# ingonyama-zk/blaze

Measured on AMD Instinct MI355X. Metric: BLS12-381 MSM/s at 2^26, higher is better.
Workload: dtype u32 registers holding 28-bit limbs (381-bit Fq, Montgomery)

## Files before the change

### blaze_amd/_lib.py

```python
from __future__ import annotations

import ctypes as C
import os

_HERE = os.path.dirname(os.path.abspath(__file__))
LIB_PATH = os.environ.get("BLAZE_HIP_LIB") or os.path.join(_HERE, "lib", "libblaze_hip.so")


class DriverClientError(Exception):

    VARIANTS = {
        1: "WriteError",
        2: "ReadError",
        3: "HBICAPNotReady",
        4: "InvalidPrimitiveParam",
        5: "CsvError",
        6: "LoadFailed",
        7: "FileError",
        8: "Unknown",
    }

    def __init__(self, code: int, message: str):
        self.code = code
        self.variant = self.VARIANTS.get(code, "Unknown")
        super().__init__(f"{self.variant}: {message}")


_lib = None
_aux = None

class BlzVecArg(C.Structure):
    _fields_ = [("d_ptr", C.c_void_p), ("buf", C.c_uint32), ("reserved", C.c_uint32), ("count", C.c_uint64)]


class BlzVecView(C.Structure):
    _fields_ = [("offset", C.c_uint64), ("stride", C.c_uint64), ("len", C.c_uint64)]


GATE_MAX_TABLES, GATE_MAX_TERMS, GATE_MAX_FACTORS, GATE_MAX_POINTS = 12, 8, 4, 6


class BlzGateTerm(C.Structure):
    _fields_ = [("nfactors", C.c_uint8), ("negate", C.c_uint8), ("factor", C.c_uint8 * GATE_MAX_FACTORS), ("reserved", C.c_uint8 * 2)]


class BlzSumGate(C.Structure):
    _fields_ = [("ntables", C.c_uint32), ("nterms", C.c_uint32), ("common", C.c_int32), ("reserved", C.c_uint32),
                ("term", BlzGateTerm * GATE_MAX_TERMS)]


class BlzVecCsr(C.Structure):
    _fields_ = [("d_row_ptr", C.c_void_p), ("d_col", C.c_void_p), ("d_val", C.c_void_p), ("rows", C.c_uint64), ("nnz", C.c_uint64)]


class BlzVecScatter(C.Structure):
    _fields_ = [("d_idx", C.c_void_p), ("d_src", C.c_void_p), ("d_val", C.c_void_p), ("nnz", C.c_uint64), ("reserved", C.c_uint64)]


_u8p = C.c_void_p
_SIGS = {
    "blz_last_error_message": (C.c_char_p, []),
    "blz_device_count": (C.c_int, []),
    "blz_point_size": (C.c_size_t, [C.c_int]),
    "blz_result_size": (C.c_size_t, [C.c_int]),
    "blz_msm_new": (C.c_int, [C.c_int, C.c_int, C.c_int, C.c_int, C.POINTER(C.c_void_p)]),
    "blz_msm_free": (None, [C.c_void_p]),
    "blz_msm_loaded_binary_parameters": (C.c_int, [C.c_void_p, C.POINTER(C.c_uint32)]),
    "blz_msm_initialize": (C.c_int, [C.c_void_p, C.c_uint32, C.c_int, C.c_uint64, C.c_uint64]),
    "blz_msm_start_process": (C.c_int, [C.c_void_p]),
    "blz_msm_set_data": (C.c_int, [C.c_void_p, _u8p, C.c_size_t, _u8p, C.c_size_t, C.c_uint32, C.c_int, C.c_uint64, C.c_uint64]),
    "blz_msm_set_data_device": (C.c_int, [C.c_void_p, _u8p, C.c_size_t, _u8p, C.c_size_t, C.c_uint32, C.c_int, C.c_uint64, C.c_uint64]),
    "blz_msm_wait_result": (C.c_int, [C.c_void_p]),
    "blz_msm_result": (C.c_int, [C.c_void_p, _u8p, C.c_size_t, C.POINTER(C.c_size_t), C.POINTER(C.c_uint32)]),
    "blz_msm_load_data_to_hbm": (C.c_int, [C.c_void_p, _u8p, C.c_size_t, C.c_uint64, C.c_uint64]),
    "blz_msm_load_data_to_hbm_device": (C.c_int, [C.c_void_p, _u8p, C.c_size_t, C.c_uint64, C.c_uint64]),
    "blz_msm_get_data_from_hbm": (C.c_int, [C.c_void_p, _u8p, C.c_size_t, C.c_uint64, C.c_uint64]),
    "blz_arena_release": (C.c_int, [C.c_int]),
    "blz_arena_set_policy": (C.c_int, [C.c_int, C.c_uint32]),
    "blz_arena_export": (C.c_int, [C.c_int, C.c_char_p]),
    "blz_arena_attach": (C.c_int, [C.c_int, C.c_char_p]),
    "blz_msm_stream": (C.c_int, [C.c_void_p, C.POINTER(C.c_void_p), C.POINTER(C.c_int)]),
    "blz_msm_task_label": (C.c_int, [C.c_void_p, C.POINTER(C.c_uint32)]),
    "blz_msm_nof_elements": (C.c_int, [C.c_void_p, C.POINTER(C.c_uint32)]),
    "blz_msm_is_engine_ready": (C.c_int, [C.c_void_p, C.POINTER(C.c_uint32)]),
    "blz_msm_stream_progress": (C.c_int, [C.c_void_p, C.POINTER(C.c_uint32)]),
    "blz_msm_reset": (C.c_int, [C.c_void_p]),
    "blz_msm_last_timings": (C.c_int, [C.c_void_p, C.POINTER(C.c_float)]),
    "blz_comm_unique_id": (C.c_int, [_u8p]),
    "blz_msm_comm_init": (C.c_int, [C.c_void_p, C.c_int, C.c_int, _u8p]),
    "blz_msm_all_gather_combine": (C.c_int, [C.c_void_p, _u8p, _u8p, C.c_size_t]),
    "blz_msm_comm_init_all": (C.c_int, [C.POINTER(C.c_void_p), C.c_int]),
    "blz_msm_all_gather_combine_all": (C.c_int, [C.POINTER(C.c_void_p), C.c_int, _u8p, _u8p, C.c_size_t]),
    "blz_msm_comm_free": (C.c_int, [C.c_void_p]),
    "blz_msm_precompute_bases_device": (C.c_int, [C.c_int, C.c_int, C.c_void_p, C.c_void_p, C.c_uint64]),
    "blz_msm_combine_partials": (C.c_int, [C.c_void_p, _u8p, C.c_size_t, _u8p, C.c_size_t]),
    "blz_msm_last_sort_hidden": (C.c_int, [C.c_void_p, C.POINTER(C.c_int)]),
    "blz_msm_memory_info": (C.c_int, [C.c_void_p, C.POINTER(C.c_uint64)]),
    "blz_msm_set_window_table": (C.c_int, [C.c_void_p, C.c_int]),
    "blz_msm_prepare_window_table": (C.c_int, [C.c_void_p, C.c_uint32, C.c_uint64, C.c_uint64, C.c_int, C.POINTER(C.c_int)]),
    "blz_msm_set_precompute_plan": (C.c_int, [C.c_void_p, C.c_int]),
    "blz_msm_prepare_precompute_plan": (C.c_int, [C.c_void_p, C.c_uint32, C.c_uint64, C.c_uint64, C.POINTER(C.c_int)]),
    "blz_msm_precompute_plan_info": (C.c_int, [C.c_void_p, C.POINTER(C.c_uint64)]),
    "blz_msm_set_scalar_range": (C.c_int, [C.c_void_p, C.c_uint32, C.c_uint32]),
    "blz_msm_shard_layout": (C.c_int, [C.c_int, C.c_uint32, C.c_int, C.c_int, C.POINTER(C.c_uint32)]),
    "blz_msm_shard_layout_ex": (C.c_int, [C.c_int, C.c_uint32, C.c_int, C.c_int, C.c_uint32, C.POINTER(C.c_uint32)]),
    "blz_msm_shard_layout_candidate": (C.c_int, [C.c_int, C.c_uint32, C.c_int, C.c_int, C.c_uint32, C.c_int, C.POINTER(C.c_uint32)]),
    "blz_msm_window_table_info": (C.c_int, [C.c_void_p, C.POINTER(C.c_uint64)]),
    "blz_msm_plan": (C.c_int, [C.c_int, C.c_uint32, C.c_int, C.POINTER(C.c_uint32), C.POINTER(C.c_uint8)]),
    "blz_ntt_new": (C.c_int, [C.c_int, C.c_int, C.POINTER(C.c_void_p)]),
    "blz_ntt_new_ex": (C.c_int, [C.c_int, C.c_int, C.c_int, C.POINTER(C.c_void_p)]),
    "blz_ntt_new_field": (C.c_int, [C.c_int, C.c_int, C.c_int, C.c_int, C.POINTER(C.c_void_p)]),
    "blz_ntt_new_ex2": (C.c_int, [C.c_int, C.c_int, C.c_int, C.c_int, C.c_uint32, C.POINTER(C.c_void_p)]),
    "blz_ntt_new_ex3": (C.c_int, [C.c_int, C.c_int, C.c_int, C.c_uint32, C.c_void_p, C.POINTER(C.c_void_p)]),
    "blz_ntt_set_coset": (C.c_int, [C.c_void_p, C.c_void_p]),
    "blz_ntt_get_coset": (C.c_int, [C.c_void_p, _u8p]),
    "blz_ntt_info": (C.c_int, [C.c_void_p, C.POINTER(C.c_uint64)]),
    "blz_ntt_exchange": (C.c_int, [C.c_void_p, C.c_size_t, _u8p, C.c_size_t, _u8p, C.c_size_t]),
    "blz_ntt_free": (None, [C.c_void_p]),
    "blz_ntt_initialize": (C.c_int, [C.c_void_p]),
    "blz_ntt_set_data": (C.c_int, [C.c_void_p, C.c_size_t, _u8p, C.c_size_t]),
    "blz_ntt_set_data_device": (C.c_int, [C.c_void_p, C.c_size_t, _u8p, C.c_size_t]),
    "blz_ntt_start_process": (C.c_int, [C.c_void_p, C.c_size_t]),
    "blz_ntt_wait_result": (C.c_int, [C.c_void_p]),
    "blz_ntt_result": (C.c_int, [C.c_void_p, C.c_size_t, _u8p, C.c_size_t]),
    "blz_ntt_result_device": (C.c_int, [C.c_void_p, C.c_size_t, _u8p, C.c_size_t]),
    "blz_ntt_stream": (C.c_int, [C.c_void_p, C.POINTER(C.c_void_p), C.POINTER(C.c_int)]),
    "blz_ntt_reset": (C.c_int, [C.c_void_p]),
    "blz_ntt_last_kernel_ms": (C.c_int, [C.c_void_p, C.POINTER(C.c_float)]),
    "blz_ntt_gate_eval": (C.c_int, [C.c_void_p, C.POINTER(BlzSumGate), C.POINTER(BlzVecArg), C.POINTER(BlzVecArg), C.POINTER(C.c_uint64), C.c_uint64]),
    "blz_ntt_vec_op": (C.c_int, [C.c_void_p, C.c_int, C.c_size_t, C.POINTER(BlzVecArg), C.POINTER(BlzVecArg), C.POINTER(BlzVecArg)]),
    "blz_ntt_vec_reduce": (C.c_int, [C.c_void_p, C.c_int, C.POINTER(BlzVecArg), C.POINTER(BlzVecArg), C.c_void_p]),
    "blz_ntt_vec_scan": (C.c_int, [C.c_void_p, C.c_int, C.c_uint32, C.c_size_t, C.POINTER(BlzVecArg), C.c_void_p]),
    "blz_ntt_vec_horner": (C.c_int, [C.c_void_p, C.c_uint32, C.c_size_t, C.POINTER(BlzVecArg), C.POINTER(BlzVecArg), C.c_void_p]),
    "blz_ntt_vec_gather": (C.c_int, [C.c_void_p, C.c_size_t, C.POINTER(BlzVecArg), C.POINTER(BlzVecView)]),
    "blz_ntt_vec_scatter": (C.c_int, [C.c_void_p, C.c_size_t, C.POINTER(BlzVecArg), C.POINTER(BlzVecScatter)]),
    "blz_ntt_vec_spmv": (C.c_int, [C.c_void_p, C.c_size_t, C.POINTER(BlzVecArg), C.POINTER(BlzVecCsr)]),
    "blz_ntt_vec_mle_fold": (C.c_int, [C.c_void_p, C.c_uint32, C.POINTER(BlzVecArg), C.POINTER(BlzVecArg), C.POINTER(BlzVecArg), C.c_uint64]),
    "blz_ntt_vec_mle_round": (C.c_int, [C.c_void_p, C.c_uint32, C.POINTER(BlzVecArg), C.POINTER(BlzVecArg), C.POINTER(BlzVecArg), C.c_uint32,
                                        C.c_uint64, C.c_void_p]),
    "blz_ntt_vec_mle_eq": (C.c_int, [C.c_void_p, C.POINTER(BlzVecArg), C.c_void_p, C.c_uint32]),
    "blz_ntt_banks_preprocess_device": (C.c_int, [C.c_void_p, _u8p, _u8p]),
    "blz_ntt_banks_postprocess_device": (C.c_int, [C.c_void_p, _u8p, _u8p]),
    "blz_ntt_sumcheck_step": (C.c_int, [C.c_void_p, C.c_uint32, C.POINTER(BlzVecArg), C.POINTER(BlzVecArg), C.POINTER(BlzVecArg), C.POINTER(BlzVecArg),
                                        C.POINTER(BlzVecArg), C.c_uint32, C.c_uint64, C.c_void_p]),
    "blz_ntt_sumcheck_gate": (C.c_int, [C.c_void_p, C.POINTER(BlzSumGate), C.POINTER(BlzVecArg), C.POINTER(BlzVecArg), C.c_uint32, C.c_uint64, C.c_void_p]),
    "blz_poseidon_new": (C.c_int, [C.c_int, C.c_int, C.POINTER(C.c_void_p)]),
    "blz_poseidon_free": (None, [C.c_void_p]),
    "blz_poseidon_loaded_binary_parameters": (C.c_int, [C.c_void_p, C.POINTER(C.c_uint32)]),
    "blz_poseidon_initialize": (C.c_int, [C.c_void_p, C.c_uint32, C.c_int, C.c_char_p]),
    "blz_poseidon_check_words": (C.c_int, [C.c_int, C.c_int, _u8p, C.c_size_t, C.POINTER(C.c_uint32)]),
    "blz_poseidon_initialize_words": (C.c_int, [C.c_void_p, C.c_uint32, C.c_int, _u8p, C.c_size_t]),
    "blz_poseidon_set_data": (C.c_int, [C.c_void_p, _u8p, C.c_size_t]),
    "blz_poseidon_set_data_device": (C.c_int, [C.c_void_p, C.c_void_p, C.c_size_t]),
    "blz_poseidon_wait_result": (C.c_int, [C.c_void_p]),
    "blz_poseidon_num_pending_results": (C.c_int, [C.c_void_p, C.POINTER(C.c_uint32)]),
    "blz_poseidon_raw_results": (C.c_int, [C.c_void_p, C.c_uint32, _u8p, C.c_size_t]),
    "blz_poseidon_result": (C.c_int, [C.c_void_p, C.c_uint32, _u8p, C.c_size_t, C.POINTER(C.c_uint32)]),
    "blz_poseidon_tree_device": (C.c_int, [C.c_void_p, C.c_void_p, C.c_size_t]),
    "blz_poseidon_counters": (C.c_int, [C.c_void_p, C.POINTER(C.c_uint32)]),
    "blz_poseidon_info": (C.c_int, [C.c_void_p, C.POINTER(C.c_uint64)]),
    "blz_poseidon_set_round_plan": (C.c_int, [C.c_void_p, C.c_int]),
    "blz_poseidon_prepare_round_plan": (C.c_int, [C.c_void_p, C.POINTER(C.c_uint32)]),
    "blz_poseidon_last_kernel_ms": (C.c_int, [C.c_void_p, C.POINTER(C.c_float)]),
    "blz_poseidon_stream": (C.c_int, [C.c_void_p, C.POINTER(C.c_void_p), C.POINTER(C.c_int)]),
    "blz_poseidon_reset": (C.c_int, [C.c_void_p]),
    "blz_device_malloc": (C.c_int, [C.c_int, C.c_size_t, C.POINTER(C.c_void_p)]),
    "blz_device_free": (C.c_int, [C.c_int, C.c_void_p]),
    "blz_host_malloc": (C.c_int, [C.c_int, C.c_size_t, C.POINTER(C.c_void_p)]),
    "blz_host_free": (C.c_int, [C.c_void_p]),
    "blz_memcpy_h2d": (C.c_int, [C.c_int, C.c_void_p, _u8p, C.c_size_t]),
    "blz_memcpy_d2h": (C.c_int, [C.c_int, _u8p, C.c_void_p, C.c_size_t]),
}
EXPORTED_SYMBOLS = tuple(_SIGS)
_AUX_SIGS = {
    "blz_synth_scalars": (C.c_int, [C.c_int, C.c_int, C.c_void_p, C.c_uint64, C.c_uint64]),
    "blz_synth_scalars_at": (C.c_int, [C.c_int, C.c_int, C.c_void_p, C.c_uint64, C.c_uint64, C.c_uint64]),
    "blz_synth_points": (C.c_int, [C.c_int, C.c_int, C.c_void_p, C.c_uint64, C.c_int, C.c_uint64]),
    "blz_synth_field_elements": (C.c_int, [C.c_int, C.c_void_p, C.c_uint64, C.c_uint64]),
    "blz_calib_mad_rate": (C.c_int, [C.c_int, C.c_uint32, C.POINTER(C.c_double)]),
    "blz_test_msm_stall": (C.c_int, [C.c_void_p, C.c_uint32, C.POINTER(C.c_void_p)]),
    "blz_test_ntt_stall": (C.c_int, [C.c_void_p, C.c_uint32, C.POINTER(C.c_void_p)]),
    "blz_test_stall_release": (C.c_int, [C.c_void_p]),
    "blz_test_field_op": (C.c_int, [C.c_int, C.c_int, C.c_int, C.c_int, _u8p, _u8p, _u8p, C.c_size_t]),
    "blz_test_ec_op": (C.c_int, [C.c_int, C.c_int, C.c_int, _u8p, _u8p, _u8p, _u8p, _u8p, C.c_size_t]),
    "blz_test_msm_tail_plan": (C.c_int, [C.c_int, C.c_int, C.c_uint32, C.c_int, C.c_int, C.c_int, C.c_int, C.c_int, C.POINTER(C.c_uint32), C.POINTER(C.c_uint8),
                                         C.c_char_p, C.c_size_t]),
    "blz_test_msm_sort_plan": (C.c_int, [C.c_int, C.c_int, C.c_uint32, C.c_int, C.c_int, C.c_int, C.c_int, C.c_int, C.c_int, C.c_int, C.c_int, C.c_int,
                                         C.c_char_p, C.c_size_t]),
    "blz_test_law_layout": (C.c_int, [C.c_int, C.c_int, C.c_int, C.POINTER(C.c_uint32)]),
    "blz_test_law_op": (C.c_int, [C.c_int, C.c_int, C.c_int, C.c_int, C.c_int, C.c_int, C.c_uint32, C.c_uint32, _u8p, _u8p, C.c_size_t]),
    "blz_test_rr_layout": (C.c_int, [C.c_int, C.c_int, C.POINTER(C.c_uint32)]),
    "blz_test_rr_op": (C.c_int, [C.c_int, C.c_int, C.c_int, C.c_int, C.c_int, _u8p, _u8p, C.c_size_t]),
    "blz_test_sort_fits_beside": (C.c_int, [C.c_int, C.c_int, C.c_int, C.c_int]),
    "blz_test_poseidon_permute": (C.c_int, [C.c_int, C.c_int, _u8p, C.c_size_t, C.c_int, _u8p, _u8p, C.c_size_t]),
    "blz_test_poseidon_hash": (C.c_int, [C.c_int, C.c_int, _u8p, C.c_size_t, C.c_int, _u8p, _u8p, C.c_size_t]),
    "blz_test_poseidon_hash_plan": (C.c_int, [C.c_int, C.c_int, _u8p, C.c_size_t, C.c_int, _u8p, _u8p, C.c_size_t, C.POINTER(C.c_uint32)]),
    "blz_test_poseidon_tree_check": (C.c_int, [C.c_int, C.c_int, _u8p, C.c_size_t, C.c_int, C.c_uint32, C.c_void_p, C.c_void_p, C.POINTER(C.c_uint64)]),
}
AUX_EXPORTED_SYMBOLS = tuple(_AUX_SIGS)


def lib():
    global _lib
    if _lib is None:
        if not os.path.exists(LIB_PATH):
            raise RuntimeError(
                f"{LIB_PATH} is missing: build it with `make -C blaze_amd/csrc` "
                "(or __graft_entry__.build()); blaze_amd has no CPU fallback"
            )
        L = C.CDLL(LIB_PATH, mode=C.RTLD_GLOBAL)
        for name, (res, args) in _SIGS.items():
            fn = getattr(L, name)
            fn.restype = res
            fn.argtypes = args
        _lib = L
    return _lib


def aux():
    global _aux
    if _aux is None:
        lib()
        path = LIB_PATH[:-3] + "_aux.so"
        if not os.path.exists(path):
            raise RuntimeError(f"{path} is missing: build it with `make -C blaze_amd/csrc`")
        A = C.CDLL(path)
        for name, (res, args) in _AUX_SIGS.items():
            fn = getattr(A, name)
            fn.restype = res
            fn.argtypes = args
        _aux = A
    return _aux


def check(rc: int):
    if rc != 0:
        msg = lib().blz_last_error_message()
        raise DriverClientError(rc, msg.decode() if msg else "")


def buf_ptr(buf):
    if buf is None:
        return None, 0, None
    if isinstance(buf, bytes):
        return C.cast(C.c_char_p(buf), C.c_void_p), len(buf), buf
    if isinstance(buf, bytearray):
        arr = (C.c_char * len(buf)).from_buffer(buf)
        return C.cast(arr, C.c_void_p), len(buf), arr
    if hasattr(buf, "ctypes") and hasattr(buf, "nbytes"):
        if not buf.flags["C_CONTIGUOUS"]:
            raise ValueError("numpy array is not C-contiguous: pass np.ascontiguousarray(a) (inputs) or a contiguous buffer (outputs)")
        return C.c_void_p(buf.ctypes.data), int(buf.nbytes), buf
    mv = memoryview(buf)
    if mv.readonly:
        b = mv.tobytes()
        return C.cast(C.c_char_p(b), C.c_void_p), len(b), b
    arr = (C.c_char * mv.nbytes).from_buffer(mv)
    return C.cast(arr, C.c_void_p), mv.nbytes, arr


class DeviceBuffer:

    def __init__(self, device_id: int, nbytes: int):
        self.device_id = device_id
        self.nbytes = nbytes
        p = C.c_void_p()
        check(lib().blz_device_malloc(device_id, nbytes, C.byref(p)))
        self.ptr = p.value

    def upload(self, data):
        p, n, _keep = buf_ptr(data)
        assert n <= self.nbytes
        check(lib().blz_memcpy_h2d(self.device_id, self.ptr, p, n))

    def download(self, nbytes: int | None = None, offset: int = 0) -> bytearray:
        n = self.nbytes - offset if nbytes is None else nbytes
        out = bytearray(n)
        p, _, _keep = buf_ptr(out)
        check(lib().blz_memcpy_d2h(self.device_id, p, self.ptr + offset, n))
        return out

    def free(self):
        if self.ptr:
            lib().blz_device_free(self.device_id, self.ptr)
            self.ptr = None

    def __del__(self):
        try:
            self.free()
        except Exception:
            pass


class HostBuffer:

    def __init__(self, device_id: int, nbytes: int):
        self.nbytes = nbytes
        p = C.c_void_p()
        check(lib().blz_host_malloc(device_id, nbytes, C.byref(p)))
        self.ptr = p.value
        self._arr = (C.c_uint8 * nbytes).from_address(self.ptr)

    def array(self):
        import numpy as np

        return np.frombuffer(self._arr, dtype=np.uint8)

    def free(self):
        if self.ptr:
            self._arr = None
            lib().blz_host_free(self.ptr)
            self.ptr = None

    def __del__(self):
        try:
            self.free()
        except Exception:
            pass
```

### blaze_amd/csrc/msm.hip

```cpp
#include "msm_engine.hpp"
#include <mutex>
#include "field.hip.hpp"
#include "msm_digits.hip.hpp"

namespace blz {

size_t fq_bytes(int curve) { return curve == BLZ_BN254 ? 32 : 48; }
size_t mont_point_bytes(int curve) { return curve == BLZ_BN254 ? 64 : 128; }

static uint32_t unit_length(uint32_t npts, int W) {
    const double chain = (double)npts * W * 5.5e-6;
    uint32_t L = 16;
    while (L < 256 && 2.0 * L <= chain) L <<= 1;
    return L;
}

static MsmPlan search_plan(uint32_t npts, int sbits, int ebits, int force_c, int split_ns, int max_w) {
    MsmPlan best;
    double best_cost = 1e300;
    const double t_entry = 0.163, t_bucket = 0.62, t_empty = 0.03, t_hot = 0.01;
    const int need = sbits + 1;
    const double t_split = (double)split_ns;
    for (int cmin = 3; cmin <= 23; ++cmin) {
        if (force_c > 0 && cmin != force_c) continue;
// ... 47 lines not shown
                    }
                    best.boff[W] = b;
                    best.Wv = (int)(G >> (cmin - 1));
                    best.cost = cost;
                    best.ebits = ebits;
                }
            }
        }
    }
    best.L = unit_length(npts, best.W);
    return best;
}

MsmPlan make_plan(uint32_t npts, int sbits, int ebits, int force_c) {
    if (ebits <= 0 || ebits > sbits) ebits = sbits;
    const int split_ns = plan_override("split_ns", 6000);
    struct Memo {
        uint32_t npts = 0;
        int sbits = 0, ebits = 0, force_c = 0, split_ns = 0;
        MsmPlan plan;
    };
    static std::mutex mu;
    static Memo memo[16];
    static unsigned next = 0;
    {
        std::lock_guard<std::mutex> lk(mu);
        for (const Memo& m : memo)
            if (m.sbits == sbits && m.npts == npts && m.ebits == ebits && m.force_c == force_c && m.split_ns == split_ns) return m.plan;
    }
    const int max_w = (sbits == 64 && force_c == 0 && npts >= (3u << 22)) ? 3 : MSM_MAX_W;
    const MsmPlan P = search_plan(npts, sbits, ebits, force_c, split_ns, max_w);
    std::lock_guard<std::mutex> lk(mu);
    Memo& m = memo[next++ % 16];
    m.npts = npts; m.sbits = sbits; m.ebits = ebits; m.force_c = force_c; m.split_ns = split_ns;
    m.plan = P;
    return P;
}

int table_window_bits(uint32_t npts, int need_bits) {
    const int forced = plan_override("table_c", 0);
    int best = 0;
    double best_cost = 1e300;
    for (int c = 16; c <= 26; ++c) {
        if (forced > 0 && c != forced) continue;
        const int W = table_windows(c, need_bits);
        if (c > 16 && table_windows(c - 1, need_bits) == W && forced <= 0) continue;
        if ((uint64_t)npts * W >= (1ull << 30)) continue;
        const double cost = (double)npts * W * 0.130 + (double)(1ull << (c - 1)) * 0.34;
        if (cost < best_cost) { best_cost = cost; best = c; }
    }
    return best;
}

MsmPlan make_table_plan(uint32_t npts, int c, int need_bits) {
    MsmPlan P;
    if (c < 16 || c > 26 || need_bits < 2 || need_bits > 257) return P;
    const int W = table_windows(c, need_bits);
    if ((uint64_t)npts * W >= (1ull << 30)) return P;
    P.npts = npts; P.sbits = need_bits - 1; P.c = c; P.W = W; P.table = true;
    P.G = 1ull << (c - 1);
    for (int w = 0; w < W; ++w) { P.width[w] = (uint8_t)c; P.boff[w] = 0; }
    P.boff[W] = (uint32_t)P.G;
    P.Bw = 1u << (c - 1 - 5);
    P.Wv = 32;
    P.L = unit_length(npts, W);
    return P;
}

int plan_tail(const MsmPlan& P, TailTraits tr, bool piecewise, TailPlan& T) {
    T = TailPlan();
    const uint64_t maxunits = ((uint64_t)P.npts * (P.table ? P.W : 1) + P.L - 1) / P.L;
    for (uint64_t stride = 1; stride < maxunits; stride *= 16) ++T.unit_passes;
    T.thr = ((uint64_t)P.npts * P.W / (P.G ? P.G : 1) > P.L / 2 || P.npts <= (1u << 22)) ? 64u : 0u;
    T.hot_start = (uint32_t)P.G;
    if (tr.rr && !P.table && !piecewise && P.ebits > 0) {
        int lowest = -1, off = 0;
        bool any = false;
        int offs[MSM_MAX_W];
        for (int w = 0; w < P.W; ++w) { offs[w] = off; off += P.width[w]; }
        for (int w = P.W - 1; w >= 0; --w) {
            const int cw = P.width[w];
            int t = P.ebits - offs[w];
            if (t > cw) t = cw;
            const double slots = (double)(1ull << (cw - 1));
            double active = t >= cw ? slots : t > 0 ? (double)(1ull << t) + 1.0 : t == 0 ? 1.0 : 0.0;
            if (active > slots) active = slots;
            const double entries = t >= 0 ? (double)P.npts : 0.0;
            const bool hot = active > 0 && entries / active >= 12.0 * (double)P.L;
            if (!hot && entries > 0) break;
            lowest = w;
            any = any || hot;
        }
        if (any && lowest > 0 && P.G - P.boff[lowest] <= 16384) T.hot_start = P.boff[lowest];
    }
    if (T.hot_start < P.G) T.hot = tr.row ? TailPlan::HOT_ROW : TailPlan::HOT_WAVES8;

    uint32_t seg0 = 64;
    while (seg0 > 8 && P.G / seg0 < 262144) seg0 >>= 1;
    seg0 = (uint32_t)exp_knob("BLAZE_MSM_SEG", (int)seg0);
    const uint32_t segu = (uint32_t)exp_knob("BLAZE_MSM_SEG_UPPER", 8);
    const uint32_t quad_max = (uint32_t)exp_knob("BLAZE_REDUCE_QUAD_MAX", 131072), row_max = (uint32_t)exp_knob("BLAZE_REDUCE_ROW_MAX", 8192);
    bool row_levels = false;
    int shift = 0;
    for (uint32_t M = P.Bw;;) {
        if (T.levels == 16) return fail(BLZ_ERR_UNKNOWN, "bucket reduce of %u buckets per window needs more than 16 levels (segments of %u / %u)", P.Bw, seg0, segu);
        TailPlan::Level& l = T.level[T.levels];
        l.M = M;
        l.SEG = T.levels == 0 ? seg0 : segu;
        l.T = l.SEG ? (M + l.SEG - 1) / l.SEG : M;
        l.shift = shift;
        if (tr.row && l.T * (uint32_t)P.Wv <= row_max) row_levels = true;
        l.kind = row_levels ? TailPlan::Level::ROW : !tr.rr ? TailPlan::Level::W32
                 : T.levels > 0 || l.T * (uint32_t)P.Wv <= quad_max ? TailPlan::Level::QUAD : TailPlan::Level::RR;
        for (uint32_t t = 1; t < l.SEG; t <<= 1) ++shift;
        ++T.levels;
        M = l.T;
        if (M == 1) break;
    }

    if (T.thr == 0 || T.hot_start == 0) T.fold = TailPlan::FOLD_NONE;
    else if (tr.row && !piecewise && P.G <= (1u << 17) && (uint64_t)P.npts * P.W / P.L <= (1u << 17))
        T.fold = T.level[0].kind == TailPlan::Level::ROW ? TailPlan::FOLD_ROW_WEAK : TailPlan::FOLD_ROW_STRICT;
    else
        T.fold = tr.rr && T.hot_start <= 32768 ? TailPlan::FOLD_WAVE : TailPlan::FOLD_LANE;

    T.finish_row = tr.row;
    FinishPlan& fp = T.fp;
    fp.W = P.W;
    fp.logV = 0;
    while ((1u << fp.logV) < P.Bw) ++fp.logV;
    if (P.table) {
        fp.W = 1;
        fp.v0[0] = 0;
        fp.m[0] = (uint8_t)(P.G >> fp.logV);
        fp.off[0] = 0;
    } else {
        int off = P.base_bit;
        for (int w = 0; w < P.W; ++w) {
            const uint32_t v0 = P.boff[w] >> fp.logV, m = (P.boff[w + 1] - P.boff[w]) >> fp.logV;
            if (v0 > 0xffffu || m > 0xffu || off > 0xffff)
                return fail(BLZ_ERR_UNKNOWN, "window plan outside k_finish's table range (window %d: v0=%u m=%u off=%d)", w, v0, m, off);
            fp.v0[w] = (uint16_t)v0;
            fp.m[w] = (uint8_t)m;
            fp.off[w] = (uint16_t)off;
            off += P.width[w];
        }
    }

    const char* bad = nullptr;
    if ((T.hot == TailPlan::HOT_WAVES8 || T.fold == TailPlan::FOLD_WAVE) && !tr.rr) bad = "a reduced-radix fold";
    if ((T.hot == TailPlan::HOT_ROW || T.fold == TailPlan::FOLD_ROW_STRICT || T.fold == TailPlan::FOLD_ROW_WEAK || T.finish_row) && !tr.row) bad = "a row-law kernel";
    if (!T.finish_row && tr.row) bad = "the quad walk";
    if (T.fold == TailPlan::FOLD_ROW_WEAK && T.level[0].kind != TailPlan::Level::ROW) bad = "a weak row fold without a row level 0 behind it";
    for (int l = 0; l < T.levels && !bad; ++l) {
        const TailPlan::Level::Kind k = T.level[l].kind;
        if (k == TailPlan::Level::ROW ? !tr.row : k == TailPlan::Level::W32 ? tr.rr : !tr.rr) bad = "a reduce level on a law the field lacks";
        else if (k == TailPlan::Level::RR && l > 0) bad = "the lane-per-segment reduced-radix level above level 0";
        else if (l > 0 && T.level[l - 1].kind == TailPlan::Level::ROW && k != TailPlan::Level::ROW) bad = "a row level in front of another law's";
    }
    if (bad) return fail(BLZ_ERR_UNKNOWN, "tail plan names %s (%s)", bad, describe(T).c_str());
    return BLZ_OK;
}

std::string describe(const TailPlan& T) {
    static const char* const hot[] = {"", " hot", " hot_row"};
    static const char* const fold[] = {"none", "lane", "wave", "row_strict", "row_weak"};
    static const char* const kind[] = {"w32", "rr", "quad", "row"};
    std::string s = "units" + std::to_string(T.unit_passes) + hot[T.hot] + " fold_" + fold[T.fold] + " |";
    for (int l = 0; l < T.levels; ++l) s += std::string(l ? " L" : " L0") + kind[T.level[l].kind];
    return s + (T.finish_row ? " finish_row" : " finish");
}

__global__ __launch_bounds__(64) void k_words_to_pinned(uint32_t* __restrict__ dst, const uint32_t* __restrict__ src, uint32_t n) {
    __builtin_amdgcn_s_setprio(3);
    if (threadIdx.x < n) __hip_atomic_store(dst + threadIdx.x, src[threadIdx.x], __ATOMIC_RELAXED, __HIP_MEMORY_SCOPE_SYSTEM);
}
int copy_words_to_pinned(void* host_pinned, const void* d_src, uint32_t dwords, hipStream_t st) {
    if (dwords > 64) return fail(BLZ_ERR_UNKNOWN, "copy_words_to_pinned: %u dwords", dwords);
    hipLaunchKernelGGL(k_words_to_pinned, dim3(1), dim3(64), 0, st, (uint32_t*)host_pinned, (const uint32_t*)d_src, dwords);
    BLZ_HIP(hipGetLastError(), BLZ_ERR_READ);
    return BLZ_OK;
}

__global__ __launch_bounds__(256) void k_iota(uint32_t* __restrict__ p, uint64_t n) {
    for (uint64_t i = (uint64_t)blockIdx.x * 256 + threadIdx.x; i < n; i += (uint64_t)gridDim.x * 256) p[i] = (uint32_t)i;
}


const MsmCurveOps* msm_ops_for(int curve, int repr) {
    switch (curve) {
        case BLZ_BLS377: return &msm_ops_bls377();
        case BLZ_BLS381: return &msm_ops_bls381();
        case BLZ_BN254: return repr ? &msm_ops_bn254_w32() : &msm_ops_bn254();
    }
    return nullptr;
}

int msm_points_from_mont(int format_id, const void* d_mont, void* d_raw, uint64_t npts, hipStream_t st) {
    const MsmCurveOps* ops = (format_id >> 16) ? nullptr : msm_ops_for(format_id & 0xff, (format_id >> 8) & 0xff);
    if (!ops) return fail(BLZ_ERR_UNKNOWN, "no conversion back from Montgomery format 0x%x", format_id);
    return ops->points_from_mont(d_mont, d_raw, npts, st);
}
int msm_points_all_canonical(int format_id, const void* d_raw, uint64_t npts, uint32_t* flag, hipStream_t st) {
    const MsmCurveOps* ops = msm_ops_for(format_id & 0xff, (format_id >> 8) & 0xff);
    if (!ops) return fail(BLZ_ERR_UNKNOWN, "unknown Montgomery format 0x%x", format_id);
    return ops->points_all_canonical(d_raw, npts, flag, st);
}

int MsmEngine::init(int device_id, int curve_id, int precompute_factor) {
    device = device_id;
    curve = curve_id;
    repr = 0;
    if (curve == BLZ_BN254) {
        repr = exp_knob("BLAZE_BN254_REPR", precompute_factor > 1 ? 1 : 0) ? 1 : 0;
    }
    if (!msm_ops_for(curve, repr)) return fail(BLZ_ERR_INVALID_PARAM, "unknown curve %d", curve);
    BLZ_TRY(use_device(device));
    int prio_low = 0, prio_high = 0;
    BLZ_HIP(hipDeviceGetStreamPriorityRange(&prio_low, &prio_high), BLZ_ERR_UNKNOWN);
    BLZ_HIP(hipStreamCreateWithFlags(&stream, hipStreamNonBlocking), BLZ_ERR_UNKNOWN);
    BLZ_HIP(hipStreamCreateWithPriority(&tail_stream, hipStreamNonBlocking, prio_high), BLZ_ERR_UNKNOWN);
    BLZ_HIP(hipStreamCreateWithPriority(&aux_stream, hipStreamNonBlocking, prio_high), BLZ_ERR_UNKNOWN);
    BLZ_HIP(hipStreamCreateWithPriority(&sort_stream, hipStreamNonBlocking, prio_high), BLZ_ERR_UNKNOWN);
    last_sort_done = nullptr;
    for (auto& S : slots) {
        BLZ_TRY(for_each_event(S, [](hipEvent_t& e, bool timed) -> int {
            if (timed) BLZ_HIP(hipEventCreate(&e), BLZ_ERR_UNKNOWN);
            else BLZ_HIP(hipEventCreateWithFlags(&e, hipEventDisableTiming), BLZ_ERR_UNKNOWN);
            return BLZ_OK;
        }));
        BLZ_HIP(hipHostMalloc((void**)&S.result_h, 256), BLZ_ERR_UNKNOWN);
        BLZ_HIP(hipHostMalloc((void**)&S.stats_h, 64), BLZ_ERR_UNKNOWN);
        memset(S.stats_h, 0, 64);
    }
    BLZ_HIP(hipHostMalloc((void**)&combine_h, 256), BLZ_ERR_UNKNOWN);
    for (auto& B : sbuf) BLZ_TRY(B.stats.reserve(64));
    BLZ_TRY(result.reserve(256 * 64));
    return BLZ_OK;
}

bool MsmEngine::destroy() {
    if (!stream) return true;
    (void)hipSetDevice(device);
    if (sync_stream_bounded(stream, "free: main stream") != BLZ_OK || sync_stream_bounded(tail_stream, "free: tail stream") != BLZ_OK ||
        sync_stream_bounded(sort_stream, "free: sort stream") != BLZ_OK) {
        BLZ_LOG(0, "MSM engine freed while its device work is wedged: workspace and streams are leaked");
        stream = tail_stream = aux_stream = sort_stream = nullptr;
        return false;
    }
    for_each_buf([](DevBuf& b) { b.release(); });
    for (auto& S : slots) {
        (void)for_each_event(S, [](hipEvent_t& e, bool) -> int { if (e) (void)hipEventDestroy(e); return BLZ_OK; });
        if (S.result_h) (void)hipHostFree(S.result_h);
        if (S.stats_h) (void)hipHostFree(S.stats_h);
        S = MsmSlot();
    }
    inputs_event = nullptr;
    if (combine_h) (void)hipHostFree(combine_h);
    combine_h = nullptr;
    for (hipStream_t s : {stream, tail_stream, aux_stream, sort_stream}) (void)hipStreamDestroy(s);
    stream = tail_stream = aux_stream = sort_stream = nullptr;
    last_sort_done = nullptr;
    return true;
}

bool MsmEngine::can_accept() const {
    for (const auto& S : slots)
        if (!S.busy) return true;
    return false;
}

int MsmEngine::sync_all() {
    BLZ_TRY(use_device(device));
    BLZ_TRY(sync_stream_bounded(stream, "reset: main stream"));
    BLZ_TRY(sync_stream_bounded(tail_stream, "reset: tail stream"));
    BLZ_TRY(sync_stream_bounded(aux_stream, "reset: exchange stream"));
    BLZ_TRY(sync_stream_bounded(sort_stream, "reset: sort stream"));
    for (auto& S : slots) { S.busy = false; S.open = false; S.task_inputs_event = nullptr; }
    return BLZ_OK;
}

int MsmEngine::points_to_mont(const void* d_raw, void* d_mont, uint32_t npts) {
    BLZ_TRY(use_device(device));
    return msm_ops_for(curve, repr)->points_to_mont(*this, d_raw, d_mont, npts);
}

int MsmEngine::points_to_mont_even(const void* d_raw, void* d_mont, uint32_t nq) {
    BLZ_TRY(use_device(device));
    return msm_ops_for(curve, repr)->points_to_mont_even(*this, d_raw, d_mont, nq);
}
int MsmEngine::check_precompute(const void* d_raw, uint64_t nelem, uint32_t* flag, hipStream_t st) {
    BLZ_TRY(use_device(device));
    return msm_ops_for(curve, 0)->check_precompute(*this, d_raw, nelem, flag, st);
}

int MsmEngine::build_table(const void* d_raw, void* d_table, uint32_t npts, int c, int W, int base_shift, void* scratch, uint32_t* flag,
                           hipStream_t st) {
    BLZ_TRY(use_device(device));
    return msm_ops_for(curve, repr)->build_table(*this, d_raw, d_table, npts, c, W, base_shift, scratch, flag, st);
}
size_t MsmEngine::table_scratch_bytes(int W) const { return msm_ops_for(curve, repr)->table_scratch_bytes(W); }

static const int kScalarFieldBits[3] = {253, 255, 254};

MsmPlan MsmEngine::plan_for(uint32_t npts, int sbits) const {
    const int ebits = sbits == 256 ? kScalarFieldBits[curve] : sbits;
    return make_plan(npts, sbits, ebits, plan_override("c", 0));
}

static MsmPlan range_plan(int curve, uint32_t npts, int bit_lo, int bit_hi) {
    const int vbits = bit_hi - bit_lo;
    int ebits = kScalarFieldBits[curve] - bit_lo;
    if (ebits > vbits) ebits = vbits;
    if (ebits < 1) ebits = 1;
    MsmPlan P = make_plan(npts, vbits, ebits, plan_override("c", 0));
    P.base_bit = bit_lo;
    return P;
}
MsmPlan MsmEngine::plan_for_range(uint32_t npts, int bit_lo, int bit_hi) const { return range_plan(curve, npts, bit_lo, bit_hi); }

int msm_task_plan(int curve, uint32_t npts, int sbits, int table_c, int bit_lo, int bit_hi, MsmPlan& P, bool* ranged_out) {
    if (curve < 0 || curve > 2) return fail(BLZ_ERR_INVALID_PARAM, "unknown curve %d", curve);
    const int ebits = sbits == 256 ? kScalarFieldBits[curve] : sbits;
    const bool ranged = bit_hi > bit_lo && !(bit_lo == 0 && bit_hi >= sbits);
    if (ranged && (sbits != 256 || (bit_lo & 31) || (bit_hi & 31) || bit_hi > 256))
        return fail(BLZ_ERR_INVALID_PARAM, "scalar range [%d, %d): 32-bit aligned ranges of 256-bit scalars", bit_lo, bit_hi);
    P = table_c > 0 ? make_table_plan(npts, table_c, ranged ? bit_hi - bit_lo + 1 : 257)
        : ranged    ? range_plan(curve, npts, bit_lo, bit_hi)
                    : make_plan(npts, sbits, ebits, plan_override("c", 0));
    if (P.c == 0) return fail(BLZ_ERR_INVALID_PARAM, "no window plan for npts=%u sbits=%d%s", npts, sbits, table_c > 0 ? " (window table)" : "");
    if (P.table && !msm_sort3_ok(P, sbits)) return fail(BLZ_ERR_INVALID_PARAM, "window-table task outside the sort's range (c=%d)", P.c);
    P.L = (uint32_t)plan_override("L", (int)P.L);
    if (P.L < 1) P.L = 1;
    if (P.L > (uint32_t)MAX_L) P.L = MAX_L;
    if (ranged_out) *ranged_out = ranged;
    return BLZ_OK;
}

int msm_task_pieces(const MsmPlan& P, int want, bool phased, uint32_t* per_out) {
    if (want < 1 || P.table) want = 1;
    if (want > MSM_MAX_SLICES) want = MSM_MAX_SLICES;
    const uint64_t halves = (phased && want >= 4) ? 2ull * want - 1 : 2ull * want;
    const uint32_t per = (uint32_t)(((2ull * P.npts + halves - 1) / halves + 15) & ~(uint64_t)15);
    if (want > 1) want = (int)(((uint64_t)P.npts + per - 1) / per);
    *per_out = want > 1 ? per : P.npts;
    return want;
}

int MsmEngine::take_slot(int* slot_out) {
    int slot = (rr_cursor + 1) % MSM_QUEUE_DEPTH;
    if (slots[slot].busy) slot = (slot + 1) % MSM_QUEUE_DEPTH;
    if (slots[slot].busy) return fail(BLZ_ERR_INVALID_PARAM, "task queue full (%d tasks in flight)", MSM_QUEUE_DEPTH);
    *slot_out = slot;
    return BLZ_OK;
}

int MsmEngine::step(int slot, int piece, bool curve_kernels, std::optional<MsmStep>& out) {
    BLZ_TRY(use_device(device));
    if (slot < 0 || slot >= MSM_QUEUE_DEPTH || !slots[slot].open) return fail(BLZ_ERR_INVALID_PARAM, "slot %d has no task being enqueued", slot);
    MsmSlot& S = slots[slot];
    if (curve_kernels && S.repr != repr) return fail(BLZ_ERR_INVALID_PARAM, "the handle's arithmetic changed while task %d was being enqueued", slot);
    if (S.slices == 1) piece = -1;
    const int set = S.sort.where == SortPlan::PINGPONG && piece >= 0 ? (slot + piece) % MSM_QUEUE_DEPTH : slot;
    out.emplace(MsmStep{slot, S, piece, S.plan, sbuf[set], stream, S.sort.where != SortPlan::OPEN ? sort_stream : stream});
    return BLZ_OK;
}

int MsmEngine::begin(uint32_t npts, int sbits, int* slot_out, int table_c, int bit_lo, int bit_hi, int nslices, bool phased) {
    BLZ_TRY(use_device(device));
    const MsmCurveOps* ops = msm_ops_for(curve, repr);
    hipStream_t st = stream;
    if (npts == 0) return fail(BLZ_ERR_INVALID_PARAM, "begin: empty task");
    int slot = -1;
    BLZ_TRY(take_slot(&slot));
    MsmSlot& S = slots[slot];
    MsmPlan P;
    bool ranged = false;
    BLZ_TRY(msm_task_plan(curve, npts, sbits, table_c, bit_lo, bit_hi, P, &ranged));
    const uint64_t G = P.G;
    uint32_t per = npts;
    nslices = msm_task_pieces(P, nslices, phased, &per);
    BLZ_TRY(plan_tail(P, ops->tail, nslices > 1, S.tail));
    const SortInputs sort_in = {env_int("BLAZE_SORT_HIDE", 1), slots[(slot + 1) % MSM_QUEUE_DEPTH].busy, recent_hot[0] || recent_hot[1],
                                msm_sort_fits_beside(ops->accumulate_vgprs(), msm_sort3_max_vgprs(P.table), ops->accumulate_lds(), msm_sort3_max_lds(P.table))};
    const SortPlan sort = plan_sort(P, npts, sbits, nslices, sort_in);
    BLZ_LOG(2, "msm plan: npts=%u sbits=%d c=%d W=%d Bw=%u G=%llu L=%u pieces=%d sort: %s tail: %s", npts, sbits, P.c, P.W, P.Bw,
            (unsigned long long)G, P.L, nslices, describe(sort).c_str(), describe(S.tail).c_str());
    const uint64_t max_entries = (uint64_t)per * P.W;
    const uint64_t max_units = G + max_entries / P.L + 1;
    if (max_units >= (1ull << 32)) return fail(BLZ_ERR_INVALID_PARAM, "unit bound %llu exceeds 32 bits", (unsigned long long)max_units);

    rr_cursor = slot;
    if (slot_out) *slot_out = slot;
    S.plan = P;
    S.npts = npts;
    S.sbits = sbits;
    S.ranged = ranged;
    S.bit_lo = bit_lo;
    S.bit_hi = bit_hi;
    S.repr = repr;
    S.slices = nslices;
    S.pts_per_slice = per;
    S.max_units = max_units;
    S.sort = sort;
    S.acc_pp_recorded[0] = S.acc_pp_recorded[1] = false;
    S.phased = phased;
    S.task_inputs_event = inputs_event;
    S.accum_timed = false;
    BLZ_HIP(hipEventRecord(S.ev[0], st), BLZ_ERR_UNKNOWN);
    for (int b = 0; b < MSM_QUEUE_DEPTH; ++b) {
        if (b != slot && sort.where != SortPlan::PINGPONG) continue;
        BLZ_TRY(sbuf[b].count.reserve((G + 1) * 4 + 16));
        BLZ_TRY(sbuf[b].off.reserve((G + 2) * 4));
        BLZ_TRY(sbuf[b].unit_off.reserve((G + 2) * 4));
        BLZ_TRY(sbuf[b].entries.reserve(max_entries * 4));
    }
    BLZ_TRY(blocksums.reserve((size_t)((G + 1 + SCAN_TILE - 1) / SCAN_TILE) * 8));
    if (nslices > 1) {
        const size_t sum_bytes = (size_t)ops->tail.partial_dwords * 4;
        BLZ_TRY(bucket_sums.reserve((G + 1) * sum_bytes));
        BLZ_TRY(bucket_ident.reserve((G + 2) * 4));
        launch_zero(bucket_sums.p, ((G + 1) * sum_bytes + 15) / 16, st);
        BLZ_HIP(hipGetLastError(), BLZ_ERR_UNKNOWN);
    }
    S.open = true;
    S.busy = true;
    return BLZ_OK;
}

int MsmEngine::sort_slice(int slot, int sl, const void* d_scalars, uint32_t np) {
    std::optional<MsmStep> C;
    BLZ_TRY(step(slot, sl, false, C));
    MsmSlot& S = C->S;
    if (sl < 0 || sl >= S.slices || np == 0 || np > S.pts_per_slice) return fail(BLZ_ERR_INVALID_PARAM, "piece %d of %d with %u points", sl, S.slices, np);
    rr_cursor = slot;
    MsmSlot& O = slots[(slot + 1) % MSM_QUEUE_DEPTH];
    const bool hide = S.sort.where != SortPlan::OPEN, pingpong = S.sort.where == SortPlan::PINGPONG;
    hipStream_t ss = C->sort_stream;
    if (last_sort_done) BLZ_HIP(hipStreamWaitEvent(ss, last_sort_done, 0), BLZ_ERR_UNKNOWN);
    if (hide) {
        if (pingpong && S.acc_pp_recorded[sl & 1]) {
            BLZ_HIP(hipStreamWaitEvent(ss, S.ev_acc_pp[sl & 1], 0), BLZ_ERR_UNKNOWN);
        } else {
            if (S.l0_recorded) BLZ_HIP(hipStreamWaitEvent(ss, S.ev_l0, 0), BLZ_ERR_UNKNOWN);
            if (O.sort.where == SortPlan::PINGPONG && O.l0_recorded) BLZ_HIP(hipStreamWaitEvent(ss, O.ev_l0, 0), BLZ_ERR_UNKNOWN);
        }
    }
    BLZ_HIP(hipEventRecord(S.ev_s0, ss), BLZ_ERR_UNKNOWN);
    BLZ_TRY(msm_sort_stage(*this, *C, d_scalars, np));
    hipEvent_t sorted = pingpong ? S.ev_sorted_pp[sl & 1] : S.ev_sorted;
    BLZ_HIP(hipEventRecord(sorted, ss), BLZ_ERR_UNKNOWN);
    last_sort_done = sorted;
    BLZ_HIP(hipEventRecord(S.ev_s1, ss), BLZ_ERR_UNKNOWN);
    if (!S.phased && S.task_inputs_event && sl + 1 == S.slices) {
        if (hide) BLZ_HIP(hipStreamWaitEvent(ss, S.ev[0], 0), BLZ_ERR_UNKNOWN);
        BLZ_HIP(hipEventRecord(S.task_inputs_event, ss), BLZ_ERR_UNKNOWN);
        S.task_inputs_event = nullptr;
    }
    return BLZ_OK;
}

int MsmEngine::accumulate_slice(int slot, int sl, const void* d_pts) {
    std::optional<MsmStep> C;
    BLZ_TRY(step(slot, sl, true, C));
    MsmSlot& S = C->S;
    const MsmCurveOps* ops = msm_ops_for(curve, repr);
    rr_cursor = slot;
    const bool pingpong = S.sort.where == SortPlan::PINGPONG;
    if (S.sort.where != SortPlan::OPEN) BLZ_HIP(hipStreamWaitEvent(stream, pingpong ? S.ev_sorted_pp[sl & 1] : S.ev_sorted, 0), BLZ_ERR_UNKNOWN);
    BLZ_TRY(ops->run_accumulate(*this, *C, d_pts, (uint32_t)S.max_units));
    if (S.slices > 1) BLZ_TRY(ops->merge_buckets(*this, *C));
    if (pingpong) {
        BLZ_HIP(hipEventRecord(S.ev_acc_pp[sl & 1], stream), BLZ_ERR_UNKNOWN);
        S.acc_pp_recorded[sl & 1] = true;
    }
    return BLZ_OK;
}

int MsmEngine::end(int slot) {
    std::optional<MsmStep> C;
    BLZ_TRY(step(slot, -1, true, C));
    MsmSlot& S = C->S;
    const MsmCurveOps* ops = msm_ops_for(curve, repr);
    rr_cursor = slot;
    if (S.task_inputs_event) {
        BLZ_HIP(hipEventRecord(S.task_inputs_event, stream), BLZ_ERR_UNKNOWN);
        S.task_inputs_event = nullptr;
    }
    if (S.slices > 1) {
        hipLaunchKernelGGL(k_iota, dim3(1024), dim3(256), 0, stream, bucket_ident.as<uint32_t>(), S.plan.G + 2);
        BLZ_TRY(ops->run_reduce(*this, *C, bucket_sums.p, bucket_ident.p));
    } else {
        BLZ_TRY(ops->run_reduce(*this, *C, partial.p, C->B.unit_off.p));
    }
    S.l0_recorded = true;
    S.open = false;
    return BLZ_OK;
}

void MsmEngine::abandon(int slot) {
    if (slot < 0 || slot >= MSM_QUEUE_DEPTH) return;
    MsmSlot& S = slots[slot];
    if (S.busy && S.open) {
        S.busy = false;
        S.open = false;
        S.task_inputs_event = nullptr;
    }
}

int MsmEngine::run(const void* d_pts, const void* d_scalars, uint32_t npts, int sbits, int* slot_out, int table_c, int bit_lo,
                   int bit_hi) {
    BLZ_TRY(use_device(device));
    if (npts == 0) {
        hipStream_t st = stream;
        int slot = -1;
        BLZ_TRY(take_slot(&slot));
        rr_cursor = slot;
        MsmSlot& S = slots[slot];
        if (slot_out) *slot_out = slot;
        BLZ_HIP(hipEventRecord(S.ev[0], st), BLZ_ERR_UNKNOWN);
        BLZ_TRY(msm_ops_for(curve, repr)->emit_infinity(*this, slot));
        for (int i = 1; i <= 4; ++i) BLZ_HIP(hipEventRecord(S.ev[i], st), BLZ_ERR_UNKNOWN);
        BLZ_TRY(copy_words_to_pinned(S.result_h, slot_result(slot), (uint32_t)(3 * fq_bytes(curve) / 4), st));
        BLZ_HIP(hipEventRecord(S.ev_done, st), BLZ_ERR_UNKNOWN);
        S.plan = MsmPlan();
        S.accum_timed = false;
        S.open = false;
        S.busy = true;
        return BLZ_OK;
    }
    int pieces = env_int("BLAZE_MSM_PIECES", 1);
    int slot = -1;
    BLZ_TRY(begin(npts, sbits, &slot, table_c, bit_lo, bit_hi, pieces, false));
    if (slot_out) *slot_out = slot;
    MsmSlot& S = slots[slot];
    int rc = BLZ_OK;
    for (int sl = 0; sl < S.slices && rc == BLZ_OK; ++sl) {
        const uint32_t p0 = (uint32_t)sl * S.pts_per_slice;
        const uint32_t np = npts - p0 < S.pts_per_slice ? npts - p0 : S.pts_per_slice;
        rc = sort_slice(slot, sl, (const char*)d_scalars + (size_t)p0 * (sbits / 8), np);
        if (rc == BLZ_OK) rc = accumulate_slice(slot, sl, (const char*)d_pts + (size_t)p0 * mont_point_bytes(curve));
    }
    if (rc == BLZ_OK) rc = end(slot);
    if (rc != BLZ_OK) abandon(slot);
    return rc;
}

int MsmEngine::finish(int slot, uint8_t* out) {
    BLZ_TRY(use_device(device));
    if (slot < 0 || slot >= MSM_QUEUE_DEPTH || !slots[slot].busy) return fail(BLZ_ERR_INVALID_PARAM, "no task in slot %d", slot);
    if (slots[slot].open) return fail(BLZ_ERR_INVALID_PARAM, "task in slot %d never received all of its data", slot);
    MsmSlot& S = slots[slot];
    BLZ_TRY(sync_event_bounded(S.ev_done, "wait_result: MSM task"));
    S.busy = false;
    if (S.plan.c) {
        BLZ_LOG(2, "msm: units=%u max_bucket=%u entries=%u", S.stats_h[0], S.stats_h[1], S.stats_h[2]);
        if ((uint64_t)S.stats_h[0] > S.max_units) return fail(BLZ_ERR_UNKNOWN, "unit count %u exceeds its bound", S.stats_h[0]);
        const uint64_t mean = (uint64_t)S.stats_h[2] / (S.plan.G ? S.plan.G : 1) + 1;
        recent_hot[1] = recent_hot[0];
        recent_hot[0] = (uint64_t)S.stats_h[1] > 64 * mean + 4096;
    }
    memcpy(out, S.result_h, 3 * fq_bytes(curve));
    float t = 0;
    (void)hipEventElapsedTime(&t, S.ev[0], S.ev[4]); last_ms[0] = t;
    last_ms[1] = 0;
    if (S.accum_timed && S.plan.c) {
        if (S.slices > 1) {
            for (int i = 0; i < S.slices; ++i)
                if (hipEventElapsedTime(&t, S.slice_ev[2 * i], S.slice_ev[2 * i + 1]) == hipSuccess) last_ms[1] += t;
        } else {
            (void)hipEventElapsedTime(&t, S.ev[5], S.ev[6]);
            last_ms[1] = t;
        }
    }
    last_sort_hidden = S.sort.where != SortPlan::OPEN && S.plan.c != 0;
    if (S.plan.c) (void)hipEventElapsedTime(&t, S.ev_s0, S.ev_s1);
    else t = 0;
    last_ms[2] = t;
    (void)hipEventElapsedTime(&t, S.ev[1], S.ev[2]); last_ms[3] = t;
    (void)hipEventElapsedTime(&t, S.ev[2], S.ev[3]); last_ms[4] = t;
    (void)hipEventElapsedTime(&t, S.ev[3], S.ev[4]); last_ms[5] = t;
    last_ms[6] = (float)S.plan.c;
    last_ms[7] = (float)S.plan.W;
    return BLZ_OK;
}

int MsmEngine::combine_partials(const uint8_t* partials, size_t cnt, uint8_t* out, bool on_device) {
    BLZ_TRY(use_device(device));
    return msm_ops_for(curve, repr)->combine(*this, partials, cnt, out, on_device);
}

}
```

### blaze_amd/csrc/msm_engine.hpp

```cpp
#pragma once
#include "common.hpp"
#include <optional>

namespace blz {

constexpr int MSM_MAX_W = 96;
constexpr uint64_t MSM_MAX_ENTRIES = (1ull << 32) - (1ull << 26);
struct MsmPlan {
    uint32_t npts = 0;
    int sbits = 256;
    int c = 0;
    int W = 0;
    uint8_t width[MSM_MAX_W] = {};
    uint32_t boff[MSM_MAX_W + 1] = {};
    uint32_t Bw = 0;
    int Wv = 0;
    uint64_t G = 0;
    uint32_t L = 0;
    bool table = false;
    int ebits = 0;
    int base_bit = 0;
    double cost = 0;
};
MsmPlan make_plan(uint32_t npts, int sbits, int ebits, int force_c);
int table_window_bits(uint32_t npts, int need_bits = 257);
inline int table_windows(int c, int need_bits = 257) { return (need_bits + c - 1) / c; }
MsmPlan make_table_plan(uint32_t npts, int c, int need_bits = 257);
int msm_task_plan(int curve, uint32_t npts, int sbits, int table_c, int bit_lo, int bit_hi, MsmPlan& P, bool* ranged);
int msm_task_pieces(const MsmPlan& P, int want, bool phased, uint32_t* per);

struct TailTraits {
    bool rr = false;
    bool row = false;
    int partial_dwords = 0;
};
struct FinishPlan {
    int W, logV;
    uint16_t v0[MSM_MAX_W], off[MSM_MAX_W];
    uint8_t m[MSM_MAX_W];
};
struct TailPlan {
    uint32_t thr = 0, hot_start = 0;
    int unit_passes = 0;
    enum Hot { HOT_NONE, HOT_WAVES8, HOT_ROW } hot = HOT_NONE;
    enum Fold { FOLD_NONE, FOLD_LANE, FOLD_WAVE, FOLD_ROW_STRICT, FOLD_ROW_WEAK } fold = FOLD_NONE;
    struct Level {
        uint32_t M, SEG, T;
        int shift;
        enum Kind { W32, RR, QUAD, ROW } kind;
    } level[16];
    int levels = 0;
    bool finish_row = false;
    FinishPlan fp;
};
int plan_tail(const MsmPlan& P, TailTraits tr, bool piecewise, TailPlan& out);
std::string describe(const TailPlan& T);

struct SortPlan {
    enum Kind { LDS, S3, TINY } kind;
    enum Where { OPEN, HIDDEN, PINGPONG } where;
};
struct SortInputs { int hide_env; bool other_busy, recent_hot, fits; };
SortPlan plan_sort(const MsmPlan& P, uint32_t npts, int sbits, int pieces, const SortInputs& in);
std::string describe(const SortPlan&);
constexpr int SCAN_TILE = 2048;
constexpr int MAX_L = 1024;

constexpr int MSM_QUEUE_DEPTH = 2;
constexpr int MSM_MAX_SLICES = 64;
struct MsmSlot {
    hipEvent_t ev[8] = {};
    hipEvent_t ev_l0 = nullptr;
    hipEvent_t ev_sorted = nullptr;
    hipEvent_t ev_s0 = nullptr, ev_s1 = nullptr;
    bool l0_recorded = false;
    hipEvent_t ev_done = nullptr;
    DevBuf lvlA[2], lvlC[2];
    uint8_t* result_h = nullptr;
    uint32_t* stats_h = nullptr;
    uint64_t max_units = 0;
    MsmPlan plan;
    SortPlan sort{};
    TailPlan tail;
    hipEvent_t slice_ev[2 * 64] = {};
    int slices = 1;
    bool accum_timed = false;
    bool busy = false;
    bool open = false;
    bool phased = false;
    bool ranged = false;
    uint32_t npts = 0, pts_per_slice = 0;
    int sbits = 0, bit_lo = 0, bit_hi = 0;
    int repr = 0;
    hipEvent_t task_inputs_event = nullptr;
    hipEvent_t ev_sorted_pp[2] = {nullptr, nullptr};
    hipEvent_t ev_acc_pp[2] = {nullptr, nullptr};
    bool acc_pp_recorded[2] = {false, false};
};

struct MsmStep;
struct MsmEngine {
    int device = 0;
    int curve = 0;
    int repr = 0;
    int format_id() const { return curve | (repr << 8); }
    hipStream_t stream = nullptr, tail_stream = nullptr, aux_stream = nullptr;
    MsmSlot slots[MSM_QUEUE_DEPTH];
    int rr_cursor = 0;
    struct SortBufs {
        DevBuf count, off, unit_off, unit_bucket, unit_order, lenhist, entries, stats;
        DevBuf range_scalars;
    };
    SortBufs sbuf[MSM_QUEUE_DEPTH];
    hipStream_t sort_stream = nullptr;
    hipEvent_t last_sort_done = nullptr;
    DevBuf coarse, inter, inter2, slice_map, partial, blocksums, result, sort3_tabs;
    DevBuf bucket_sums, bucket_ident;
    int begin(uint32_t npts, int sbits, int* slot, int table_c, int bit_lo, int bit_hi, int pieces, bool phased);
    int sort_slice(int slot, int piece, const void* d_scalars, uint32_t np);
    int accumulate_slice(int slot, int piece, const void* d_points_mont);
    int end(int slot);
    void abandon(int slot);
    int take_slot(int* slot);
    int step(int slot, int piece, bool curve_kernels, std::optional<MsmStep>& out);
    hipEvent_t inputs_event = nullptr;
    uint8_t* combine_h = nullptr;
    float last_ms[8] = {};
    bool last_sort_hidden = false;
    bool recent_hot[2] = {false, false};
    template <class Fn>
    void for_each_buf(Fn&& f) {
        for (DevBuf* b : {&coarse, &inter, &inter2, &slice_map, &partial, &blocksums, &result, &sort3_tabs, &bucket_sums, &bucket_ident}) f(*b);
        for (auto& B : sbuf)
            for (DevBuf* b : {&B.count, &B.off, &B.unit_off, &B.unit_bucket, &B.unit_order, &B.lenhist, &B.entries, &B.stats, &B.range_scalars}) f(*b);
        for (auto& S : slots)
            for (DevBuf* b : {&S.lvlA[0], &S.lvlA[1], &S.lvlC[0], &S.lvlC[1]}) f(*b);
    }
    template <class Fn>
    static int for_each_event(MsmSlot& S, Fn&& f) {
        for (auto& e : S.ev) BLZ_TRY(f(e, true));
        for (auto& e : S.slice_ev) BLZ_TRY(f(e, true));
        for (hipEvent_t* e : {&S.ev_l0, &S.ev_done, &S.ev_sorted, &S.ev_sorted_pp[0], &S.ev_acc_pp[0], &S.ev_sorted_pp[1], &S.ev_acc_pp[1]}) BLZ_TRY(f(*e, false));
        for (hipEvent_t* e : {&S.ev_s0, &S.ev_s1}) BLZ_TRY(f(*e, true));
        return BLZ_OK;
    }

    int init(int device_id, int curve_id, int precompute_factor);
    bool destroy();
    uint32_t* slot_result(int s) { return result.as<uint32_t>() + (size_t)s * 64; }
    bool can_accept() const;
    MsmPlan plan_for(uint32_t npts, int sbits) const;
    int points_to_mont(const void* d_raw, void* d_mont, uint32_t npts);
    int points_to_mont_even(const void* d_raw, void* d_mont, uint32_t nq);
    int check_precompute(const void* d_raw, uint64_t nelem, uint32_t* flag, hipStream_t st);
    int build_table(const void* d_raw, void* d_table, uint32_t npts, int c, int W, int base_shift, void* scratch, uint32_t* flag,
                    hipStream_t st);
    size_t table_scratch_bytes(int W) const;
    int run(const void* d_points_mont, const void* d_scalars, uint32_t npts, int sbits, int* slot, int table_c = 0, int bit_lo = 0,
            int bit_hi = 0);
    MsmPlan plan_for_range(uint32_t npts, int bit_lo, int bit_hi) const;
    int finish(int slot, uint8_t* out);
    int combine_partials(const uint8_t* partials, size_t count, uint8_t* out, bool on_device);
    int sync_all();
};

struct MsmStep {
    int slot;
    MsmSlot& S;
    int piece;
    const MsmPlan& P;
    MsmEngine::SortBufs& B;
    hipStream_t stream, sort_stream;
};

int msm_points_from_mont(int format_id, const void* d_mont, void* d_raw, uint64_t npts, hipStream_t st);
int msm_points_all_canonical(int format_id, const void* d_raw, uint64_t npts, uint32_t* flag, hipStream_t st);
int copy_words_to_pinned(void* host_pinned, const void* d_src, uint32_t dwords, hipStream_t st);
size_t fq_bytes(int curve);
size_t mont_point_bytes(int curve);
int msm_sort_stage(MsmEngine& E, const MsmStep& C, const void* d_scalars, uint32_t np);
void launch_zero(void* p, size_t n16, hipStream_t st);
bool msm_sort3_ok(const MsmPlan& P, int sbits);
int msm_sort3_max_vgprs(bool table);
int msm_sort3_max_lds(bool table);
bool msm_sort_fits_beside(int av, int sv, int al, int sl);
bool msm_sort_tiny_ok(const MsmPlan& P, uint32_t npts, int sbits);

struct MsmCurveOps {
    int (*points_to_mont)(MsmEngine&, const void* d_raw, void* d_mont, uint32_t npts);
    int (*emit_infinity)(MsmEngine&, int slot);
    int (*run_accumulate)(MsmEngine&, const MsmStep& C, const void* d_pts, uint32_t max_units);
    int (*merge_buckets)(MsmEngine&, const MsmStep& C);
    int (*run_reduce)(MsmEngine&, const MsmStep& C, const void* sums, const void* unit_off);
    TailTraits tail;
    int (*accumulate_vgprs)();
    int (*accumulate_lds)();
    int (*build_table)(MsmEngine&, const void* d_raw, void* d_table, uint32_t npts, int c, int W, int base_shift, void* scratch,
                       uint32_t* flag, hipStream_t st);
    size_t (*table_scratch_bytes)(int W);
    int (*combine)(MsmEngine&, const uint8_t* partials, size_t count, uint8_t* out, bool on_device);
    int (*points_to_mont_even)(MsmEngine&, const void* d_raw, void* d_mont, uint32_t nq);
    int (*check_precompute)(MsmEngine&, const void* d_raw, uint64_t nelem, uint32_t* flag, hipStream_t st);
    int (*points_from_mont)(const void* d_mont, void* d_raw, uint64_t npts, hipStream_t st);
    int (*points_all_canonical)(const void* d_raw, uint64_t npts, uint32_t* flag, hipStream_t st);
};
const MsmCurveOps& msm_ops_bls377();
const MsmCurveOps& msm_ops_bls381();
const MsmCurveOps& msm_ops_bn254();
const MsmCurveOps& msm_ops_bn254_w32();
const MsmCurveOps* msm_ops_for(int curve, int repr = 0);

}
```

### blaze_amd/csrc/msm_sort3.hip

```cpp
#include "msm_sort.hpp"
#include "msm_digits.hip.hpp"

namespace blz {

constexpr int S3_THREADS = 256;
constexpr int S3_SH1 = 14;
constexpr int S3_SH2 = 7;
#ifndef BLZ_S3_T
#define BLZ_S3_T 8
#endif
constexpr int S3_T = BLZ_S3_T;
constexpr int S3_PB = S3_THREADS * S3_T;
constexpr uint32_t S3_SLICE2 = 4096;
constexpr int S3_T2 = S3_SLICE2 / S3_THREADS;
constexpr int S3_T3 = 28;
constexpr uint32_t S3_R3 = S3_THREADS * S3_T3;
constexpr uint32_t S3_MAXNB1 = 2048;
constexpr uint32_t S3_CNT_PTS = 16384;
constexpr uint32_t S3T_IMG = 12288;

struct S3Geom {
    int W, prio;
    uint32_t NB1;
    uint8_t width[MSM_MAX_W];
    uint16_t bitoff[MSM_MAX_W];
    uint16_t binoff1[MSM_MAX_W + 1];
    static constexpr bool TABLE = false;
    static constexpr uint32_t HIST1 = S3_MAXNB1;
    using Win = int;
    __device__ int cw(int w) const { return width[w]; }
    __device__ uint32_t first_bin(int w) const { return binoff1[w]; }
    __device__ static constexpr uint32_t shift1() { return S3_SH1; }
    static constexpr uint32_t bits3() { return S3_SH2; }
    __device__ static uint32_t index1(uint32_t p, uint32_t, uint32_t) { return p; }
    __device__ static uint32_t rem1(uint32_t rem) { return rem; }
    struct L2 {
        int prio;
        using Lo = uint8_t;
        static constexpr uint32_t TAB2 = 128;
        static constexpr uint32_t KY_D = 8, KY_R = 16;
        static constexpr uint32_t LO_MASK = 127u;
        __device__ static constexpr uint32_t shift2() { return S3_SH2; }
        __device__ static constexpr uint32_t bits2() { return S3_SH1 - S3_SH2; }
        __device__ static uint32_t low2(uint32_t r, uint32_t) { return r & 127u; }
        __device__ static uint32_t index2(uint32_t iw) { return iw; }
    };
    L2 l2() const { return L2{prio}; }
};

struct S3TGeom {
    int W, prio, c;
    uint32_t sh1, b2, b3, xs, NB1;
    static constexpr bool TABLE = true;
    static constexpr uint32_t HIST1 = 256;
    using Win = uint32_t;
    __device__ int cw(int) const { return c; }
    __device__ static constexpr uint32_t first_bin(int) { return 0; }
    __device__ uint32_t shift1() const { return sh1; }
    uint32_t bits3() const { return b3; }
    __device__ uint32_t index1(uint32_t p, uint32_t w, uint32_t rem) const { return (p * (uint32_t)W + w) | (xs ? (rem & 1u) << 30 : 0u); }
    __device__ uint32_t rem1(uint32_t rem) const { return rem >> xs; }
    using L2 = S3TGeom;
    using Lo = uint16_t;
    static constexpr uint32_t TAB2 = 256;
    static constexpr uint32_t KY_D = 10, KY_R = 18;
    static constexpr uint32_t LO_MASK = 0x3ffu;
    __device__ uint32_t shift2() const { return b3 - xs; }
    __device__ uint32_t bits2() const { return b2; }
    __device__ uint32_t low2(uint32_t r, uint32_t iw) const {
        const uint32_t lomask = (1u << shift2()) - 1u;
        return xs ? ((r & lomask) << 1) | ((iw >> 30) & 1u) : (r & lomask);
    }
    __device__ static uint32_t index2(uint32_t iw) { return iw & 0xbfffffffu; }
    const L2& l2() const { return *this; }
};

__device__ __forceinline__ void s3_setprio(int p) {
    if (p >= 3) __builtin_amdgcn_s_setprio(3);
    else if (p == 2) __builtin_amdgcn_s_setprio(2);
    else if (p == 1) __builtin_amdgcn_s_setprio(1);
}

__device__ __forceinline__ uint32_t s3_wave_incl_scan(uint32_t v) {
    for (int o = 1; o < 64; o <<= 1) {
        uint32_t t = __shfl_up(v, o, 64);
        if ((threadIdx.x & 63u) >= (uint32_t)o) v += t;
    }
    return v;
}
__device__ __forceinline__ uint32_t s3_block_excl_scan(uint32_t v, uint32_t* wave_tot, uint32_t* total) {
    const uint32_t incl = s3_wave_incl_scan(v);
    if ((threadIdx.x & 63u) == 63u) wave_tot[threadIdx.x >> 6] = incl;
    __syncthreads();
    uint32_t wbase = 0;
    for (uint32_t q = 0; q < (threadIdx.x >> 6); ++q) wbase += wave_tot[q];
    *total = wave_tot[0] + wave_tot[1] + wave_tot[2] + wave_tot[3];
    return wbase + incl - v;
}

template <class Geom, int NW>
__global__ __launch_bounds__(S3_THREADS, 4) void k3_l1_count(const uint32_t* __restrict__ scalars, uint32_t npts, Geom g,
                                                            uint32_t* __restrict__ cnt1) {
    s3_setprio(g.prio);
    __shared__ uint32_t hist[Geom::HIST1];
    if constexpr (Geom::HIST1 == S3_THREADS) hist[threadIdx.x] = 0;
    else for (uint32_t i = threadIdx.x; i < g.NB1; i += S3_THREADS) hist[i] = 0;
    __syncthreads();
    const uint32_t base = blockIdx.x * S3_CNT_PTS;
    uint32_t end = base + S3_CNT_PTS;
    if (end > npts) end = npts;
    for (uint32_t p0 = base + threadIdx.x; p0 < end; p0 += 4 * S3_THREADS) {
        ScalarWords<NW> sw[4];
#pragma unroll
        for (int u = 0; u < 4; ++u) {
            const uint32_t p = p0 + u * S3_THREADS;
            sw[u].load(scalars, p < end ? p : p0);
        }
#pragma unroll
        for (int u = 0; u < 4; ++u) {
            if (p0 + u * S3_THREADS >= end) break;
            uint32_t carry = 0;
            for (int w = 0; w < g.W; ++w) {
                const int cw = g.cw(w);
                const int d = sw[u].next(cw, (1u << cw) - 1u, 1u << (cw - 1), carry);
                if (d != 0) {
                    const uint32_t b = (uint32_t)(d < 0 ? -d : d) - 1u;
                    atomicAdd(&hist[g.first_bin(w) + (b >> g.shift1())], 1u);
                }
            }
        }
    }
    __syncthreads();
    auto flush = [&](uint32_t i) {
        const uint32_t v = hist[i];
        if (v) atomicAdd(&cnt1[i], v);
    };
    if constexpr (Geom::HIST1 == S3_THREADS) { if (threadIdx.x < g.NB1) flush(threadIdx.x); }
    else for (uint32_t i = threadIdx.x; i < g.NB1; i += S3_THREADS) flush(i);
}

__global__ __launch_bounds__(S3_THREADS) void k3_scan_small(const uint32_t* __restrict__ cnt, uint32_t n, uint32_t* __restrict__ off,
                                                           uint32_t* __restrict__ cur, int prio) {
    s3_setprio(prio);
    __shared__ uint32_t wave_tot[4];
    uint32_t v[8], sum = 0;
    const uint32_t b0 = threadIdx.x * 8u;
#pragma unroll
    for (int k = 0; k < 8; ++k) {
        v[k] = b0 + k < n ? cnt[b0 + k] : 0u;
        sum += v[k];
    }
    uint32_t total;
    uint32_t run = s3_block_excl_scan(sum, wave_tot, &total);
#pragma unroll
    for (int k = 0; k < 8; ++k) {
        if (b0 + k < n) {
            off[b0 + k] = run;
            cur[b0 + k] = run;
        }
        run += v[k];
    }
    if (threadIdx.x == 0) off[n] = total;
}

template <class Geom, int NW>
__global__ __launch_bounds__(S3_THREADS, 4) void k3_l1_scatter(const uint32_t* __restrict__ scalars, uint32_t npts, Geom g,
                                                              uint32_t* __restrict__ cur1, uint32_t* __restrict__ o_idx,
                                                              uint16_t* __restrict__ o_rem) {
    s3_setprio(g.prio);
    extern __shared__ __attribute__((aligned(16))) uint32_t sh[];
    uint32_t* sc = sh;
    uint2* stage = reinterpret_cast<uint2*>(sh + NW * S3_PB);
    uint32_t* hist = sh + (NW + 2) * S3_PB;
    uint32_t* lstart = hist + 256;
    uint32_t* gbase = lstart + 256;
    __shared__ uint32_t wave_tot[4];
    const uint32_t tid = threadIdx.x;
    const uint32_t base = blockIdx.x * (uint32_t)S3_PB;
#pragma unroll
    for (int u = 0; u < S3_T; ++u) {
        const uint32_t p = base + u * S3_THREADS + tid;
        const uint32_t i = u * S3_THREADS + tid;
        if constexpr (NW == 8) {
            uint4 a = make_uint4(0, 0, 0, 0), b = make_uint4(0, 0, 0, 0);
            if (p < npts) {
                const uint4* q = reinterpret_cast<const uint4*>(scalars) + 2 * (size_t)p;
                a = q[0];
                b = q[1];
            }
            sc[0 * S3_PB + i] = a.x; sc[1 * S3_PB + i] = a.y; sc[2 * S3_PB + i] = a.z; sc[3 * S3_PB + i] = a.w;
            sc[4 * S3_PB + i] = b.x; sc[5 * S3_PB + i] = b.y; sc[6 * S3_PB + i] = b.z; sc[7 * S3_PB + i] = b.w;
        } else if constexpr (NW == 2) {
            uint2 a = make_uint2(0, 0);
            if (p < npts) a = reinterpret_cast<const uint2*>(scalars)[p];
            sc[0 * S3_PB + i] = a.x; sc[1 * S3_PB + i] = a.y;
        } else {
            sc[i] = p < npts ? scalars[p] : 0u;
        }
    }
    uint32_t carry = 0;
    using Win = typename Geom::Win;
    for (Win w = 0; w < (Win)g.W; ++w) {
        uint32_t cw, off, nb;
        if constexpr (Geom::TABLE) { cw = (uint32_t)g.c; off = w * cw; nb = g.NB1; }
        else { cw = g.width[w]; off = g.bitoff[w]; nb = (uint32_t)g.binoff1[w + 1] - (uint32_t)g.binoff1[w]; }
        const uint32_t sh1 = g.shift1(), lowmask = (1u << sh1) - 1u;
        const uint32_t j = off >> 5, shb = off & 31u, mask = (1u << cw) - 1u, half = 1u << (cw - 1);
        if (Geom::TABLE || tid < nb) hist[tid] = 0;
        __syncthreads();
        uint32_t key[S3_T], rk[S3_T];
#pragma unroll
        for (int u = 0; u < S3_T; ++u) {
            const uint32_t i = u * S3_THREADS + tid;
            const uint32_t lo = j < (uint32_t)NW ? sc[j * S3_PB + i] : 0u;
            const uint32_t hi = j + 1 < (uint32_t)NW ? sc[(j + 1) * S3_PB + i] : 0u;
            const uint32_t raw = (shb ? __builtin_amdgcn_alignbit(hi, lo, shb) : lo) & mask;
            const uint32_t v = raw + ((carry >> u) & 1u);
            int d;
            if (v > half) { d = (int)v - (int)(half << 1); carry |= 1u << u; }
            else { d = (int)v; carry &= ~(1u << u); }
            rk[u] = ~0u;
            key[u] = 0;
            if (d != 0 && base + i < npts) {
                const uint32_t b = (uint32_t)(d < 0 ? -d : d) - 1u;
                const uint32_t bin = b >> sh1;
                key[u] = (b & lowmask) | (bin << sh1) | (d < 0 ? 0x80000000u : 0u);
                rk[u] = atomicAdd(&hist[bin], 1u);
            }
        }
        __syncthreads();
        {
            const uint32_t v = tid < nb ? hist[tid] : 0u;
            uint32_t total;
            const uint32_t excl = s3_block_excl_scan(v, wave_tot, &total);
            if (tid < nb) {
                lstart[tid] = excl;
                uint32_t ci;
                if constexpr (Geom::TABLE) ci = tid; else ci = (uint32_t)g.binoff1[w] + tid;
                gbase[tid] = v ? atomicAdd(&cur1[ci], v) : 0u;
            }
            __syncthreads();
#pragma unroll
            for (int u = 0; u < S3_T; ++u) {
                if (rk[u] != ~0u) {
                    const uint32_t bin = (key[u] >> sh1) & (Geom::TABLE ? 0xffu : 0x1ffu);
                    const uint32_t p = base + u * S3_THREADS + tid;
                    const uint32_t rem = key[u] & lowmask;
                    stage[lstart[bin] + rk[u]] = make_uint2((Geom::TABLE ? g.index1(p, (uint32_t)w, rem) : p) | (key[u] & 0x80000000u), g.rem1(rem) | (bin << 16));
                }
            }
            __syncthreads();
            for (uint32_t slot = tid; slot < total; slot += S3_THREADS) {
                const uint2 e = stage[slot];
                const uint32_t bin = e.y >> 16;
                const uint32_t dst = gbase[bin] + (slot - lstart[bin]);
                o_idx[dst] = e.x;
                o_rem[dst] = (uint16_t)e.y;
            }
        }
        __syncthreads();
    }
}

__global__ __launch_bounds__(S3_THREADS) void k3_slice_map(const uint32_t* __restrict__ off, uint32_t nbins, uint32_t slice,
                                                          uint2* __restrict__ map, uint32_t* __restrict__ nitems, int prio) {
    s3_setprio(prio);
    __shared__ uint32_t wave_tot[4];
    __shared__ uint32_t carry_sh;
    if (threadIdx.x == 0) carry_sh = 0;
    __syncthreads();
    for (uint32_t base = 0; base < nbins; base += S3_THREADS) {
        const uint32_t i = base + threadIdx.x;
        const uint32_t size = i < nbins ? off[i + 1] - off[i] : 0u;
        const uint32_t v = (size + slice - 1) / slice;
        uint32_t total;
        const uint32_t excl = s3_block_excl_scan(v, wave_tot, &total);
        const uint32_t first = carry_sh + excl;
        for (uint32_t q = 0; q < v; ++q) map[first + q] = make_uint2(i, q);
        __syncthreads();
        if (threadIdx.x == 0) carry_sh += total;
        __syncthreads();
    }
    if (threadIdx.x == 0) *nitems = carry_sh;
}

__global__ __launch_bounds__(S3_THREADS) void k3_scan_a(const uint32_t* __restrict__ cnt, uint32_t n, uint32_t* __restrict__ bsum, int prio) {
    s3_setprio(prio);
    __shared__ uint32_t wave_tot[4];
    const uint32_t b0 = blockIdx.x * 2048u + threadIdx.x * 8u;
    uint32_t sum = 0;
#pragma unroll
    for (int k = 0; k < 8; ++k) sum += b0 + k < n ? cnt[b0 + k] : 0u;
    uint32_t total;
    (void)s3_block_excl_scan(sum, wave_tot, &total);
    if (threadIdx.x == 0) bsum[blockIdx.x] = total;
}
__global__ __launch_bounds__(S3_THREADS) void k3_scan_b(uint32_t* __restrict__ bsum, uint32_t nblocks, int prio) {
    s3_setprio(prio);
    __shared__ uint32_t wave_tot[4];
    const uint32_t v = threadIdx.x < nblocks ? bsum[threadIdx.x] : 0u;
    uint32_t total;
    const uint32_t excl = s3_block_excl_scan(v, wave_tot, &total);
    if (threadIdx.x < nblocks) bsum[threadIdx.x] = excl;
    if (threadIdx.x == 0) bsum[256] = total;
}
__global__ __launch_bounds__(S3_THREADS) void k3_scan_c(const uint32_t* __restrict__ cnt, uint32_t n, const uint32_t* __restrict__ bsum,
                                                       uint32_t* __restrict__ off, uint32_t* __restrict__ cur, int prio) {
    s3_setprio(prio);
    __shared__ uint32_t wave_tot[4];
    const uint32_t b0 = blockIdx.x * 2048u + threadIdx.x * 8u;
    uint32_t v[8], sum = 0;
#pragma unroll
    for (int k = 0; k < 8; ++k) {
        v[k] = b0 + k < n ? cnt[b0 + k] : 0u;
        sum += v[k];
    }
    uint32_t total;
    uint32_t run = bsum[blockIdx.x] + s3_block_excl_scan(sum, wave_tot, &total);
#pragma unroll
    for (int k = 0; k < 8; ++k) {
        if (b0 + k < n) {
            off[b0 + k] = run;
            cur[b0 + k] = run;
        }
        run += v[k];
    }
    if (blockIdx.x == 0 && threadIdx.x == 0) off[n] = bsum[256];
}

__device__ __forceinline__ bool s3_item(const uint32_t* off1, const uint2* map, const uint32_t* nitems, uint32_t id, uint32_t slice,
                                        uint32_t& k, uint32_t& lo, uint32_t& hi) {
    if (id >= *nitems) return false;
    const uint2 m = map[id];
    k = m.x;
    const uint32_t a = off1[k], b = off1[k + 1];
    lo = a + m.y * slice;
    hi = lo + slice < b ? lo + slice : b;
    return lo < hi;
}

template <class Geom>
__global__ __launch_bounds__(S3_THREADS, 4) void k3_l2_count(const uint16_t* __restrict__ rem, const uint32_t* __restrict__ off1,
                                                            const uint2* __restrict__ map, const uint32_t* __restrict__ nitems,
                                                            uint32_t* __restrict__ cnt2, Geom g) {
    s3_setprio(g.prio);
    __shared__ uint32_t hist[Geom::TAB2];
    uint32_t k, lo, hi;
    if (!s3_item(off1, map, nitems, blockIdx.x, S3_SLICE2, k, lo, hi)) return;
    if (Geom::TAB2 == S3_THREADS || threadIdx.x < Geom::TAB2) hist[threadIdx.x] = 0;
    __syncthreads();
    const uint32_t sh = g.shift2();
    uint32_t r[S3_T2];
#pragma unroll
    for (int t = 0; t < S3_T2; ++t) {
        const uint32_t i = lo + t * S3_THREADS + threadIdx.x;
        r[t] = i < hi ? rem[i] : 0xffffffffu;
    }
#pragma unroll
    for (int t = 0; t < S3_T2; ++t)
        if (r[t] != 0xffffffffu) atomicAdd(&hist[r[t] >> sh], 1u);
    __syncthreads();
    if (threadIdx.x < (1u << g.bits2())) {
        const uint32_t v = hist[threadIdx.x];
        if (v) atomicAdd(&cnt2[(k << g.bits2()) + threadIdx.x], v);
    }
}

template <class Geom>
__global__ __launch_bounds__(S3_THREADS, 4) void k3_l2_scatter(const uint32_t* __restrict__ i_idx, const uint16_t* __restrict__ i_rem,
                                                              const uint32_t* __restrict__ off1, const uint2* __restrict__ map,
                                                              const uint32_t* __restrict__ nitems, uint32_t* __restrict__ cur2,
                                                              uint32_t* __restrict__ o_idx, typename Geom::Lo* __restrict__ o_lo, Geom g) {
    s3_setprio(g.prio);
    constexpr uint32_t TAB2 = Geom::TAB2, KY_D = Geom::KY_D, KY_R = Geom::KY_R;
    __shared__ uint2 stage[S3_SLICE2];
    __shared__ uint32_t hist[TAB2], lstart[TAB2], gbase[TAB2];
    __shared__ uint32_t wave_tot[4];
    uint32_t k, lo, hi;
    if (!s3_item(off1, map, nitems, blockIdx.x, S3_SLICE2, k, lo, hi)) return;
    const uint32_t tid = threadIdx.x;
    if (TAB2 == S3_THREADS || tid < TAB2) hist[tid] = 0;
    __syncthreads();
    const uint32_t sh = g.shift2(), nb2 = 1u << g.bits2();
    uint32_t ex[S3_T2], ky[S3_T2];
#pragma unroll
    for (int t = 0; t < S3_T2; ++t) {
        const uint32_t i = lo + t * S3_THREADS + tid;
        ky[t] = 0xffffffffu;
        ex[t] = 0;
        if (i < hi) {
            const uint32_t r = i_rem[i];
            const uint32_t iw = i_idx[i];
            const uint32_t h2 = r >> sh;
            const uint32_t low = g.low2(r, iw);
            ex[t] = g.index2(iw);
            const uint32_t rank = atomicAdd(&hist[h2], 1u);
            ky[t] = low | (h2 << KY_D) | (rank << KY_R);
        }
    }
    __syncthreads();
    const uint32_t v = tid < nb2 ? hist[tid] : 0u;
    uint32_t total;
    const uint32_t excl = s3_block_excl_scan(v, wave_tot, &total);
    if (tid < nb2) {
        lstart[tid] = excl;
        gbase[tid] = v ? atomicAdd(&cur2[(k << g.bits2()) + tid], v) : 0u;
    }
    __syncthreads();
#pragma unroll
    for (int t = 0; t < S3_T2; ++t) {
        if (ky[t] != 0xffffffffu) {
            const uint32_t h2 = (ky[t] >> KY_D) & (TAB2 - 1u);
            stage[lstart[h2] + (ky[t] >> KY_R)] = make_uint2(ex[t], ky[t] & ((TAB2 << KY_D) - 1u));
        }
    }
    __syncthreads();
    for (uint32_t slot = tid; slot < total; slot += S3_THREADS) {
        const uint2 e = stage[slot];
        const uint32_t h2 = (e.y >> KY_D) & (TAB2 - 1u);
        const uint32_t dst = gbase[h2] + (slot - lstart[h2]);
        o_idx[dst] = e.x;
        o_lo[dst] = (typename Geom::Lo)(e.y & Geom::LO_MASK);
    }
}

__global__ __launch_bounds__(S3_THREADS, 4) void k3_l3(const uint32_t* __restrict__ i_idx, const uint8_t* __restrict__ i_lo,
                                                      const uint32_t* __restrict__ off2, uint32_t* __restrict__ count,
                                                      uint32_t* __restrict__ entries, int prio) {
    s3_setprio(prio);
    __shared__ uint32_t out[S3_R3];
    __shared__ uint32_t hist[128], cursor[128];
    __shared__ uint32_t wave_tot[4];
    const uint32_t j = blockIdx.x, tid = threadIdx.x;
    const uint32_t a = off2[j], b = off2[j + 1], s = b - a;
    if (tid < 128) hist[tid] = 0;
    __syncthreads();
    if (s <= S3_R3) {
        uint32_t ex[S3_T3], ky[S3_T3];
#pragma unroll
        for (int t = 0; t < S3_T3; ++t) {
            const uint32_t i = a + t * S3_THREADS + tid;
            ky[t] = 0xffffffffu;
            ex[t] = 0;
            if (i < b) {
                ky[t] = i_lo[i];
                ex[t] = i_idx[i];
            }
        }
#pragma unroll
        for (int t = 0; t < S3_T3; ++t)
            if (ky[t] != 0xffffffffu) ky[t] |= atomicAdd(&hist[ky[t]], 1u) << 8;
        __syncthreads();
        const uint32_t v = tid < 128 ? hist[tid] : 0u;
        uint32_t total;
        const uint32_t excl = s3_block_excl_scan(v, wave_tot, &total);
        if (tid < 128) {
            count[((size_t)j << 7) + tid] = v;
            cursor[tid] = excl;
        }
        __syncthreads();
#pragma unroll
        for (int t = 0; t < S3_T3; ++t)
            if (ky[t] != 0xffffffffu) out[cursor[ky[t] & 127u] + (ky[t] >> 8)] = ex[t];
        __syncthreads();
        for (uint32_t t = tid; t < s; t += S3_THREADS) entries[a + t] = out[t];
    } else {
        for (uint32_t i = a + tid; i < b; i += S3_THREADS) atomicAdd(&hist[i_lo[i]], 1u);
        __syncthreads();
        const uint32_t v = tid < 128 ? hist[tid] : 0u;
        uint32_t total;
        const uint32_t excl = s3_block_excl_scan(v, wave_tot, &total);
        if (tid < 128) {
            count[((size_t)j << 7) + tid] = v;
            cursor[tid] = excl;
        }
        constexpr int TB = S3_T3 / 2;
        constexpr uint32_t RB = S3_THREADS * TB;
        __shared__ uint32_t chist[128], cstart[128];
        __shared__ uint8_t cbkt[RB];
        for (uint32_t c0 = a; c0 < b; c0 += RB) {
            const uint32_t c1 = c0 + RB < b ? c0 + RB : b;
            if (tid < 128) chist[tid] = 0;
            __syncthreads();
            uint32_t ex[TB], ky[TB];
#pragma unroll
            for (int t = 0; t < TB; ++t) {
                const uint32_t i = c0 + t * S3_THREADS + tid;
                ky[t] = 0xffffffffu;
                ex[t] = 0;
                if (i < c1) {
                    ky[t] = i_lo[i];
                    ex[t] = i_idx[i];
                }
            }
#pragma unroll
            for (int t = 0; t < TB; ++t)
                if (ky[t] != 0xffffffffu) ky[t] |= atomicAdd(&chist[ky[t]], 1u) << 8;
            __syncthreads();
            const uint32_t cv = tid < 128 ? chist[tid] : 0u;
            uint32_t ctotal;
            const uint32_t cexcl = s3_block_excl_scan(cv, wave_tot, &ctotal);
            if (tid < 128) cstart[tid] = cexcl;
            __syncthreads();
#pragma unroll
            for (int t = 0; t < TB; ++t)
                if (ky[t] != 0xffffffffu) {
                    const uint32_t slot = cstart[ky[t] & 127u] + (ky[t] >> 8);
                    out[slot] = ex[t];
                    cbkt[slot] = (uint8_t)(ky[t] & 127u);
                }
            __syncthreads();
            for (uint32_t slot = tid; slot < ctotal; slot += S3_THREADS) {
                const uint32_t bk = cbkt[slot];
                entries[a + cursor[bk] + (slot - cstart[bk])] = out[slot];
            }
            __syncthreads();
            if (tid < 128) cursor[tid] += chist[tid];
            __syncthreads();
        }
    }
}

template <bool REGS>
__global__ __launch_bounds__(S3_THREADS, 4) void k3t_l3(const uint32_t* __restrict__ i_idx, const uint16_t* __restrict__ i_lo,
                                                       const uint32_t* __restrict__ off2, uint32_t* __restrict__ count,
                                                       uint32_t* __restrict__ entries, S3TGeom g, uint32_t img) {
    s3_setprio(g.prio);
    extern __shared__ __attribute__((aligned(16))) uint32_t out[];
    __shared__ uint32_t hist[1024], cursor[1024];
    __shared__ uint32_t wave_tot[4];
    const uint32_t j = blockIdx.x, tid = threadIdx.x;
    const uint32_t a = off2[j], b = off2[j + 1], s = b - a;
    const uint32_t nb3 = 1u << g.b3;
#pragma unroll
    for (int q = 0; q < 4; ++q) hist[q * S3_THREADS + tid] = 0;
    __syncthreads();
    auto scan_counts = [&]() {
        uint32_t v[4], sum = 0;
#pragma unroll
        for (int q = 0; q < 4; ++q) {
            const uint32_t t = tid * 4u + q;
            v[q] = t < nb3 ? hist[t] : 0u;
            sum += v[q];
        }
        uint32_t total;
        uint32_t run = s3_block_excl_scan(sum, wave_tot, &total);
#pragma unroll
        for (int q = 0; q < 4; ++q) {
            const uint32_t t = tid * 4u + q;
            if (t < nb3) {
                count[((size_t)j << g.b3) + t] = v[q];
                cursor[t] = run;
            }
            run += v[q];
        }
    };
    if (REGS && s <= S3_R3 && s <= img) {
        uint32_t ex[S3_T3], ky[S3_T3];
#pragma unroll
        for (int t = 0; t < S3_T3; ++t) {
            const uint32_t i = a + t * S3_THREADS + tid;
            ky[t] = 0xffffffffu;
            ex[t] = 0;
            if (i < b) {
                ky[t] = i_lo[i];
                ex[t] = i_idx[i];
            }
        }
#pragma unroll
        for (int t = 0; t < S3_T3; ++t)
            if (ky[t] != 0xffffffffu) ky[t] |= atomicAdd(&hist[ky[t]], 1u) << 10;
        __syncthreads();
        scan_counts();
        __syncthreads();
#pragma unroll
        for (int t = 0; t < S3_T3; ++t)
            if (ky[t] != 0xffffffffu) out[cursor[ky[t] & 1023u] + (ky[t] >> 10)] = ex[t];
        __syncthreads();
        for (uint32_t t = tid; t < s; t += S3_THREADS) entries[a + t] = out[t];
        return;
    }
    for (uint32_t i = a + tid; i < b; i += S3_THREADS) atomicAdd(&hist[i_lo[i]], 1u);
    __syncthreads();
    scan_counts();
    __syncthreads();
    if (s <= img) {
        for (uint32_t i = a + tid; i < b; i += S3_THREADS) out[atomicAdd(&cursor[i_lo[i]], 1u)] = i_idx[i];
        __syncthreads();
        for (uint32_t t = tid; t < s; t += S3_THREADS) entries[a + t] = out[t];
    } else {
        for (uint32_t i = a + tid; i < b; i += S3_THREADS) entries[a + atomicAdd(&cursor[i_lo[i]], 1u)] = i_idx[i];
    }
}

static S3Geom s3_geometry(const MsmPlan& P) {
    S3Geom g;
    g.W = P.W;
    g.prio = exp_knob("BLAZE_SORT_PRIO", 3);
    g.NB1 = (uint32_t)(P.G >> S3_SH1);
    uint32_t bit = 0;
    for (int w = 0; w < P.W; ++w) {
        g.width[w] = P.width[w];
        g.bitoff[w] = (uint16_t)bit;
        g.binoff1[w] = (uint16_t)(P.boff[w] >> S3_SH1);
        bit += P.width[w];
    }
    g.binoff1[P.W] = (uint16_t)(P.boff[P.W] >> S3_SH1);
    return g;
}

static S3TGeom s3t_geometry(const MsmPlan& P, uint32_t npts) {
    S3TGeom g;
    g.W = P.W;
    g.c = P.c;
    g.prio = exp_knob("BLAZE_SORT_PRIO", 3);
    g.sh1 = (uint32_t)(P.c - 1 - 8);
    g.NB1 = (uint32_t)(P.G >> g.sh1);
    const double per_bucket = (double)npts * P.W / (double)P.G;
    int b3 = 4;
    while (b3 < 10 && (double)(2u << b3) * per_bucket <= 6144.0) ++b3;
    if ((uint32_t)b3 > g.sh1) b3 = (int)g.sh1;
    int b2 = (int)g.sh1 - b3;
    if (b2 > 8) { b2 = 8; b3 = (int)g.sh1 - 8; }
    g.b2 = (uint32_t)b2;
    g.b3 = (uint32_t)b3;
    g.xs = g.sh1 > 16 ? g.sh1 - 16 : 0;
    return g;
}

bool msm_sort3_ok(const MsmPlan& P, int sbits) {
    if (P.table) {
        if (sbits != 256 || P.sbits < 1 || P.sbits > 256 || P.c < 16 || P.c > 26 || P.W * P.c < P.sbits + 1) return false;
        if ((uint64_t)P.npts * P.W >= (1ull << 30)) return false;
        const S3TGeom g = s3t_geometry(P, P.npts);
        return g.NB1 <= 256 && g.b2 <= 8 && g.b3 >= 1 && g.b3 <= 10 && g.xs <= 1 && g.b3 > g.xs;
    }
    if ((sbits != 256 && sbits != 64 && sbits != 32) || P.W < 1) return false;
    for (int w = 0; w < P.W; ++w)
        if (P.width[w] < S3_SH1 + 1 || P.width[w] > 23) return false;
    if ((P.G >> S3_SH1) > S3_MAXNB1 || (P.G & ((1u << S3_SH1) - 1u))) return false;
    if ((P.G >> S3_SH2) > 2048u * 256u) return false;
    return true;
}

static constexpr size_t s3_lds1(int nw) { return (size_t)((nw + 2) * S3_PB + 3 * 256) * 4; }
struct S3Need { int vgprs, lds; };
static S3Need s3_needs(bool table) {
    using L2 = S3Geom::L2;
    struct K { const void* f; size_t dyn; };
    static const K plain_ks[] = {{(const void*)k3_l1_count<S3Geom, 8>, 0}, {(const void*)k3_l1_scatter<S3Geom, 8>, s3_lds1(8)},
                                 {(const void*)k3_l1_count<S3Geom, 1>, 0}, {(const void*)k3_l1_scatter<S3Geom, 1>, s3_lds1(1)},
                                 {(const void*)k3_l1_count<S3Geom, 2>, 0}, {(const void*)k3_l1_scatter<S3Geom, 2>, s3_lds1(2)},
                                 {(const void*)k3_l2_count<L2>, 0}, {(const void*)k3_l2_scatter<L2>, 0}, {(const void*)k3_l3, 0}};
    static const K table_ks[] = {{(const void*)k3_l1_count<S3TGeom, 8>, 0}, {(const void*)k3_l1_scatter<S3TGeom, 8>, s3_lds1(8)},
                                 {(const void*)k3_l2_count<S3TGeom>, 0}, {(const void*)k3_l2_scatter<S3TGeom>, 0},
                                 {(const void*)k3t_l3<true>, (size_t)S3_R3 * 4}, {(const void*)k3t_l3<false>, (size_t)S3T_IMG * 4}};
    static S3Need cached[2] = {{-1, -1}, {-1, -1}};
    S3Need& c = cached[table ? 1 : 0];
    if (c.vgprs >= 0) return c;
    const K* ks = table ? table_ks : plain_ks;
    const size_t n = table ? sizeof(table_ks) / sizeof(*table_ks) : sizeof(plain_ks) / sizeof(*plain_ks);
    S3Need mx = {0, 0};
    for (size_t i = 0; i < n; ++i) {
        hipFuncAttributes a;
        if (hipFuncGetAttributes(&a, ks[i].f) != hipSuccess) {
            (void)hipGetLastError();
            return c = S3Need{0, 0};
        }
        if (a.numRegs > mx.vgprs) mx.vgprs = a.numRegs;
        const int lds = (int)(a.sharedSizeBytes + ks[i].dyn);
        if (lds > mx.lds) mx.lds = lds;
    }
    return c = mx;
}
int msm_sort3_max_vgprs(bool table) { return s3_needs(table).vgprs; }
int msm_sort3_max_lds(bool table) { return s3_needs(table).lds; }

template <class Geom, int NW>
static int s3_level1(hipStream_t st, const uint32_t* sc, uint32_t npts, const Geom& g, uint32_t* cnt1, uint32_t* off1, uint32_t* cur1,
                     uint32_t* i1_idx, uint16_t* i1_rem) {
    const dim3 blk(S3_THREADS);
    const size_t lds1 = s3_lds1(NW);
    hipLaunchKernelGGL((k3_l1_count<Geom, NW>), dim3((npts + S3_CNT_PTS - 1) / S3_CNT_PTS), blk, 0, st, sc, npts, g, cnt1);
    hipLaunchKernelGGL(k3_scan_small, dim3(1), blk, 0, st, cnt1, g.NB1, off1, cur1, g.prio);
    BLZ_TRY(ensure_dynamic_lds((const void*)k3_l1_scatter<Geom, NW>, (int)lds1));
    hipLaunchKernelGGL((k3_l1_scatter<Geom, NW>), dim3((npts + S3_PB - 1) / S3_PB), blk, lds1, st, sc, npts, g, cur1, i1_idx, i1_rem);
    return BLZ_OK;
}

template <class Geom>
static int s3_enqueue(MsmEngine& E, const MsmStep& C, const Geom& g, const void* d_scalars, uint32_t npts, int sbits) {
    using L2 = typename Geom::L2;
    using Lo = typename L2::Lo;
    const MsmPlan& P = C.P;
    hipStream_t st = C.sort_stream;
    MsmEngine::SortBufs& B = C.B;
    const uint32_t NB1 = g.NB1, NB2 = (uint32_t)(P.G >> g.bits3());
    const uint64_t max_entries = (uint64_t)npts * P.W;
    const uint32_t max_items = (uint32_t)(max_entries / S3_SLICE2) + NB1 + 1;
    const uint32_t nsb = (NB2 + 2047u) / 2048u;
    if (Geom::TABLE && nsb > 256) return fail(BLZ_ERR_UNKNOWN, "window-table sort: %u final-level bins exceed the scan's range", NB2);
    const size_t tab_dw = (size_t)3 * (NB1 + 2) + (size_t)3 * (NB2 + 2) + 260 + 4 + 2 * ((size_t)max_items + 2);
    BLZ_TRY(E.sort3_tabs.reserve(tab_dw * 4));
    uint32_t* cnt1 = E.sort3_tabs.as<uint32_t>();
    uint32_t* off1 = cnt1 + NB1 + 2;
    uint32_t* cur1 = off1 + NB1 + 2;
    uint32_t* cnt2 = cur1 + NB1 + 2;
    uint32_t* off2 = cnt2 + NB2 + 2;
    uint32_t* cur2 = off2 + NB2 + 2;
    uint32_t* bsum = cur2 + NB2 + 2;
    uint32_t* nitems = bsum + 260;
    uint2* map = reinterpret_cast<uint2*>(nitems + 4);
    BLZ_TRY(E.inter.reserve(max_entries * 6 + 64));
    BLZ_TRY(E.inter2.reserve(max_entries * (4 + sizeof(Lo)) + 64));
    uint32_t* i1_idx = E.inter.as<uint32_t>();
    uint16_t* i1_rem = reinterpret_cast<uint16_t*>(i1_idx + max_entries);
    uint32_t* i2_idx = E.inter2.as<uint32_t>();
    Lo* i2_lo = reinterpret_cast<Lo*>(i2_idx + max_entries);
    uint32_t* count = B.count.as<uint32_t>();
    uint32_t* entries = B.entries.as<uint32_t>();
    const uint32_t* sc = (const uint32_t*)d_scalars;
    const dim3 blk(S3_THREADS);
    const L2 g2 = g.l2();

    BLZ_HIP(hipMemsetAsync(cnt1, 0, (size_t)(NB1 + 2) * 4, st), BLZ_ERR_UNKNOWN);
    BLZ_HIP(hipMemsetAsync(cnt2, 0, (size_t)(NB2 + 2) * 4, st), BLZ_ERR_UNKNOWN);
    if constexpr (Geom::TABLE) {
        BLZ_TRY((s3_level1<Geom, 8>(st, sc, npts, g, cnt1, off1, cur1, i1_idx, i1_rem)));
    } else {
        BLZ_SW_DISPATCH(sbits, BLZ_TRY((s3_level1<Geom, SW>(st, sc, npts, g, cnt1, off1, cur1, i1_idx, i1_rem))));
    }
    hipLaunchKernelGGL(k3_slice_map, dim3(1), blk, 0, st, off1, NB1, S3_SLICE2, map, nitems, g.prio);
    hipLaunchKernelGGL(k3_l2_count<L2>, dim3(max_items), blk, 0, st, i1_rem, off1, map, nitems, cnt2, g2);
    hipLaunchKernelGGL(k3_scan_a, dim3(nsb), blk, 0, st, cnt2, NB2, bsum, g.prio);
    hipLaunchKernelGGL(k3_scan_b, dim3(1), blk, 0, st, bsum, nsb, g.prio);
    hipLaunchKernelGGL(k3_scan_c, dim3(nsb), blk, 0, st, cnt2, NB2, bsum, off2, cur2, g.prio);
    hipLaunchKernelGGL(k3_l2_scatter<L2>, dim3(max_items), blk, 0, st, i1_idx, i1_rem, off1, map, nitems, cur2, i2_idx, i2_lo, g2);
    if constexpr (Geom::TABLE) {
        const double mean_bin = (double)max_entries / (double)(NB2 ? NB2 : 1);
        const bool big_bins = mean_bin * 1.1 > (double)S3_R3;
        const uint32_t img = big_bins ? S3T_IMG : S3_R3;
        auto l3 = big_bins ? k3t_l3<false> : k3t_l3<true>;
        BLZ_TRY(ensure_dynamic_lds((const void*)l3, (int)(img * 4)));
        hipLaunchKernelGGL(l3, dim3(NB2), blk, (size_t)img * 4, st, i2_idx, i2_lo, off2, count, entries, g, img);
    } else {
        hipLaunchKernelGGL(k3_l3, dim3(NB2), blk, 0, st, i2_idx, i2_lo, off2, count, entries, g.prio);
    }
    BLZ_HIP(hipGetLastError(), BLZ_ERR_UNKNOWN);
    return BLZ_OK;
}

int msm_sort3(MsmEngine& E, const MsmStep& C, const void* d_scalars, uint32_t npts, int sbits) {
    const MsmPlan& P = C.P;
    return P.table ? s3_enqueue(E, C, s3t_geometry(P, P.npts), d_scalars, npts, sbits) : s3_enqueue(E, C, s3_geometry(P), d_scalars, npts, sbits);
}

}
```

### blaze_amd/csrc/msm_sort_stage.hip

```cpp
#include "msm_sort.hpp"

namespace blz {

SortPlan plan_sort(const MsmPlan& P, uint32_t npts, int sbits, int pieces, const SortInputs& in) {
    const bool on = in.hide_env != 0, guarded = in.hide_env == 1;
    if (P.table)
        return {SortPlan::S3, on && in.other_busy && (!guarded || in.fits) ? SortPlan::HIDDEN : SortPlan::OPEN};
    const bool s3_ok = on && msm_sort3_ok(P, sbits);
    if (pieces > 1) return s3_ok && !in.other_busy && !in.recent_hot && in.fits ? SortPlan{SortPlan::S3, SortPlan::PINGPONG} : SortPlan{SortPlan::LDS, SortPlan::OPEN};
    const bool s3 = s3_ok && (!guarded || (!in.recent_hot && in.fits));
    if (s3 && in.other_busy) return {SortPlan::S3, SortPlan::HIDDEN};
    if (s3 && in.hide_env == 2) return {SortPlan::S3, SortPlan::OPEN};
    return {msm_sort_tiny_ok(P, npts, sbits) ? SortPlan::TINY : SortPlan::LDS, SortPlan::OPEN};
}

std::string describe(const SortPlan& s) {
    static const char* const kind[] = {"lds", "s3", "tiny"};
    static const char* const where[] = {"open", "hidden", "pingpong"};
    return std::string(kind[s.kind]) + " " + where[s.where];
}

bool msm_sort_fits_beside(int av, int sv, int al, int sl) {
    if (av <= 0 || sv <= 0) return true;
    const int a = (av + 7) & ~7, s = (sv + 7) & ~7;
    int waves = 512 / a;
    if (waves > 4) waves = 4;
    if (waves < 1) waves = 1;
    if (waves * a + s > 512 - 32) return false;
    if (al <= 0 || sl <= 0) return true;
    const int ak = (al + 1023) >> 10, sk = (sl + 1023) >> 10;
    return 2 * waves * ak + sk <= 160;
}

__global__ __launch_bounds__(256) void k_zero(uint4* __restrict__ p, size_t n16) {
    __builtin_amdgcn_s_setprio(3);
    const uint4 z = make_uint4(0, 0, 0, 0);
    for (size_t i = (size_t)blockIdx.x * 256 + threadIdx.x; i < n16; i += (size_t)gridDim.x * 256) p[i] = z;
}
void launch_zero(void* p, size_t n16, hipStream_t st) { hipLaunchKernelGGL(k_zero, dim3(2048), dim3(256), 0, st, (uint4*)p, n16); }

__global__ __launch_bounds__(256) void k_extract_range(const uint32_t* __restrict__ src, uint32_t* __restrict__ dst, uint64_t n, uint32_t w0,
                                                       uint32_t nw) {
    __builtin_amdgcn_s_setprio(3);
    const uint64_t total = n * 8;
    for (uint64_t i = (uint64_t)blockIdx.x * 256 + threadIdx.x; i < total; i += (uint64_t)gridDim.x * 256) {
        const uint32_t j = (uint32_t)(i & 7u);
        dst[i] = j < nw ? src[(i & ~(uint64_t)7) + w0 + j] : 0u;
    }
}

constexpr int SCAN_ITEMS = 8;
static_assert(SCAN_TILE == 256 * SCAN_ITEMS, "a scan block of 256 lanes takes SCAN_ITEMS buckets per lane");

__device__ __forceinline__ uint64_t pack_cu(uint32_t cnt, uint32_t L) {
    return (uint64_t)cnt | ((uint64_t)((cnt + L - 1) / L) << 32);
}
__device__ __forceinline__ uint64_t block_sum_u64(uint64_t v, uint64_t* sh) {
    for (int o = 32; o > 0; o >>= 1) v += __shfl_down(v, o, 64);
    int lane = threadIdx.x & 63, wv = threadIdx.x >> 6;
    if (lane == 0) sh[wv] = v;
    __syncthreads();
    uint64_t t = sh[0] + sh[1] + sh[2] + sh[3];
    __syncthreads();
    return t;
}

__global__ __launch_bounds__(256) void k_scan_reduce(const uint32_t* __restrict__ count, uint64_t G, uint32_t L,
                                                     uint64_t* __restrict__ blocksums, uint32_t* __restrict__ stats) {
    __builtin_amdgcn_s_setprio(3);
    __shared__ uint64_t sh[4];
    uint64_t base = (uint64_t)blockIdx.x * SCAN_TILE;
    uint64_t acc = 0;
    uint32_t mx = 0;
#pragma unroll
    for (int k = 0; k < SCAN_ITEMS; ++k) {
        uint64_t i = base + (uint64_t)k * 256 + threadIdx.x;
        if (i < G) {
            uint32_t cn = count[i];
            acc += pack_cu(cn, L);
            mx = cn > mx ? cn : mx;
        }
    }
    uint64_t tot = block_sum_u64(acc, sh);
    for (int o = 32; o > 0; o >>= 1) { uint32_t t = __shfl_down(mx, o, 64); mx = t > mx ? t : mx; }
    if ((threadIdx.x & 63) == 0 && mx > *(volatile uint32_t*)&stats[1]) atomicMax(&stats[1], mx);
    if (threadIdx.x == 0) blocksums[blockIdx.x] = tot;
}

constexpr int SCAN_SUMS_THREADS = 256;
__global__ __launch_bounds__(SCAN_SUMS_THREADS) void k_scan_sums(uint64_t* __restrict__ blocksums, uint32_t nblocks,
                                                                 uint32_t* __restrict__ stats) {
    __builtin_amdgcn_s_setprio(3);
    __shared__ uint64_t sh[SCAN_SUMS_THREADS];
    __shared__ uint64_t carry_sh;
    if (threadIdx.x == 0) carry_sh = 0;
    __syncthreads();
    for (uint32_t base = 0; base < nblocks; base += SCAN_SUMS_THREADS) {
        uint32_t i = base + threadIdx.x;
        uint64_t v = i < nblocks ? blocksums[i] : 0;
        sh[threadIdx.x] = v;
        __syncthreads();
        for (int o = 1; o < SCAN_SUMS_THREADS; o <<= 1) {
            uint64_t t = threadIdx.x >= (uint32_t)o ? sh[threadIdx.x - o] : 0;
            __syncthreads();
            sh[threadIdx.x] += t;
            __syncthreads();
        }
        uint64_t incl = sh[threadIdx.x];
        uint64_t carry = carry_sh;
        if (i < nblocks) blocksums[i] = carry + incl - v;
        __syncthreads();
        if (threadIdx.x == SCAN_SUMS_THREADS - 1) carry_sh = carry + incl;
        __syncthreads();
    }
    if (threadIdx.x == 0) {
        stats[0] = (uint32_t)(carry_sh >> 32);
        stats[2] = (uint32_t)(carry_sh & 0xffffffffu);
    }
}

__global__ __launch_bounds__(256) void k_scan_final(uint32_t* __restrict__ count, uint64_t G, uint32_t L,
                                                    const uint64_t* __restrict__ blocksums,
                                                    uint32_t* __restrict__ off, uint32_t* __restrict__ unit_off) {
    __builtin_amdgcn_s_setprio(3);
    __shared__ uint64_t sh[256];
    uint64_t base = (uint64_t)blockIdx.x * SCAN_TILE + (uint64_t)threadIdx.x * SCAN_ITEMS;
    uint64_t v[SCAN_ITEMS];
    uint64_t tsum = 0;
#pragma unroll
    for (int k = 0; k < SCAN_ITEMS; ++k) {
        uint64_t i = base + k;
        v[k] = i < G ? pack_cu(count[i], L) : 0;
        tsum += v[k];
    }
    sh[threadIdx.x] = tsum;
    __syncthreads();
    for (int o = 1; o < 256; o <<= 1) {
        uint64_t t = threadIdx.x >= (uint32_t)o ? sh[threadIdx.x - o] : 0;
        __syncthreads();
        sh[threadIdx.x] += t;
        __syncthreads();
    }
    uint64_t run = blocksums[blockIdx.x] + sh[threadIdx.x] - tsum;
#pragma unroll
    for (int k = 0; k < SCAN_ITEMS; ++k) {
        uint64_t i = base + k;
        if (i <= G) {
            off[i] = (uint32_t)(run & 0xffffffffu);
            unit_off[i] = (uint32_t)(run >> 32);
            if (i < G) count[i] = (uint32_t)(run & 0xffffffffu);
        }
        run += v[k];
    }
}

constexpr uint32_t UNITS_INLINE = 8;

constexpr uint32_t UNIT_GRID = 2048;

__global__ __launch_bounds__(256) void k_fill_units(const uint32_t* __restrict__ off, const uint32_t* __restrict__ unit_off,
                                                    uint64_t G, uint32_t L, uint32_t* __restrict__ unit_bucket,
                                                    uint32_t* __restrict__ hist) {
    __builtin_amdgcn_s_setprio(3);
    __shared__ uint32_t sh[MAX_L + 1];
    __shared__ uint32_t big[256], nbig;
    for (uint32_t i = threadIdx.x; i <= L; i += 256) sh[i] = 0;
    const uint64_t nchunks = (G + 255) / 256;
    for (uint64_t chunk = blockIdx.x; chunk < nchunks; chunk += gridDim.x) {
        if (threadIdx.x == 0) nbig = 0;
        __syncthreads();
        const uint64_t g0 = chunk * 256;
        uint64_t g = g0 + threadIdx.x;
        if (g < G) {
            uint32_t u0 = unit_off[g], u1 = unit_off[g + 1];
            uint32_t cnt = off[g + 1] - off[g];
            uint32_t nfull = cnt / L, rem = cnt - nfull * L;
            if (nfull) atomicAdd(&sh[L], nfull);
            if (rem) atomicAdd(&sh[rem], 1u);
            if (u1 - u0 > UNITS_INLINE) big[atomicAdd(&nbig, 1u)] = threadIdx.x;
            else for (uint32_t u = u0; u < u1; ++u) unit_bucket[u] = (uint32_t)g;
        }
        __syncthreads();
        for (uint32_t b = 0; b < nbig; ++b) {
            uint64_t gb = g0 + big[b];
            uint32_t u0 = unit_off[gb], u1 = unit_off[gb + 1];
            for (uint32_t u = u0 + threadIdx.x; u < u1; u += 256) unit_bucket[u] = (uint32_t)gb;
        }
        __syncthreads();
    }
    for (uint32_t i = threadIdx.x; i <= L; i += 256)
        if (sh[i]) atomicAdd(&hist[i], sh[i]);
}

__global__ __launch_bounds__(256) void k_unit_len_scan(const uint32_t* __restrict__ hist, uint32_t L,
                                                       uint32_t* __restrict__ cursor) {
    __builtin_amdgcn_s_setprio(3);
    if (threadIdx.x != 0) return;
    uint32_t run = 0;
    for (int len = (int)L; len >= 0; --len) {
        cursor[len] = run;
        run += hist[len];
    }
}

__global__ __launch_bounds__(256) void k_unit_order(const uint32_t* __restrict__ off, const uint32_t* __restrict__ unit_off,
                                                    uint64_t G, uint32_t L, uint32_t* __restrict__ cursor,
                                                    uint32_t* __restrict__ unit_order) {
    __builtin_amdgcn_s_setprio(3);
    __shared__ uint32_t sh_cnt[MAX_L + 1];
    __shared__ uint32_t sh_base[MAX_L + 1];
    __shared__ uint32_t big[256], big_pos[256], nbig;
    for (uint32_t i = threadIdx.x; i <= L; i += 256) sh_cnt[i] = 0;
    __syncthreads();
    const uint64_t nchunks = (G + 255) / 256;
    for (uint64_t chunk = blockIdx.x; chunk < nchunks; chunk += gridDim.x) {
        uint64_t g = chunk * 256 + threadIdx.x;
        if (g < G) {
            uint32_t cnt = off[g + 1] - off[g];
            uint32_t nfull = cnt / L, rem = cnt - nfull * L;
            if (nfull) atomicAdd(&sh_cnt[L], nfull);
            if (rem) atomicAdd(&sh_cnt[rem], 1u);
        }
    }
    __syncthreads();
    for (uint32_t i = threadIdx.x; i <= L; i += 256) {
        uint32_t v = sh_cnt[i];
        sh_base[i] = v ? atomicAdd(&cursor[i], v) : 0u;
        sh_cnt[i] = 0;
    }
    for (uint64_t chunk = blockIdx.x; chunk < nchunks; chunk += gridDim.x) {
        if (threadIdx.x == 0) nbig = 0;
        __syncthreads();
        const uint64_t g0 = chunk * 256;
        uint64_t g = g0 + threadIdx.x;
        if (g < G) {
            uint32_t u0 = unit_off[g];
            uint32_t cnt = off[g + 1] - off[g];
            uint32_t nfull = cnt / L, rem = cnt - nfull * L;
            if (nfull) {
                uint32_t pos = sh_base[L] + atomicAdd(&sh_cnt[L], nfull);
                if (nfull > UNITS_INLINE) {
                    uint32_t q = atomicAdd(&nbig, 1u);
                    big[q] = threadIdx.x;
                    big_pos[q] = pos;
                } else {
                    for (uint32_t k = 0; k < nfull; ++k) unit_order[pos + k] = u0 + k;
                }
            }
            if (rem) unit_order[sh_base[rem] + atomicAdd(&sh_cnt[rem], 1u)] = u0 + nfull;
        }
        __syncthreads();
        for (uint32_t b = 0; b < nbig; ++b) {
            uint64_t gb = g0 + big[b];
            uint32_t ub = unit_off[gb];
            uint32_t nf = (off[gb + 1] - off[gb]) / L, pos = big_pos[b];
            for (uint32_t k = threadIdx.x; k < nf; k += 256) unit_order[pos + k] = ub + k;
        }
        __syncthreads();
    }
}

int launch_fill_units(const MsmStep& C, uint32_t U ) {
    const uint64_t G = C.P.G;
    const uint32_t L = C.P.L;
    hipStream_t st = C.sort_stream;
    MsmEngine::SortBufs& B = C.B;
    BLZ_TRY(B.unit_bucket.reserve(((size_t)U + 1) * 4));
    BLZ_TRY(B.unit_order.reserve(((size_t)U + 1) * 4));
    BLZ_TRY(B.lenhist.reserve(2 * (MAX_L + 1) * 4));
    uint32_t* hist = B.lenhist.as<uint32_t>();
    uint32_t* cursor = hist + (MAX_L + 1);
    BLZ_HIP(hipMemsetAsync(hist, 0, 2 * (MAX_L + 1) * 4, st), BLZ_ERR_UNKNOWN);
    uint64_t nchunks = (G + 255) / 256;
    dim3 gg((uint32_t)(nchunks < UNIT_GRID ? nchunks : UNIT_GRID)), b(256);
    hipLaunchKernelGGL(k_fill_units, gg, b, 0, st, B.off.as<uint32_t>(), B.unit_off.as<uint32_t>(), G, L, B.unit_bucket.as<uint32_t>(), hist);
    hipLaunchKernelGGL(k_unit_len_scan, dim3(1), b, 0, st, hist, L, cursor);
    hipLaunchKernelGGL(k_unit_order, gg, b, 0, st, B.off.as<uint32_t>(), B.unit_off.as<uint32_t>(), G, L, cursor, B.unit_order.as<uint32_t>());
    BLZ_HIP(hipGetLastError(), BLZ_ERR_UNKNOWN);
    return BLZ_OK;
}

static void launch_scans(MsmEngine& E, const MsmStep& C) {
    const uint64_t G = C.P.G;
    const uint32_t nscan = (uint32_t)((G + 1 + SCAN_TILE - 1) / SCAN_TILE);
    MsmEngine::SortBufs& B = C.B;
    hipStream_t ss = C.sort_stream;
    dim3 b256(256);
    hipLaunchKernelGGL(k_scan_reduce, dim3(nscan), b256, 0, ss, B.count.as<uint32_t>(), G, C.P.L, E.blocksums.as<uint64_t>(),
                       B.stats.as<uint32_t>());
    hipLaunchKernelGGL(k_scan_sums, dim3(1), dim3(SCAN_SUMS_THREADS), 0, ss, E.blocksums.as<uint64_t>(), nscan, B.stats.as<uint32_t>());
    hipLaunchKernelGGL(k_scan_final, dim3(nscan), b256, 0, ss, B.count.as<uint32_t>(), G, C.P.L, E.blocksums.as<uint64_t>(),
                       B.off.as<uint32_t>(), B.unit_off.as<uint32_t>());
}

int msm_sort_stage(MsmEngine& E, const MsmStep& C, const void* d_scalars, uint32_t np) {
    MsmSlot& S = C.S;
    MsmEngine::SortBufs& B = C.B;
    hipStream_t ss = C.sort_stream;
    const char* sc_s = (const char*)d_scalars;
    if (S.ranged) {
        BLZ_TRY(B.range_scalars.reserve((size_t)np * 32 + 16));
        hipLaunchKernelGGL(k_extract_range, dim3(2048), dim3(256), 0, ss, (const uint32_t*)sc_s, B.range_scalars.as<uint32_t>(),
                           (uint64_t)np, (uint32_t)(S.bit_lo >> 5), (uint32_t)((S.bit_hi - S.bit_lo) >> 5));
        sc_s = (const char*)B.range_scalars.p;
    }
    BLZ_HIP(hipMemsetAsync(B.stats.p, 0, 64, ss), BLZ_ERR_UNKNOWN);
    auto stats_to_host = [&]() -> int {
        BLZ_HIP(hipGetLastError(), BLZ_ERR_UNKNOWN);
        return copy_words_to_pinned(S.stats_h, B.stats.p, 4, ss);
    };
    switch (S.sort.kind) {
        case SortPlan::TINY:
            BLZ_TRY(msm_sort_tiny(E, C, sc_s, np, S.sbits, (uint32_t)S.max_units));
            BLZ_TRY(stats_to_host());
            break;
        case SortPlan::S3:
            BLZ_TRY(msm_sort3(E, C, sc_s, np, S.sbits));
            launch_scans(E, C);
            BLZ_TRY(stats_to_host());
            BLZ_TRY(launch_fill_units(C, (uint32_t)S.max_units));
            break;
        case SortPlan::LDS: {
// ... 15 lines not shown
```

### blaze_amd/csrc/testhooks.hip

```cpp
#include "common.hpp"
#include "ec_rr.hip.hpp"
#include "ec_row.hip.hpp"
#include "ec_law.hip.hpp"
#include "poseidon_engine.hpp"
#include "poseidon_impl.hip.hpp"
#include "msm_engine.hpp"
#include "../../include/blaze_hip_aux.h"

namespace blz {

template <class P>
__global__ __launch_bounds__(64) void k_test_field(int op, const uint32_t* a, const uint32_t* b, uint32_t* out, uint32_t n) {
    uint32_t i = blockIdx.x * 64u + threadIdx.x;
    if (i >= n) return;
    Fp<P> x, y, r;
    fp_load(x, a + (size_t)i * P::N);
    fp_load(y, b + (size_t)i * P::N);
    fp_to_mont(x, x);
    fp_to_mont(y, y);
    switch (op) {
        case 0: fp_mul(r, x, y); break;
        case 1: fp_add(r, x, y); break;
        case 2: fp_sub(r, x, y); break;
        case 3: fp_inv(r, x); break;
        case 5:
        case 6:
            if constexpr (P::LAZY) {
                Fp<P> s, d;
                fp_add(s, x, y);
                fp_sub(d, x, y);
                if (op == 5) fp_mul2(r, x, y, s, d);
                else fp_mulsub2(r, x, y, s, d);
            } else {
                fp_zero(r);
            }
            break;
        case 10: case 11: case 12: case 13: case 14: case 15:
            if constexpr (USE_RR<P>) {
                using Q = typename P::RR;
                fp_load(x, a + (size_t)i * P::N);
                fp_load(y, b + (size_t)i * P::N);
                Frr<Q, 1, 2> xr, yr, rr;
                rr_to_mont_from_words<Q>(xr, x.v);
                rr_to_mont_from_words<Q>(yr, y.v);
                if (op == 10) rr_mul(rr, xr, yr);
                else if (op == 11) rr_sqr(rr, xr);
                else if (op == 12) rr_mul2(rr, xr, yr, rr_norm(rr_add(xr, yr)), rr_sub<2>(xr, yr));
                else if (op == 13) rr_mul(rr, rr_norm(rr_sub_twice<2>(rr_sub<2>(xr, yr), yr)), yr);
                else if (op == 15) {
                    const auto t = rr_reduce2m(rr_sub_twice<2>(rr_sub<2>(xr, yr), yr));
                    rr_mul(rr, t, xr);
                }
                else {
                    const auto d = rr_sub<2>(xr, yr);
                    const bool eq = rr_maybe_equal(xr, yr) && rr_is_zero(d);
                    if (rr_is_zero(d) != eq) { rr_zero(rr); rr.v[0] = 7; }
                    else if (eq) rr_one(rr);
                    else rr_zero(rr);
                }
                rr_to_mont32_words<Q>(r.v, rr);
            } else {
                fp_zero(r);
            }
            break;
        default: fp_sqr(r, x); break;
    }
    fp_from_mont(r, r);
    fp_store(out + (size_t)i * P::N, r);
}

template <class F>
__global__ __launch_bounds__(64) void k_test_ec(int op, const uint32_t* p, const uint32_t* q, const uint8_t* inf_flags,
                                                uint32_t* out, uint8_t* out_inf, uint32_t n) {
    uint32_t i = blockIdx.x * 64u + threadIdx.x;
    if (i >= n) return;
    Affine<F> P, Q;
    fp_load(P.x, p + (size_t)i * 2 * F::N);
    fp_load(P.y, p + (size_t)i * 2 * F::N + F::N);
    fp_load(Q.x, q + (size_t)i * 2 * F::N);
    fp_load(Q.y, q + (size_t)i * 2 * F::N + F::N);
    fp_to_mont(P.x, P.x); fp_to_mont(P.y, P.y); fp_to_mont(Q.x, Q.x); fp_to_mont(Q.y, Q.y);
    uint8_t fl = inf_flags[i];
    XYZZ<F> acc, qq;
    if (fl & 1) pt_set_inf(acc); else pt_from_affine(acc, P);
    if (fl & 2) pt_set_inf(qq); else pt_from_affine(qq, Q);
    if (!(fl & 1)) {
        Fp<F> z, z2, z3;
        z = P.x; fp_add(z, z, Q.y);
        if (fp_is_zero(z)) fp_one(z);
        fp_sqr(z2, z); fp_mul(z3, z2, z);
        fp_mul(acc.x, acc.x, z2); fp_mul(acc.y, acc.y, z3); acc.zz = z2; acc.zzz = z3;
    }
    switch (op) {
        case 0: if (!(fl & 2)) pt_madd(acc, Q); break;
        case 1: { XYZZ<F> d; pt_dbl(d, acc); acc = d; } break;
        case 2: {
            if (!(fl & 2)) {
                Fp<F> z, z2, z3;
                z = Q.x; fp_add(z, z, P.y);
                if (fp_is_zero(z)) fp_one(z);
                fp_sqr(z2, z); fp_mul(z3, z2, z);
                fp_mul(qq.x, qq.x, z2); fp_mul(qq.y, qq.y, z3); qq.zz = z2; qq.zzz = z3;
            }
            pt_add(acc, qq);
        } break;
        case 4: case 5:
            if constexpr (USE_RR<F>) {
                if (!(fl & 2)) {
                    using QQ = typename F::RR;
                    XYZZRR<QQ> a;
                    ptrr_from_xyzz32<F>(a, acc);
                    AffineRR<QQ> q;
                    rr_from_mont32_words<QQ>(q.x, Q.x.v);
                    rr_from_mont32_words<QQ>(q.y, Q.y.v);
                    ptrr_madd<QQ, 2>(a, q, op == 5);
                    ptrr_madd<QQ, 2>(a, q, op == 5);
                    ptrr_madd<QQ, 2>(a, q, op != 5);
                    ptrr_to_xyzz32<F>(acc, a);
                }
            } else {
                pt_set_inf(acc);
            }
            break;
        case 8: case 9:
            if constexpr (USE_RR<F>) {
                using QQ = typename F::RR;
                if (op == 8 && !(fl & 2)) {
                    Fp<F> z, z2, z3;
                    z = Q.x; fp_add(z, z, P.y);
                    if (fp_is_zero(z)) fp_one(z);
                    fp_sqr(z2, z); fp_mul(z3, z2, z);
                    fp_mul(qq.x, qq.x, z2); fp_mul(qq.y, qq.y, z3); qq.zz = z2; qq.zzz = z3;
                }
                XYZZRR<QQ> a, b;
                ptrr_from_xyzz32<F>(a, acc);
                ptrr_from_xyzz32<F>(b, qq);
                if (op == 8) ptrr_add<QQ, 2>(a, b);
                else a = ptrr_dbl_val<QQ, 2>(a);
                ptrr_to_xyzz32<F>(acc, a);
            } else {
                pt_set_inf(acc);
            }
            break;
        case 6: case 7:
            if constexpr (USE_RR<F>) {
                using QQ = typename F::RR;
                AffineRR<QQ> p, q;
                rr_from_mont32_words<QQ>(p.x, P.x.v);
                rr_from_mont32_words<QQ>(p.y, P.y.v);
                rr_from_mont32_words<QQ>(q.x, Q.x.v);
                rr_from_mont32_words<QQ>(q.y, Q.y.v);
                XYZZRR<QQ> a;
                ptrr_set_inf(a);
                if (fl == 0) ptrr_aadd<QQ, 2>(a, p, op == 7, q, false);
                else if (fl == 1) ptrr_madd<QQ, 2>(a, q, false);
                else if (fl == 2) ptrr_madd<QQ, 2>(a, p, op == 7);
                ptrr_to_xyzz32<F>(acc, a);
            } else {
                pt_set_inf(acc);
            }
            break;
        default: if (!(fl & 2)) { fp_neg(Q.y, Q.y); pt_madd(acc, Q); } break;
    }
    Affine<F> r;
    bool fin = pt_to_affine(r, acc);
    Fp<F> x, y;
    if (fin) { fp_from_mont(x, r.x); fp_from_mont(y, r.y); } else { fp_zero(x); fp_zero(y); }
    fp_store(out + (size_t)i * 2 * F::N, x);
    fp_store(out + (size_t)i * 2 * F::N + F::N, y);
    out_inf[i] = fin ? 0 : 1;
}

struct Tmp {
    std::vector<void*> ptrs;
    ~Tmp() { for (void* p : ptrs) (void)hipFree(p); }
    int alloc(void** p, size_t n) {
        BLZ_HIP(hipMalloc(p, n ? n : 16), BLZ_ERR_UNKNOWN);
        ptrs.push_back(*p);
        return BLZ_OK;
    }
};

template <class P>
__global__ __launch_bounds__(64) void k_test_row(int op, const uint32_t* a, const uint32_t* b, uint32_t* out, uint32_t n) {
    if constexpr (USE_RR<P>) {
        using Q = typename P::RR;
        if constexpr (!RR_TIGHT<Q> && Q::B == 28) {
            __shared__ uint32_t sh[2][4][16];
            const RowCtx<Q> c = row_ctx<Q>();
            const uint32_t e = op == 23 ? blockIdx.x : blockIdx.x * 4u + c.row;
            const uint32_t ee = e < n ? e : n - 1;
            Fp<P> x, y;
            fp_load(x, a + (size_t)ee * P::N);
            fp_load(y, b + (size_t)ee * P::N);
            uint32_t xl = 0, yl = 0;
            if (op == 24) {
                const uint32_t bits = (x.v[c.li % P::N] >> (3u * (c.li / P::N))) ^ (y.v[(c.li * 5u) % P::N] >> 7);
                const uint32_t pat[8] = {0u, 1u, Q::MASK, Q::MASK - 1u, 1u << 28, (1u << 28) + 3u, 15u * (1u << 28) + Q::MASK, (7u << 28) + 1u};
                xl = c.li < (uint32_t)Q::NL ? pat[bits & 7u] : 0u;
                if (c.li == (uint32_t)Q::NL - 1u) xl &= 0xffffu;
            } else {
                Frr<Q, 1, 2> xr, yr;
                rr_to_mont_from_words<Q>(xr, x.v);
                rr_to_mont_from_words<Q>(yr, y.v);
                if ((threadIdx.x & 15u) == 0u) {
#pragma unroll
                    for (int i = 0; i < Q::NL; ++i) { sh[0][c.row][i] = xr.v[i]; sh[1][c.row][i] = yr.v[i]; }
                    sh[0][c.row][14] = sh[0][c.row][15] = sh[1][c.row][14] = sh[1][c.row][15] = 0u;
                }
                __syncthreads();
                xl = sh[0][c.row][c.li];
                yl = sh[1][c.row][c.li];
                __syncthreads();
            }
            uint32_t r = 0;
            if (op == 20) r = row_mul<Q>(c, xl, yl);
            else if (op == 21) r = row_mul<Q>(c, row_norm<Q>(c, xl + (c.km2 - yl) + 2u * (c.km2 - yl)), yl);
            else if (op == 22) {
                r = row_mul<Q>(c, xl + (c.km5 - yl), xl + yl);
            } else if (op == 23) {
                const uint32_t d = row_norm<Q>(c, xl + (c.km2 - yl));
                const bool z = row_is_zero<Q>(c, d);
                const bool eq = row_maybe_equal<Q>(c, d) && z;
                r = z != eq ? (c.li == 0u ? 7u : 0u) : eq ? c.one : 0u;
            } else if (op == 24) {
                r = row_resolve<Q>(c, row_norm<Q>(c, xl));
            }
            if (op != 24) r = row_resolve<Q>(c, r);
            sh[0][c.row][c.li] = r;
            sh[1][c.row][c.li] = xl;
            __syncthreads();
            if (c.li == 0u && e < n && (op != 23 || c.row == 0u)) {
                Fp<P> o;
                if (op == 24) {
                    uint64_t carry = 0;
                    bool same = true;
                    for (int i = 0; i < Q::NL; ++i) {
                        const uint64_t t = (uint64_t)sh[1][c.row][i] + carry;
                        const uint32_t want = i + 1 < Q::NL ? (uint32_t)t & Q::MASK : (uint32_t)t;
                        carry = i + 1 < Q::NL ? t >> Q::B : 0;
                        same = same && want == sh[0][c.row][i];
                    }
                    fp_zero(o);
                    o.v[0] = same ? 1u : 0u;
                    fp_store(out + (size_t)e * P::N, o);
                } else {
                    Frr<Q, 1, 2> rr;
#pragma unroll
                    for (int i = 0; i < Q::NL; ++i) rr.v[i] = sh[0][c.row][i];
                    rr_to_mont32_words<Q>(o.v, rr);
                    fp_from_mont(o, o);
                    fp_store(out + (size_t)e * P::N, o);
                }
            }
        }
    }
}

template <class P>
int test_field_t(int op, const uint8_t* a, const uint8_t* b, uint8_t* out, size_t n) {
    Tmp tmp;
    size_t bytes = n * P::N * 4;
    void *da, *db, *dout;
    BLZ_TRY(tmp.alloc(&da, bytes)); BLZ_TRY(tmp.alloc(&db, bytes)); BLZ_TRY(tmp.alloc(&dout, bytes));
    BLZ_HIP(hipMemcpy(da, a, bytes, hipMemcpyHostToDevice), BLZ_ERR_WRITE);
    BLZ_HIP(hipMemcpy(db, b, bytes, hipMemcpyHostToDevice), BLZ_ERR_WRITE);
    if (op >= 20 && op <= 24) {
        BLZ_HIP(hipMemset(dout, 0, bytes), BLZ_ERR_UNKNOWN);
        hipLaunchKernelGGL(k_test_row<P>, dim3((unsigned)(op == 23 ? n : (n + 3) / 4)), dim3(64), 0, 0, op, (const uint32_t*)da, (const uint32_t*)db,
                           (uint32_t*)dout, (uint32_t)n);
    } else
        hipLaunchKernelGGL(k_test_field<P>, dim3((unsigned)((n + 63) / 64)), dim3(64), 0, 0, op, (const uint32_t*)da,
                           (const uint32_t*)db, (uint32_t*)dout, (uint32_t)n);
    BLZ_HIP(hipGetLastError(), BLZ_ERR_UNKNOWN);
    BLZ_HIP(hipMemcpy(out, dout, bytes, hipMemcpyDeviceToHost), BLZ_ERR_READ);
    return BLZ_OK;
}

template <class F>
int test_ec_t(int op, const uint8_t* p, const uint8_t* q, const uint8_t* fl, uint8_t* out, uint8_t* out_inf, size_t n) {
    Tmp tmp;
    size_t bytes = n * 2 * F::N * 4;
    void *dp, *dq, *dfl, *dout, *dinf;
    BLZ_TRY(tmp.alloc(&dp, bytes)); BLZ_TRY(tmp.alloc(&dq, bytes)); BLZ_TRY(tmp.alloc(&dfl, n));
    BLZ_TRY(tmp.alloc(&dout, bytes)); BLZ_TRY(tmp.alloc(&dinf, n));
    BLZ_HIP(hipMemcpy(dp, p, bytes, hipMemcpyHostToDevice), BLZ_ERR_WRITE);
    BLZ_HIP(hipMemcpy(dq, q, bytes, hipMemcpyHostToDevice), BLZ_ERR_WRITE);
    BLZ_HIP(hipMemcpy(dfl, fl, n, hipMemcpyHostToDevice), BLZ_ERR_WRITE);
    hipLaunchKernelGGL(k_test_ec<F>, dim3((unsigned)((n + 63) / 64)), dim3(64), 0, 0, op, (const uint32_t*)dp,
                       (const uint32_t*)dq, (const uint8_t*)dfl, (uint32_t*)dout, (uint8_t*)dinf, (uint32_t)n);
    BLZ_HIP(hipGetLastError(), BLZ_ERR_UNKNOWN);
    BLZ_HIP(hipMemcpy(out, dout, bytes, hipMemcpyDeviceToHost), BLZ_ERR_READ);
    BLZ_HIP(hipMemcpy(out_inf, dinf, n, hipMemcpyDeviceToHost), BLZ_ERR_READ);
    return BLZ_OK;
}


template <class P>
__global__ __launch_bounds__(64) void k_test_pos_mont(const uint32_t* words, uint32_t* out, uint32_t n) {
    const uint32_t i = blockIdx.x * 64u + threadIdx.x;
    if (i >= n) return;
    Fp<P> x;
    fp_load(x, words + (size_t)i * P::N);
    fp_to_mont(x, x);
    fp_store(out + (size_t)i * P::N, x);
}
template <class P>
BLZ_DEV void pos_def_load(Fp<P>& x, const uint32_t* p) {
    fp_load(x, p);
// ... 686 lines not shown
            uint32_t w[Q::N32], w32[Q::N32];
            rr_to_words<Q>(w, a);
            rr_to_mont32_words<Q>(w32, a);
            rr_put_words<Q::NL>(out, 0, w);
            rr_put_words<Q::NL>(out, 1, w32);
        } else {
            uint32_t w[Q::N32];
#pragma unroll
            for (int i = 0; i < Q::N32; ++i) w[i] = in[i];
            Frr<Q, 1, 2> r;
            if constexpr (VAR == 0) {
                Frr<Q, 1, VRAW> x;
                rr_from_words<Q>(x, w);
                rr_to_mont_from_words<Q>(r, w);
                rr_put(out, 0, x);
                rr_put(out, 1, r);
            } else {
                rr_from_mont32_words<Q>(r, w);
                rr_put(out, 0, r);
            }
        }
    }
};
template <class Q, int VAR, int VIN, bool U>
struct RrvDft8 {
    using RQ = Q;
    static constexpr int op = RR_DFT8, var = VAR, param = U ? 0 : 1;
    using A = Frr<Q, 1, VIN>;
    using W = std::conditional_t<U, RRShoupU<Q>, RRShoup<Q>>;
    using O = decltype(dft8_rr<Q>(std::declval<const A (&)[8]>(), std::declval<const W&>(), std::declval<const W&>(), std::declval<const W&>()));
    using In = cat_t<typename Rep<8, A>::type, typename Rep<3, Frr<Q, 1, 1>>::type>;
    using Out = typename OctTypes<O>::type;
    static BLZ_DEV void run(const uint32_t* in, uint32_t* out) {
        A a[8];
#pragma unroll
        for (int j = 0; j < 8; ++j) a[j] = rr_img<A>(in, j);
        RRShoup<Q> t[3];
#pragma unroll
        for (int j = 0; j < 3; ++j) rr_shoup_quot<Q>(t[j], rr_img<Frr<Q, 1, 1>>(in, 8 + j));
        if constexpr (U) {
            RRShoupU<Q> u[3];
#pragma unroll
            for (int j = 0; j < 3; ++j) rr_shoup_uniform<Q>(u[j], t[j]);
            auto o = dft8_rr<Q>(a, u[0], u[1], u[2]);
            BLZ_RR_FOR8(o, { rr_put(out, K, X); })
        } else {
            auto o = dft8_rr<Q>(a, t[0], t[1], t[2]);
            BLZ_RR_FOR8(o, { rr_put(out, K, X); })
        }
    }
};

template <class Q>
struct RrList {
    using L = RrLim<Q>;
    static constexpr bool SH = Q::NL == 9, TIGHT = RR_TIGHT<Q>;
    static constexpr int VX = XYZZRR<Q>::VX;
    static constexpr bool DFT = SH && !std::is_same_v<Q, Fq_BN254::RR>;
    using D2 = RrDftTypes<Q, 2>;
    using D1 = RrDftTypes<Q, L::VIN1>;
    using Mul = TL<RrvMul<Q, 0, L::F1, L::VMAX, 1, 1>, RrvMul<Q, 1, 1, 1, L::F1, L::VMAX>, RrvMul<Q, 2, L::FBA, L::VBA, L::FBB, L::VBB>,
                   RrvMul<Q, 100, 1, VX, 1, 2>>;
    using Sqr = TL<RrvSqr<Q, 0, L::FSQ, L::VBA>, std::conditional_t<TIGHT, RrvSqr<Q, 100, 1, 6>, RrvSqr<Q, 100, 3, 10>>>;
    using Mul2 = TL<RrvMul2<Q, 0, L::FM2A, L::VMAX / 2, 1, 1, L::FS - L::FM2A, 1, 1, L::VMAX / 2>,
                    RrvMul2<Q, 1, L::FM2, L::VHA, L::FM2, L::VHB, 1, L::VHB, L::FS - L::FM2 * L::FM2, L::VHA>,
                    std::conditional_t<TIGHT, RrvMul2<Q, 100, 3, 6, 1, 6, 2, 4, 1, 2>, RrvMul2<Q, 100, 3, 10, 3, 34, 2, 8, 1, 2>>>;
    using Pair = TL<RrvMulPair<Q, 0, L::F1, L::VMAX, 1, 1, L::FBA, L::VBA, L::FBB, L::VBB>, RrvSqrPair<Q, 1, L::FSQ, L::VBA, 1, 1>,
                    RrvMulPair<Q, 100, 1, 2, 1, 2, 2, 4, 1, 2>,
                    std::conditional_t<TIGHT, RrvSqrPair<Q, 101, 1, 6, 1, 6>, RrvSqrPair<Q, 101, 3, 34, 3, 10>>>;
    template <int... Ns>
    static auto dots(std::integer_sequence<int, Ns...>) -> TL<RrvDot<Q, Ns + 1, Ns + 1, 1, L::VMAX / (Ns + 1), 1, 1>...>;
    using Dot = cat_t<decltype(dots(std::make_integer_sequence<int, L::FS>{})),
                      only_if<SH, RrvDot<Q, 100, POS_DOT, 1, 7, 1, 1>>, only_if<SH, RrvDot<Q, 101, POS_DOT, 1, 3, 1, 1>>>;
    using Shoup = std::conditional_t<SH,
        TL<RrvShoup<Q, 0, 1, L::VMAX, false>, RrvShoup<Q, 1, L::F1, L::VMAX, false>, RrvShoup<Q, 100, 3, 6, false>, RrvShoup<Q, 101, 1, L::VIN1, false>,
           RrvShoup<Q, 0, 1, L::VMAX, true>, RrvShoup<Q, 1, L::F1, L::VMAX, true>, RrvShoup<Q, 100, 3, 6, true>, RrvShoup<Q, 101, 1, L::VIN1, true>,
           RrvShoupQuot<Q, 0>, RrvShoupQuot<Q, 1>>,
        TL<>>;
    using Lin = cat_t<TL<RrvNorm<Q, 0, L::FMAX, L::VMAX>, RrvNorm<Q, 100, 2, 4>, RrvReduce2m<Q, 0, Frr<Q, L::FMAX, L::VR2M>>,
                         RrvReduce2m<Q, 100, Frr<Q, 3, 6>>>,
                      only_if<SH, RrvReduce2m<Q, 101, typename D2::Q02s>>, only_if<SH, RrvReduce2m<Q, 102, typename D1::Q02s>>,
                      rr_sub_list_t<Q, RR_SUB>, rr_sub_list_t<Q, RR_SUB_TWICE>, rr_sub_list_t<Q, RR_NEG>, rr_sub_list_t<Q, RR_CNEG>>;
    using Bfly = cat_t<TL<RrvBfly<Q, 0, typename D2::A, typename D2::A>, RrvBfly<Q, 1, typename D2::Pd, typename D2::M>,
                          RrvBfly<Q, 2, typename D2::Ps, typename D2::Ps>, RrvBfly<Q, 3, typename D2::Q02s, typename D2::Q02s>,
                          RrvBfly<Q, 4, typename D2::Q13s, typename D2::M>, RrvBfly<Q, 5, typename D2::Q02d, typename D2::M>,
                          RrvBfly<Q, 6, Frr<Q, 1, 2>, Frr<Q, 2, 4>>>,
                       only_if<SH, RrvBfly<Q, 10, typename D1::A, typename D1::A>>, only_if<SH, RrvBfly<Q, 11, typename D1::Pd, typename D1::M>>,
                       only_if<SH, RrvBfly<Q, 12, typename D1::Ps, typename D1::Ps>>, only_if<SH, RrvBfly<Q, 13, typename D1::Q02s, typename D1::Q02s>>>;
    using Rest = cat_t<TL<RrvCanon<Q, 0>, RrvZero<Q, 0, L::F1, L::VMAX, L::F1, L::VMAX>, RrvZero<Q, 100, 3, 6, 1, 2>, RrvWords<Q, 0>, RrvWords<Q, 1>,
                          RrvWords<Q, 2>>,
                       only_if<DFT, RrvDft8<Q, 0, 2, true>>, only_if<DFT, RrvDft8<Q, 1, L::VIN1, true>>, only_if<DFT, RrvDft8<Q, 2, 2, false>>>;
    using type = cat_t<Mul, Sqr, Mul2, Pair, Dot, Shoup, Lin, Bfly, Rest>;
};

struct RrOp {
    int op, var;
    const uint32_t* in;
    uint32_t* out;
    size_t n;
};
template <class Vt>
__global__ __launch_bounds__(64) void k_test_rr(const uint32_t* in, uint32_t* out, uint32_t n) {
    constexpr uint32_t NL = Vt::RQ::NL;
    const uint32_t i = blockIdx.x * 64u + threadIdx.x;
    const uint32_t e = i < n ? i : n - 1u;
    Vt::run(in + (size_t)e * Vt::In::n * NL, out + (size_t)i * Vt::Out::n * NL);
}
template <class Vt>
int rr_run(const RrOp& o) {
    constexpr size_t NL = Vt::RQ::NL;
    const size_t waves = (o.n + 63) / 64, in_bytes = o.n * Vt::In::n * NL * 4, out_bytes = o.n * Vt::Out::n * NL * 4;
    Tmp tmp;
    void *din, *dout;
    BLZ_TRY(tmp.alloc(&din, in_bytes));
    BLZ_TRY(tmp.alloc(&dout, waves * 64 * Vt::Out::n * NL * 4));
    BLZ_HIP(hipMemcpy(din, o.in, in_bytes, hipMemcpyHostToDevice), BLZ_ERR_WRITE);
    BLZ_HIP(hipMemset(dout, 0, waves * 64 * Vt::Out::n * NL * 4), BLZ_ERR_UNKNOWN);
    hipLaunchKernelGGL(k_test_rr<Vt>, dim3((unsigned)waves), dim3(64), 0, 0, (const uint32_t*)din, (uint32_t*)dout, (uint32_t)o.n);
    BLZ_HIP(hipGetLastError(), BLZ_ERR_UNKNOWN);
    BLZ_TRY(sync_stream_bounded(nullptr, "reduced-radix primitive test kernel"));
    BLZ_HIP(hipMemcpy(o.out, dout, out_bytes, hipMemcpyDeviceToHost), BLZ_ERR_READ);
    return BLZ_OK;
}
template <class... T>
void rr_emit_bounds(std::vector<uint32_t>& w, TL<T...>) {
    ((w.push_back((uint32_t)rr_bounds<T>::f), w.push_back((uint32_t)rr_bounds<T>::v)), ...);
}
template <class Vt>
void rr_emit(std::vector<uint32_t>& w) {
    const uint32_t head[5] = {(uint32_t)Vt::op, (uint32_t)Vt::var, (uint32_t)Vt::In::n, (uint32_t)Vt::Out::n, (uint32_t)Vt::param};
    w.insert(w.end(), head, head + 5);
    rr_emit_bounds(w, typename Vt::In{});
    rr_emit_bounds(w, typename Vt::Out{});
}
template <class... Vs>
int rr_each(TL<Vs...>, std::vector<uint32_t>* lay, const RrOp* o) {
    int rc = -1;
    ([&] {
        if (lay) rr_emit<Vs>(*lay);
        if (o && Vs::op == o->op && Vs::var == o->var) rc = rr_run<Vs>(*o);
    }(), ...);
    if (!o) return BLZ_OK;
    return rc == -1 ? fail(BLZ_ERR_INVALID_PARAM, "the field has no variant %d of reduced-radix op %d", o->var, o->op) : rc;
}
template <class Q>
int test_rr_field(uint32_t* layout, const RrOp* o) {
    using L = RrLim<Q>;
    std::vector<uint32_t> rec;
    BLZ_TRY(rr_each(typename RrList<Q>::type{}, layout ? &rec : nullptr, o));
    if (layout) {
        constexpr size_t R0 = 16 + Q::NL;
        if (R0 + rec.size() > BLZ_RR_LAYOUT_WORDS) return fail(BLZ_ERR_UNKNOWN, "the layout needs %zu words", R0 + rec.size());
        memset(layout, 0, BLZ_RR_LAYOUT_WORDS * sizeof(uint32_t));
        const uint32_t head[11] = {(uint32_t)Q::B, (uint32_t)Q::NL, (uint32_t)L::H, (uint32_t)Q::NKM, (uint32_t)L::FS, (uint32_t)(Q::B * Q::NL),
                                   (uint32_t)Q::N32, (uint32_t)POS_DOT, Q::T2M, (uint32_t)RrList<Q>::type::n, (uint32_t)(R0 + rec.size())};
        memcpy(layout, head, sizeof(head));
        for (int i = 0; i < Q::NL; ++i) layout[16 + i] = Q::MOD[i];
        memcpy(layout + R0, rec.data(), rec.size() * sizeof(uint32_t));
    }
    return BLZ_OK;
}
static int test_rr_dispatch(int curve, int field, uint32_t* layout, const RrOp* o) {
    if (field == 0 || field == 1) {
        switch (curve) {
            case BLZ_BLS377: return field ? test_rr_field<Fr_BLS377::RR>(layout, o) : test_rr_field<Fq_BLS377::RR>(layout, o);
            case BLZ_BLS381: return field ? test_rr_field<Fr_BLS381::RR>(layout, o) : test_rr_field<Fq_BLS381::RR>(layout, o);
            case BLZ_BN254: return field ? test_rr_field<Fr_BN254::RR>(layout, o) : test_rr_field<Fq_BN254::RR>(layout, o);
        }
    }
    return fail(BLZ_ERR_INVALID_PARAM, "no reduced-radix field %d of curve %d", field, curve);
}

}

using namespace blz;

extern "C" {

int blz_test_field_op(int device_id, int curve, int field, int op, const uint8_t* a, const uint8_t* b, uint8_t* out, size_t n) {
    BLZ_TRY(use_device(device_id));
    if (n == 0) return BLZ_OK;
    if (field == 0) {
        switch (curve) {
            case BLZ_BLS377: return test_field_t<Fq_BLS377>(op, a, b, out, n);
            case BLZ_BLS381: return test_field_t<Fq_BLS381>(op, a, b, out, n);
            case BLZ_BN254: return test_field_t<Fq_BN254>(op, a, b, out, n);
        }
    } else {
        switch (curve) {
            case BLZ_BLS377: return test_field_t<Fr_BLS377>(op, a, b, out, n);
            case BLZ_BLS381: return test_field_t<Fr_BLS381>(op, a, b, out, n);
            case BLZ_BN254: return test_field_t<Fr_BN254>(op, a, b, out, n);
        }
    }
    return fail(BLZ_ERR_INVALID_PARAM, "unknown curve %d", curve);
}

int blz_test_ec_op(int device_id, int curve, int op, const uint8_t* p, const uint8_t* q, const uint8_t* inf_flags,
                   uint8_t* out, uint8_t* out_inf, size_t n) {
    BLZ_TRY(use_device(device_id));
    if (n == 0) return BLZ_OK;
    switch (curve) {
        case BLZ_BLS377: return test_ec_t<Fq_BLS377>(op, p, q, inf_flags, out, out_inf, n);
        case BLZ_BLS381: return test_ec_t<Fq_BLS381>(op, p, q, inf_flags, out, out_inf, n);
        case BLZ_BN254: return test_ec_t<Fq_BN254>(op, p, q, inf_flags, out, out_inf, n);
    }
    return fail(BLZ_ERR_INVALID_PARAM, "unknown curve %d", curve);
}

int blz_test_poseidon_permute(int device_id, int field, const uint8_t* words, size_t len, int t, const uint8_t* states_in, uint8_t* states_out, size_t n) {
    if (!words || !states_in || !states_out) return fail(BLZ_ERR_INVALID_PARAM, "null argument");
    if (t < 2 || t > 16) return fail(BLZ_ERR_INVALID_PARAM, "width %d out of range", t);
    PoseidonStream checked;
    BLZ_TRY(poseidon_parse(field, 1u << t, words, len, checked));
    PosDefBlock b;
    if (!pos_def_find(words, len, t, b)) return fail(BLZ_ERR_INVALID_PARAM, "the stream has no block of width %d", t);
    BLZ_TRY(use_device(device_id));
    if (n == 0) return BLZ_OK;
    switch (field) {
        case BLZ_BLS377: return test_pos_permute_t<Fr_BLS377>(words, b, states_in, states_out, n);
        case BLZ_BLS381: return test_pos_permute_t<Fr_BLS381>(words, b, states_in, states_out, n);
        case BLZ_BN254: return test_pos_permute_t<Fr_BN254>(words, b, states_in, states_out, n);
    }
    return fail(BLZ_ERR_INVALID_PARAM, "unknown field %d", field);
}

int blz_test_poseidon_hash(int device_id, int field, const uint8_t* words, size_t len, int t, const uint8_t* inputs, uint8_t* digests, size_t n) {
    if (!words || !inputs || !digests) return fail(BLZ_ERR_INVALID_PARAM, "null argument");
    if (t < 2 || t > 16) return fail(BLZ_ERR_INVALID_PARAM, "width %d out of range", t);
    BLZ_TRY(use_device(device_id));
    if (n == 0) return BLZ_OK;
    Tmp tmp;
    void *din, *dout;
    BLZ_TRY(tmp.alloc(&din, n * (size_t)(t - 1) * 32)); BLZ_TRY(tmp.alloc(&dout, n * 32));
    BLZ_HIP(hipMemcpy(din, inputs, n * (size_t)(t - 1) * 32, hipMemcpyHostToDevice), BLZ_ERR_WRITE);
    BLZ_TRY(poseidon_hash_batch(device_id, field, words, len, t, din, dout, n));
    BLZ_HIP(hipMemcpy(digests, dout, n * 32, hipMemcpyDeviceToHost), BLZ_ERR_READ);
    return BLZ_OK;
}

int blz_test_poseidon_hash_plan(int device_id, int field, const uint8_t* words, size_t len, int t, const uint8_t* inputs, uint8_t* digests, size_t n,
                                uint32_t* state) {
    if (!words || !inputs || !digests || !state) return fail(BLZ_ERR_INVALID_PARAM, "null argument");
    if (t < 2 || t > 16) return fail(BLZ_ERR_INVALID_PARAM, "width %d out of range", t);
    BLZ_TRY(use_device(device_id));
    *state = 0;
    Tmp tmp;
    void *din, *dout;
    BLZ_TRY(tmp.alloc(&din, (n ? n : 1) * (size_t)(t - 1) * 32)); BLZ_TRY(tmp.alloc(&dout, (n ? n : 1) * 32));
    BLZ_HIP(hipMemcpy(din, inputs, n * (size_t)(t - 1) * 32, hipMemcpyHostToDevice), BLZ_ERR_WRITE);
    BLZ_TRY(poseidon_hash_batch(device_id, field, words, len, t, din, dout, n, state));
    if (*state == HADES_OK) BLZ_HIP(hipMemcpy(digests, dout, n * 32, hipMemcpyDeviceToHost), BLZ_ERR_READ);
    return BLZ_OK;
}

int blz_test_poseidon_tree_check(int device_id, int field, const uint8_t* words, size_t len, int tree_mode, uint32_t tree_height, const void* d_input,
                                 const void* d_records, uint64_t out[2]) {
    if (!words || !d_input || !d_records || !out) return fail(BLZ_ERR_INVALID_PARAM, "null argument");
    if (tree_height < 1 || tree_height > 11) return fail(BLZ_ERR_INVALID_PARAM, "tree height out of range");
    BLZ_TRY(blz_poseidon_check_words(field, tree_mode, words, len, nullptr));
    BLZ_TRY(use_device(device_id));
    switch (field) {
        case BLZ_BLS377: return test_pos_tree_check_t<Fr_BLS377>(words, len, tree_mode, tree_height, d_input, d_records, out);
        case BLZ_BLS381: return test_pos_tree_check_t<Fr_BLS381>(words, len, tree_mode, tree_height, d_input, d_records, out);
        case BLZ_BN254: return test_pos_tree_check_t<Fr_BN254>(words, len, tree_mode, tree_height, d_input, d_records, out);
    }
    return fail(BLZ_ERR_INVALID_PARAM, "unknown field %d", field);
}

int blz_test_msm_tail_plan(int curve, int repr, uint32_t npts, int sbits, int pieces, int table_c, int bit_lo, int bit_hi, uint32_t plan_out[8],
                           uint8_t* widths, char* text, size_t cap) {
    if (!plan_out || !text || cap == 0) return fail(BLZ_ERR_INVALID_PARAM, "null argument");
    const MsmCurveOps* ops = msm_ops_for(curve, repr);
    if (!ops || npts == 0) return fail(BLZ_ERR_INVALID_PARAM, "unknown curve %d or empty task", curve);
    MsmPlan P;
    BLZ_TRY(msm_task_plan(curve, npts, sbits, table_c, bit_lo, bit_hi, P, nullptr));
    uint32_t per = 0;
    pieces = msm_task_pieces(P, pieces, false, &per);
    TailPlan T;
    BLZ_TRY(plan_tail(P, ops->tail, pieces > 1, T));
    const uint32_t out[8] = {(uint32_t)P.c, (uint32_t)P.W, (uint32_t)P.G, P.L, P.Bw, (uint32_t)P.Wv, (uint32_t)P.ebits, P.table ? 1u : 0u};
    memcpy(plan_out, out, sizeof(out));
    if (widths) memcpy(widths, P.width, (size_t)P.W);
    const std::string line = describe(T);
    if (line.size() >= cap) return fail(BLZ_ERR_INVALID_PARAM, "text buffer of %zu bytes for a line of %zu", cap, line.size());
    memcpy(text, line.c_str(), line.size() + 1);
    return BLZ_OK;
}

int blz_test_msm_sort_plan(int curve, int repr, uint32_t npts, int sbits, int pieces, int table_c, int bit_lo, int bit_hi, int hide_env, int other_busy,
                           int recent_hot, int fits, char* text, size_t cap) {
    if (!text || cap == 0) return fail(BLZ_ERR_INVALID_PARAM, "null argument");
    if (!msm_ops_for(curve, repr) || npts == 0) return fail(BLZ_ERR_INVALID_PARAM, "unknown curve %d or empty task", curve);
    MsmPlan P;
    BLZ_TRY(msm_task_plan(curve, npts, sbits, table_c, bit_lo, bit_hi, P, nullptr));
    uint32_t per = 0;
    pieces = msm_task_pieces(P, pieces, false, &per);
    const std::string line = describe(plan_sort(P, npts, sbits, pieces, SortInputs{hide_env, other_busy != 0, recent_hot != 0, fits != 0}));
    if (line.size() >= cap) return fail(BLZ_ERR_INVALID_PARAM, "text buffer of %zu bytes for a line of %zu", cap, line.size());
    memcpy(text, line.c_str(), line.size() + 1);
    return BLZ_OK;
}

int blz_test_law_layout(int curve, int repr, int law, uint32_t out[32]) {
    if (!out) return fail(BLZ_ERR_INVALID_PARAM, "null argument");
    LawLayout L;
    BLZ_TRY(test_law_dispatch(curve, repr, law, &L, nullptr));
    memset(out, 0, 32 * sizeof(uint32_t));
    const uint32_t head[6] = {L.B, L.NL, L.stride, L.e, L.lanes, L.closed};
    memcpy(out, head, sizeof(head));
    const LawBound* b[4] = {&L.in, &L.store, &L.strict, &L.to_lane};
    for (int i = 0; i < 4; ++i) memcpy(out + 6 + 5 * i, b[i], sizeof(LawBound));
    out[26] = L.tree ? 1u : 0u;
    return BLZ_OK;
}

int blz_test_law_op(int device_id, int curve, int repr, int law, int program, int exit, uint32_t k, uint32_t arg, const uint32_t* in, uint32_t* out,
                    size_t n) {
    if (!in || !out) return fail(BLZ_ERR_INVALID_PARAM, "null argument");
    LawLayout L;
    BLZ_TRY(test_law_dispatch(curve, repr, law, &L, nullptr));
    if (program < 0 || program >= LAW_PROGRAMS) return fail(BLZ_ERR_INVALID_PARAM, "unknown program %d", program);
    if (program == LAW_TREE) {
        if (!L.tree) return fail(BLZ_ERR_INVALID_PARAM, "the shuffle tree runs on the reduced-radix lane law only");
        if (k < 1 || k > 64 || arg < 1 || arg > k) return fail(BLZ_ERR_INVALID_PARAM, "tree of %u lanes over %u points", arg, k);
    } else {
        if (k != 4) return fail(BLZ_ERR_INVALID_PARAM, "program %d takes 4 points per case, not %u", program, k);
        if (arg > 64) return fail(BLZ_ERR_INVALID_PARAM, "%u doublings per step (at most 64)", arg);
    }
    const LawBound& ex = exit == 0 ? L.store : exit == 1 ? L.to_lane : L.strict;
    if (exit < 0 || exit > 2 || ex.limb_max == 0) return fail(BLZ_ERR_INVALID_PARAM, "law %d has no exit %d", law, exit);
    if (n == 0) return BLZ_OK;
    if (n > (1u << 20)) return fail(BLZ_ERR_INVALID_PARAM, "%zu cases (at most 2^20)", n);
    BLZ_TRY(use_device(device_id));
    const LawOp op = {program, exit, k, arg, in, out, n};
    return test_law_dispatch(curve, repr, law, nullptr, &op);
}

int blz_test_rr_layout(int curve, int field, uint32_t* out) {
    if (!out) return fail(BLZ_ERR_INVALID_PARAM, "null argument");
    return test_rr_dispatch(curve, field, out, nullptr);
}

int blz_test_rr_op(int device_id, int curve, int field, int op, int variant, const uint32_t* in, uint32_t* out, size_t n) {
    if (!in || !out) return fail(BLZ_ERR_INVALID_PARAM, "null argument");
    if (n == 0 || n > (1u << 20)) return fail(BLZ_ERR_INVALID_PARAM, "%zu cases (1 .. 2^20)", n);
    BLZ_TRY(use_device(device_id));
    const RrOp o = {op, variant, in, out, n};
    return test_rr_dispatch(curve, field, nullptr, &o);
}

int blz_test_sort_fits_beside(int acc_vgprs, int sort_vgprs, int acc_lds, int sort_lds) {
    return msm_sort_fits_beside(acc_vgprs, sort_vgprs, acc_lds, sort_lds) ? 1 : 0;
}

}
```

### include/blaze_hip_aux.h

```cpp
#ifndef BLAZE_HIP_AUX_H
#define BLAZE_HIP_AUX_H

#include "blaze_hip.h"

#ifdef __cplusplus
extern "C" {
#endif


int blz_synth_scalars(int device_id, int curve, void* d_out, uint64_t n, uint64_t seed);
int blz_synth_scalars_at(int device_id, int curve, void* d_out, uint64_t n, uint64_t seed, uint64_t start);
int blz_synth_points(int device_id, int curve, void* d_out, uint64_t n, int pf, uint64_t start);
int blz_synth_field_elements(int device_id, void* d_out, uint64_t n, uint64_t seed);

int blz_calib_mad_rate(int device_id, uint32_t target_ms, double out[4]);

int blz_test_msm_stall(blz_msm* h, uint32_t max_ms, void** token);
int blz_test_ntt_stall(blz_ntt* h, uint32_t max_ms, void** token);
int blz_test_stall_release(void* token);

int blz_test_field_op(int device_id, int curve, int field, int op, const uint8_t* a, const uint8_t* b,
                      uint8_t* out, size_t n);
int blz_test_ec_op(int device_id, int curve, int op, const uint8_t* p, const uint8_t* q,
                   const uint8_t* inf_flags, uint8_t* out, uint8_t* out_inf, size_t n);

int blz_test_msm_tail_plan(int curve, int repr, uint32_t npts, int sbits, int pieces, int table_c, int bit_lo, int bit_hi, uint32_t plan_out[8],
                           uint8_t* widths, char* text, size_t cap);
int blz_test_msm_sort_plan(int curve, int repr, uint32_t npts, int sbits, int pieces, int table_c, int bit_lo, int bit_hi, int hide_env, int other_busy,
                           int recent_hot, int fits, char* text, size_t cap);

int blz_test_law_layout(int curve, int repr, int law, uint32_t out[32]);
int blz_test_law_op(int device_id, int curve, int repr, int law, int program, int exit, uint32_t k, uint32_t arg, const uint32_t* in,
                    uint32_t* out, size_t n);

#define BLZ_RR_LAYOUT_WORDS 8192
int blz_test_rr_layout(int curve, int field, uint32_t* out);
int blz_test_rr_op(int device_id, int curve, int field, int op, int variant, const uint32_t* in, uint32_t* out, size_t n);

int blz_test_sort_fits_beside(int acc_vgprs, int sort_vgprs, int acc_lds, int sort_lds);

int blz_test_poseidon_permute(int device_id, int field, const uint8_t* words, size_t len, int t, const uint8_t* states_in,
                              uint8_t* states_out, size_t n);
int blz_test_poseidon_hash(int device_id, int field, const uint8_t* words, size_t len, int t, const uint8_t* inputs, uint8_t* digests,
                           size_t n);
int blz_test_poseidon_hash_plan(int device_id, int field, const uint8_t* words, size_t len, int t, const uint8_t* inputs, uint8_t* digests,
                                size_t n, uint32_t* state);
int blz_test_poseidon_tree_check(int device_id, int field, const uint8_t* words, size_t len, int tree_mode, uint32_t tree_height,
                                 const void* d_input, const void* d_records, uint64_t out[2]);

#ifdef __cplusplus
}
#endif
#endif
```

Baseline: 8.495.

## Skip level-1 count pass with statistically sized optimistic sort regions

```diff
diff --git a/blaze_amd/_lib.py b/blaze_amd/_lib.py
--- a/blaze_amd/_lib.py
+++ b/blaze_amd/_lib.py
@@ -187,6 +187,10 @@
                                          C.c_char_p, C.c_size_t]),
     "blz_test_msm_sort_plan": (C.c_int, [C.c_int, C.c_int, C.c_uint32, C.c_int, C.c_int, C.c_int, C.c_int, C.c_int, C.c_int, C.c_int, C.c_int, C.c_int,
                                          C.c_char_p, C.c_size_t]),
+    "blz_test_msm_sort_level1": (C.c_int, [C.c_int, C.c_int, C.c_uint32, C.c_int, C.c_int, C.c_int, C.c_int, C.c_int, C.c_int, C.c_int, C.c_int, C.c_int,
+                                           C.c_int, C.c_char_p, C.c_size_t]),
+    "blz_test_msm_sort_regions": (C.c_int, [C.c_int, C.c_uint32, C.c_int, C.POINTER(C.c_uint32)]),
+    "blz_test_msm_sort_path": (C.c_int, [C.c_void_p, C.POINTER(C.c_int)]),
     "blz_test_law_layout": (C.c_int, [C.c_int, C.c_int, C.c_int, C.POINTER(C.c_uint32)]),
     "blz_test_law_op": (C.c_int, [C.c_int, C.c_int, C.c_int, C.c_int, C.c_int, C.c_int, C.c_uint32, C.c_uint32, _u8p, _u8p, C.c_size_t]),
     "blz_test_rr_layout": (C.c_int, [C.c_int, C.c_int, C.POINTER(C.c_uint32)]),
diff --git a/blaze_amd/csrc/msm.hip b/blaze_amd/csrc/msm.hip
--- a/blaze_amd/csrc/msm.hip
+++ b/blaze_amd/csrc/msm.hip
@@ -373,6 +373,7 @@
 size_t MsmEngine::table_scratch_bytes(int W) const { return msm_ops_for(curve, repr)->table_scratch_bytes(W); }
 
 static const int kScalarFieldBits[3] = {253, 255, 254};
+static const double kScalarFieldFrac[3] = {0x12ab655e / 536870912.0, 0x73eda753 / 2147483648.0, 0x30644e72 / 1073741824.0};
 
 MsmPlan MsmEngine::plan_for(uint32_t npts, int sbits) const {
     const int ebits = sbits == 256 ? kScalarFieldBits[curve] : sbits;
@@ -401,6 +402,7 @@
                     : make_plan(npts, sbits, ebits, plan_override("c", 0));
     if (P.c == 0) return fail(BLZ_ERR_INVALID_PARAM, "no window plan for npts=%u sbits=%d%s", npts, sbits, table_c > 0 ? " (window table)" : "");
     if (P.table && !msm_sort3_ok(P, sbits)) return fail(BLZ_ERR_INVALID_PARAM, "window-table task outside the sort's range (c=%d)", P.c);
+    if (sbits == 256 && !P.table && P.ebits == kScalarFieldBits[curve] - (ranged ? bit_lo : 0)) P.ufrac = kScalarFieldFrac[curve];
     P.L = (uint32_t)plan_override("L", (int)P.L);
     if (P.L < 1) P.L = 1;
     if (P.L > (uint32_t)MAX_L) P.L = MAX_L;
@@ -453,10 +455,11 @@
     nslices = msm_task_pieces(P, nslices, phased, &per);
     BLZ_TRY(plan_tail(P, ops->tail, nslices > 1, S.tail));
     const SortInputs sort_in = {env_int("BLAZE_SORT_HIDE", 1), slots[(slot + 1) % MSM_QUEUE_DEPTH].busy, recent_hot[0] || recent_hot[1],
-                                msm_sort_fits_beside(ops->accumulate_vgprs(), msm_sort3_max_vgprs(P.table), ops->accumulate_lds(), msm_sort3_max_lds(P.table))};
+                                msm_sort_fits_beside(ops->accumulate_vgprs(), msm_sort3_max_vgprs(P.table), ops->accumulate_lds(), msm_sort3_max_lds(P.table)),
+                                recent_overflow};
     const SortPlan sort = plan_sort(P, npts, sbits, nslices, sort_in);
-    BLZ_LOG(2, "msm plan: npts=%u sbits=%d c=%d W=%d Bw=%u G=%llu L=%u pieces=%d sort: %s tail: %s", npts, sbits, P.c, P.W, P.Bw,
-            (unsigned long long)G, P.L, nslices, describe(sort).c_str(), describe(S.tail).c_str());
+    BLZ_LOG(2, "msm plan: npts=%u sbits=%d c=%d W=%d Bw=%u G=%llu L=%u pieces=%d sort: %s (level 1: %s) tail: %s", npts, sbits, P.c, P.W, P.Bw,
+            (unsigned long long)G, P.L, nslices, describe(sort).c_str(), describe_level1(sort), describe(S.tail).c_str());
     const uint64_t max_entries = (uint64_t)per * P.W;
     const uint64_t max_units = G + max_entries / P.L + 1;
     if (max_units >= (1ull << 32)) return fail(BLZ_ERR_INVALID_PARAM, "unit bound %llu exceeds 32 bits", (unsigned long long)max_units);
@@ -625,11 +628,13 @@
     BLZ_TRY(sync_event_bounded(S.ev_done, "wait_result: MSM task"));
     S.busy = false;
     if (S.plan.c) {
-        BLZ_LOG(2, "msm: units=%u max_bucket=%u entries=%u", S.stats_h[0], S.stats_h[1], S.stats_h[2]);
+        BLZ_LOG(2, "msm: units=%u max_bucket=%u entries=%u level1_overflow=%u", S.stats_h[0], S.stats_h[1], S.stats_h[2], S.stats_h[3]);
         if ((uint64_t)S.stats_h[0] > S.max_units) return fail(BLZ_ERR_UNKNOWN, "unit count %u exceeds its bound", S.stats_h[0]);
         const uint64_t mean = (uint64_t)S.stats_h[2] / (S.plan.G ? S.plan.G : 1) + 1;
         recent_hot[1] = recent_hot[0];
         recent_hot[0] = (uint64_t)S.stats_h[1] > 64 * mean + 4096;
+        last_sort_optimistic = S.sort.optimistic;
+        recent_overflow = S.stats_h[3] != 0;
     }
     memcpy(out, S.result_h, 3 * fq_bytes(curve));
     float t = 0;
diff --git a/blaze_amd/csrc/msm_engine.hpp b/blaze_amd/csrc/msm_engine.hpp
--- a/blaze_amd/csrc/msm_engine.hpp
+++ b/blaze_amd/csrc/msm_engine.hpp
@@ -21,6 +21,7 @@
     int ebits = 0;
     int base_bit = 0;
     double cost = 0;
+    double ufrac = 1.0;
 };
 MsmPlan make_plan(uint32_t npts, int sbits, int ebits, int force_c);
 int table_window_bits(uint32_t npts, int need_bits = 257);
@@ -59,10 +60,22 @@
 struct SortPlan {
     enum Kind { LDS, S3, TINY } kind;
     enum Where { OPEN, HIDDEN, PINGPONG } where;
-};
-struct SortInputs { int hide_env; bool other_busy, recent_hot, fits; };
+    bool optimistic = false;
+};
+struct SortInputs { int hide_env; bool other_busy, recent_hot, fits; bool recent_overflow = false; };
 SortPlan plan_sort(const MsmPlan& P, uint32_t npts, int sbits, int pieces, const SortInputs& in);
 std::string describe(const SortPlan&);
+const char* describe_level1(const SortPlan&);
+struct S3Regions {
+    int W = 0;
+    uint32_t rbase[MSM_MAX_W + 1] = {}, cap[MSM_MAX_W] = {}, cap2[MSM_MAX_W] = {};
+    uint16_t occ[MSM_MAX_W] = {}, occ2[MSM_MAX_W] = {}, bin0[MSM_MAX_W + 1] = {};
+    __host__ __device__ uint32_t start(int w, uint32_t k) const {
+        const uint32_t a = k < occ2[w] ? k : occ2[w], b = k < occ[w] ? k : occ[w];
+        return rbase[w] + a * cap2[w] + (b - a) * cap[w];
+    }
+};
+bool msm_sort3_regions(const MsmPlan& P, uint32_t npts, S3Regions& R);
 constexpr int SCAN_TILE = 2048;
 constexpr int MAX_L = 1024;
 
@@ -128,6 +141,7 @@
     float last_ms[8] = {};
     bool last_sort_hidden = false;
     bool recent_hot[2] = {false, false};
+    bool last_sort_optimistic = false, recent_overflow = false;
     template <class Fn>
     void for_each_buf(Fn&& f) {
         for (DevBuf* b : {&coarse, &inter, &inter2, &slice_map, &partial, &blocksums, &result, &sort3_tabs, &bucket_sums, &bucket_ident}) f(*b);
diff --git a/blaze_amd/csrc/msm_sort3.hip b/blaze_amd/csrc/msm_sort3.hip
--- a/blaze_amd/csrc/msm_sort3.hip
+++ b/blaze_amd/csrc/msm_sort3.hip
@@ -98,9 +98,32 @@
     return wbase + incl - v;
 }
 
+constexpr uint32_t S3_COUNTED = 0, S3_OPTIMISTIC = 1, S3_FALLBACK = 2;
+__device__ __forceinline__ bool s3_skip(const uint32_t* ovf, uint32_t mode) {
+    if (mode == S3_COUNTED) return false;
+    __shared__ uint32_t raised;
+    if (threadIdx.x == 0) raised = __hip_atomic_load(ovf, __ATOMIC_RELAXED, __HIP_MEMORY_SCOPE_AGENT);
+    __syncthreads();
+    return (mode == S3_FALLBACK) != (raised != 0u);
+}
+
+__global__ __launch_bounds__(S3_THREADS) void ks3_regions(S3Regions R, uint32_t* __restrict__ off1, uint32_t* __restrict__ cur1, int prio) {
+    s3_setprio(prio);
+    for (int w = 0; w < R.W; ++w) {
+        const uint32_t b0 = R.bin0[w], nb = (uint32_t)R.bin0[w + 1] - b0;
+        for (uint32_t k = threadIdx.x; k < nb; k += S3_THREADS) {
+            const uint32_t s = R.start(w, k);
+            off1[b0 + k] = s;
+            cur1[b0 + k] = s;
+        }
+    }
+    if (threadIdx.x == 0) off1[R.bin0[R.W]] = R.rbase[R.W];
+}
+
 template <class Geom, int NW>
 __global__ __launch_bounds__(S3_THREADS, 4) void k3_l1_count(const uint32_t* __restrict__ scalars, uint32_t npts, Geom g,
-                                                            uint32_t* __restrict__ cnt1) {
+                                                            uint32_t* __restrict__ cnt1, const uint32_t* __restrict__ ovf, uint32_t mode) {
+    if (s3_skip(ovf, mode)) return;
     s3_setprio(g.prio);
     __shared__ uint32_t hist[Geom::HIST1];
     if constexpr (Geom::HIST1 == S3_THREADS) hist[threadIdx.x] = 0;
@@ -140,7 +163,8 @@
 }
 
 __global__ __launch_bounds__(S3_THREADS) void k3_scan_small(const uint32_t* __restrict__ cnt, uint32_t n, uint32_t* __restrict__ off,
-                                                           uint32_t* __restrict__ cur, int prio) {
+                                                           uint32_t* __restrict__ cur, int prio, const uint32_t* __restrict__ ovf, uint32_t mode) {
+    if (s3_skip(ovf, mode)) return;
     s3_setprio(prio);
     __shared__ uint32_t wave_tot[4];
     uint32_t v[8], sum = 0;
@@ -166,7 +190,9 @@
 template <class Geom, int NW>
 __global__ __launch_bounds__(S3_THREADS, 4) void k3_l1_scatter(const uint32_t* __restrict__ scalars, uint32_t npts, Geom g,
                                                               uint32_t* __restrict__ cur1, uint32_t* __restrict__ o_idx,
-                                                              uint16_t* __restrict__ o_rem) {
+                                                              uint16_t* __restrict__ o_rem, const uint32_t* __restrict__ off1,
+                                                              uint32_t* __restrict__ ovf, uint32_t mode) {
+    if constexpr (!Geom::TABLE) { if (s3_skip(ovf, mode)) return; }
     s3_setprio(g.prio);
     extern __shared__ __attribute__((aligned(16))) uint32_t sh[];
     uint32_t* sc = sh;
@@ -175,8 +201,10 @@
     uint32_t* lstart = hist + 256;
     uint32_t* gbase = lstart + 256;
     __shared__ uint32_t wave_tot[4];
+    __shared__ uint32_t full;
     const uint32_t tid = threadIdx.x;
     const uint32_t base = blockIdx.x * (uint32_t)S3_PB;
+    if constexpr (!Geom::TABLE) { if (tid == 0) full = 0; }
 #pragma unroll
     for (int u = 0; u < S3_T; ++u) {
         const uint32_t p = base + u * S3_THREADS + tid;
@@ -237,9 +265,17 @@
                 lstart[tid] = excl;
                 uint32_t ci;
                 if constexpr (Geom::TABLE) ci = tid; else ci = (uint32_t)g.binoff1[w] + tid;
-                gbase[tid] = v ? atomicAdd(&cur1[ci], v) : 0u;
+                const uint32_t gb = v ? atomicAdd(&cur1[ci], v) : 0u;
+                gbase[tid] = gb;
+                if constexpr (!Geom::TABLE) {
+                    if (v && gb + v > off1[ci + 1]) {
+                        atomicOr(ovf, 1u);
+                        full = 1u;
+                    }
+                }
             }
             __syncthreads();
+            if constexpr (!Geom::TABLE) { if (full) return; }
 #pragma unroll
             for (int u = 0; u < S3_T; ++u) {
                 if (rk[u] != ~0u) {
@@ -262,8 +298,8 @@
     }
 }
 
-__global__ __launch_bounds__(S3_THREADS) void k3_slice_map(const uint32_t* __restrict__ off, uint32_t nbins, uint32_t slice,
-                                                          uint2* __restrict__ map, uint32_t* __restrict__ nitems, int prio) {
+__global__ __launch_bounds__(S3_THREADS) void k3_slice_map(const uint32_t* __restrict__ off, const uint32_t* __restrict__ end, uint32_t nbins,
+                                                          uint32_t slice, uint2* __restrict__ map, uint32_t* __restrict__ nitems, int prio) {
     s3_setprio(prio);
     __shared__ uint32_t wave_tot[4];
     __shared__ uint32_t carry_sh;
@@ -271,7 +307,7 @@
     __syncthreads();
     for (uint32_t base = 0; base < nbins; base += S3_THREADS) {
         const uint32_t i = base + threadIdx.x;
-        const uint32_t size = i < nbins ? off[i + 1] - off[i] : 0u;
+        const uint32_t size = i < nbins ? end[i] - off[i] : 0u;
         const uint32_t v = (size + slice - 1) / slice;
         uint32_t total;
         const uint32_t excl = s3_block_excl_scan(v, wave_tot, &total);
@@ -328,12 +364,12 @@
     if (blockIdx.x == 0 && threadIdx.x == 0) off[n] = bsum[256];
 }
 
-__device__ __forceinline__ bool s3_item(const uint32_t* off1, const uint2* map, const uint32_t* nitems, uint32_t id, uint32_t slice,
-                                        uint32_t& k, uint32_t& lo, uint32_t& hi) {
+__device__ __forceinline__ bool s3_item(const uint32_t* off1, const uint32_t* end1, const uint2* map, const uint32_t* nitems, uint32_t id,
+                                        uint32_t slice, uint32_t& k, uint32_t& lo, uint32_t& hi) {
     if (id >= *nitems) return false;
     const uint2 m = map[id];
     k = m.x;
-    const uint32_t a = off1[k], b = off1[k + 1];
+    const uint32_t a = off1[k], b = end1[k];
     lo = a + m.y * slice;
     hi = lo + slice < b ? lo + slice : b;
     return lo < hi;
@@ -341,12 +377,12 @@
 
 template <class Geom>
 __global__ __launch_bounds__(S3_THREADS, 4) void k3_l2_count(const uint16_t* __restrict__ rem, const uint32_t* __restrict__ off1,
-                                                            const uint2* __restrict__ map, const uint32_t* __restrict__ nitems,
-                                                            uint32_t* __restrict__ cnt2, Geom g) {
+                                                            const uint32_t* __restrict__ end1, const uint2* __restrict__ map,
+                                                            const uint32_t* __restrict__ nitems, uint32_t* __restrict__ cnt2, Geom g) {
     s3_setprio(g.prio);
     __shared__ uint32_t hist[Geom::TAB2];
     uint32_t k, lo, hi;
-    if (!s3_item(off1, map, nitems, blockIdx.x, S3_SLICE2, k, lo, hi)) return;
+    if (!s3_item(off1, end1, map, nitems, blockIdx.x, S3_SLICE2, k, lo, hi)) return;
     if (Geom::TAB2 == S3_THREADS || threadIdx.x < Geom::TAB2) hist[threadIdx.x] = 0;
     __syncthreads();
     const uint32_t sh = g.shift2();
@@ -368,8 +404,8 @@
 
 template <class Geom>
 __global__ __launch_bounds__(S3_THREADS, 4) void k3_l2_scatter(const uint32_t* __restrict__ i_idx, const uint16_t* __restrict__ i_rem,
-                                                              const uint32_t* __restrict__ off1, const uint2* __restrict__ map,
-                                                              const uint32_t* __restrict__ nitems, uint32_t* __restrict__ cur2,
+                                                              const uint32_t* __restrict__ off1, const uint32_t* __restrict__ end1,
+                                                              const uint2* __restrict__ map, const uint32_t* __restrict__ nitems, uint32_t* __restrict__ cur2,
                                                               uint32_t* __restrict__ o_idx, typename Geom::Lo* __restrict__ o_lo, Geom g) {
     s3_setprio(g.prio);
     constexpr uint32_t TAB2 = Geom::TAB2, KY_D = Geom::KY_D, KY_R = Geom::KY_R;
@@ -377,7 +413,7 @@
     __shared__ uint32_t hist[TAB2], lstart[TAB2], gbase[TAB2];
     __shared__ uint32_t wave_tot[4];
     uint32_t k, lo, hi;
-    if (!s3_item(off1, map, nitems, blockIdx.x, S3_SLICE2, k, lo, hi)) return;
+    if (!s3_item(off1, end1, map, nitems, blockIdx.x, S3_SLICE2, k, lo, hi)) return;
     const uint32_t tid = threadIdx.x;
     if (TAB2 == S3_THREADS || tid < TAB2) hist[tid] = 0;
     __syncthreads();
@@ -678,13 +714,18 @@
 
 template <class Geom, int NW>
 static int s3_level1(hipStream_t st, const uint32_t* sc, uint32_t npts, const Geom& g, uint32_t* cnt1, uint32_t* off1, uint32_t* cur1,
-                     uint32_t* i1_idx, uint16_t* i1_rem) {
-    const dim3 blk(S3_THREADS);
+                     uint32_t* i1_idx, uint16_t* i1_rem, uint32_t* ovf, const S3Regions* R) {
+    const dim3 blk(S3_THREADS), grid1((npts + S3_PB - 1) / S3_PB);
     const size_t lds1 = s3_lds1(NW);
-    hipLaunchKernelGGL((k3_l1_count<Geom, NW>), dim3((npts + S3_CNT_PTS - 1) / S3_CNT_PTS), blk, 0, st, sc, npts, g, cnt1);
-    hipLaunchKernelGGL(k3_scan_small, dim3(1), blk, 0, st, cnt1, g.NB1, off1, cur1, g.prio);
     BLZ_TRY(ensure_dynamic_lds((const void*)k3_l1_scatter<Geom, NW>, (int)lds1));
-    hipLaunchKernelGGL((k3_l1_scatter<Geom, NW>), dim3((npts + S3_PB - 1) / S3_PB), blk, lds1, st, sc, npts, g, cur1, i1_idx, i1_rem);
+    if (R) {
+        hipLaunchKernelGGL(ks3_regions, dim3(1), blk, 0, st, *R, off1, cur1, g.prio);
+        hipLaunchKernelGGL((k3_l1_scatter<Geom, NW>), grid1, blk, lds1, st, sc, npts, g, cur1, i1_idx, i1_rem, off1, ovf, S3_OPTIMISTIC);
+    }
+    const uint32_t mode = R ? S3_FALLBACK : S3_COUNTED;
+    hipLaunchKernelGGL((k3_l1_count<Geom, NW>), dim3((npts + S3_CNT_PTS - 1) / S3_CNT_PTS), blk, 0, st, sc, npts, g, cnt1, ovf, mode);
+    hipLaunchKernelGGL(k3_scan_small, dim3(1), blk, 0, st, cnt1, g.NB1, off1, cur1, g.prio, ovf, mode);
+    hipLaunchKernelGGL((k3_l1_scatter<Geom, NW>), grid1, blk, lds1, st, sc, npts, g, cur1, i1_idx, i1_rem, off1, ovf, mode);
     return BLZ_OK;
 }
 
@@ -711,10 +752,15 @@
     uint32_t* bsum = cur2 + NB2 + 2;
     uint32_t* nitems = bsum + 260;
     uint2* map = reinterpret_cast<uint2*>(nitems + 4);
-    BLZ_TRY(E.inter.reserve(max_entries * 6 + 64));
+    S3Regions R;
+    bool optimistic = false;
+    if constexpr (!Geom::TABLE) optimistic = C.S.sort.optimistic && msm_sort3_regions(P, npts, R);
+    const uint64_t len1 = optimistic && R.rbase[R.W] > max_entries ? R.rbase[R.W] : max_entries;
+    BLZ_TRY(E.inter.reserve(len1 * 6 + 64));
     BLZ_TRY(E.inter2.reserve(max_entries * (4 + sizeof(Lo)) + 64));
     uint32_t* i1_idx = E.inter.as<uint32_t>();
-    uint16_t* i1_rem = reinterpret_cast<uint16_t*>(i1_idx + max_entries);
+    uint16_t* i1_rem = reinterpret_cast<uint16_t*>(i1_idx + len1);
+    uint32_t* ovf = B.stats.as<uint32_t>() + 3;
     uint32_t* i2_idx = E.inter2.as<uint32_t>();
     Lo* i2_lo = reinterpret_cast<Lo*>(i2_idx + max_entries);
     uint32_t* count = B.count.as<uint32_t>();
@@ -726,16 +772,16 @@
     BLZ_HIP(hipMemsetAsync(cnt1, 0, (size_t)(NB1 + 2) * 4, st), BLZ_ERR_UNKNOWN);
     BLZ_HIP(hipMemsetAsync(cnt2, 0, (size_t)(NB2 + 2) * 4, st), BLZ_ERR_UNKNOWN);
     if constexpr (Geom::TABLE) {
-        BLZ_TRY((s3_level1<Geom, 8>(st, sc, npts, g, cnt1, off1, cur1, i1_idx, i1_rem)));
+        BLZ_TRY((s3_level1<Geom, 8>(st, sc, npts, g, cnt1, off1, cur1, i1_idx, i1_rem, ovf, nullptr)));
     } else {
-        BLZ_SW_DISPATCH(sbits, BLZ_TRY((s3_level1<Geom, SW>(st, sc, npts, g, cnt1, off1, cur1, i1_idx, i1_rem))));
-    }
-    hipLaunchKernelGGL(k3_slice_map, dim3(1), blk, 0, st, off1, NB1, S3_SLICE2, map, nitems, g.prio);
-    hipLaunchKernelGGL(k3_l2_count<L2>, dim3(max_items), blk, 0, st, i1_rem, off1, map, nitems, cnt2, g2);
+        BLZ_SW_DISPATCH(sbits, BLZ_TRY((s3_level1<Geom, SW>(st, sc, npts, g, cnt1, off1, cur1, i1_idx, i1_rem, ovf, optimistic ? &R : nullptr))));
+    }
+    hipLaunchKernelGGL(k3_slice_map, dim3(1), blk, 0, st, off1, cur1, NB1, S3_SLICE2, map, nitems, g.prio);
+    hipLaunchKernelGGL(k3_l2_count<L2>, dim3(max_items), blk, 0, st, i1_rem, off1, cur1, map, nitems, cnt2, g2);
     hipLaunchKernelGGL(k3_scan_a, dim3(nsb), blk, 0, st, cnt2, NB2, bsum, g.prio);
     hipLaunchKernelGGL(k3_scan_b, dim3(1), blk, 0, st, bsum, nsb, g.prio);
     hipLaunchKernelGGL(k3_scan_c, dim3(nsb), blk, 0, st, cnt2, NB2, bsum, off2, cur2, g.prio);
-    hipLaunchKernelGGL(k3_l2_scatter<L2>, dim3(max_items), blk, 0, st, i1_idx, i1_rem, off1, map, nitems, cur2, i2_idx, i2_lo, g2);
+    hipLaunchKernelGGL(k3_l2_scatter<L2>, dim3(max_items), blk, 0, st, i1_idx, i1_rem, off1, cur1, map, nitems, cur2, i2_idx, i2_lo, g2);
     if constexpr (Geom::TABLE) {
         const double mean_bin = (double)max_entries / (double)(NB2 ? NB2 : 1);
         const bool big_bins = mean_bin * 1.1 > (double)S3_R3;
diff --git a/blaze_amd/csrc/msm_sort_stage.hip b/blaze_amd/csrc/msm_sort_stage.hip
--- a/blaze_amd/csrc/msm_sort_stage.hip
+++ b/blaze_amd/csrc/msm_sort_stage.hip
@@ -2,7 +2,7 @@
 
 namespace blz {
 
-SortPlan plan_sort(const MsmPlan& P, uint32_t npts, int sbits, int pieces, const SortInputs& in) {
+static SortPlan plan_sort_where(const MsmPlan& P, uint32_t npts, int sbits, int pieces, const SortInputs& in) {
     const bool on = in.hide_env != 0, guarded = in.hide_env == 1;
     if (P.table)
         return {SortPlan::S3, on && in.other_busy && (!guarded || in.fits) ? SortPlan::HIDDEN : SortPlan::OPEN};
@@ -14,10 +14,72 @@
     return {msm_sort_tiny_ok(P, npts, sbits) ? SortPlan::TINY : SortPlan::LDS, SortPlan::OPEN};
 }
 
+SortPlan plan_sort(const MsmPlan& P, uint32_t npts, int sbits, int pieces, const SortInputs& in) {
+    SortPlan s = plan_sort_where(P, npts, sbits, pieces, in);
+#ifndef BLZ_S3_COUNTED
+    if (s.kind == SortPlan::S3 && !P.table && !in.recent_hot && !in.recent_overflow) {
+        S3Regions R;
+        s.optimistic = msm_sort3_regions(P, npts, R);
+    }
+#endif
+    return s;
+}
+
 std::string describe(const SortPlan& s) {
     static const char* const kind[] = {"lds", "s3", "tiny"};
     static const char* const where[] = {"open", "hidden", "pingpong"};
     return std::string(kind[s.kind]) + " " + where[s.where];
+}
+const char* describe_level1(const SortPlan& s) { return s.kind != SortPlan::S3 ? "-" : s.optimistic ? "optimistic" : "counted"; }
+
+bool msm_sort3_regions(const MsmPlan& P, uint32_t npts, S3Regions& R) {
+    if (P.table || P.W < 1 || P.W > MSM_MAX_W) return false;
+    const int forced = plan_override("s3_cap", 0);
+    const double f = P.ufrac > 0.5 && P.ufrac < 1.0 ? P.ufrac : 1.0;
+    const int ebits = P.ebits > 0 ? P.ebits : P.sbits;
+    auto region = [&](double p) -> uint32_t {
+        if (p > 1.0) p = 1.0;
+        const double mean = (double)npts * p;
+        double cap = ceil(mean + 8.0 * sqrt(mean * (1.0 - p)) + 1.0);
+        if (cap > (double)npts) cap = (double)npts;
+        return ((uint32_t)cap + 31u) & ~31u;
+    };
+    R = S3Regions();
+    R.W = P.W;
+    uint64_t total = 0;
+    int bit = 0;
+    for (int w = 0; w < P.W; ++w) {
+        const int cw = P.width[w], t = ebits - bit;
+        const uint32_t nb = (1u << (cw - 1)) >> 14;
+        if (cw < 15 || nb > 256) return false;
+        uint32_t occ = nb, occ2 = 0, cap = 0, cap2 = 0;
+        if (forced > 0) cap = ((uint32_t)forced + 31u) & ~31u;
+        else if (t > cw) cap = region((1.0 + ldexp(1.0, cw - t + 2)) / (double)nb);
+        else if (t == cw) cap = region(4.0 * 16384.0 / ldexp(1.0, t));
+        else if (t > 0) {
+            const double X = ldexp(1.0, t);
+            const double reach = ceil((f * X + 2.0) / 16384.0), reach2 = ceil(((1.0 - f) * X + 2.0) / 16384.0);
+            if (reach < (double)nb) occ = (uint32_t)reach;
+            if (f < 1.0) occ2 = reach2 < (double)occ ? (uint32_t)reach2 : occ;
+            cap = region(16384.0 / (f * X));
+            cap2 = region(2.0 * 16384.0 / X);
+        } else {
+            occ = 1;
+            cap = region(t == 0 ? 1.0 : 0.0);
+        }
+        R.cap[w] = cap;
+        R.cap2[w] = cap2;
+        R.occ[w] = (uint16_t)occ;
+        R.occ2[w] = (uint16_t)occ2;
+        R.bin0[w] = (uint16_t)(P.boff[w] >> 14);
+        R.rbase[w] = (uint32_t)total;
+        total += (uint64_t)occ2 * cap2 + (uint64_t)(occ - occ2) * cap;
+        if (total + (uint64_t)npts >= MSM_MAX_ENTRIES) return false;
+        bit += cw;
+    }
+    R.bin0[P.W] = (uint16_t)(P.boff[P.W] >> 14);
+    R.rbase[P.W] = (uint32_t)total;
+    return true;
 }
 
 bool msm_sort_fits_beside(int av, int sv, int al, int sl) {
diff --git a/blaze_amd/csrc/testhooks.hip b/blaze_amd/csrc/testhooks.hip
--- a/blaze_amd/csrc/testhooks.hip
+++ b/blaze_amd/csrc/testhooks.hip
@@ -5,6 +5,7 @@
 #include "poseidon_engine.hpp"
 #include "poseidon_impl.hip.hpp"
 #include "msm_engine.hpp"
+#include "msm_handle.hpp"
 #include "../../include/blaze_hip_aux.h"
 
 namespace blz {
@@ -1297,6 +1298,44 @@
     return BLZ_OK;
 }
 
+int blz_test_msm_sort_level1(int curve, int repr, uint32_t npts, int sbits, int pieces, int table_c, int bit_lo, int bit_hi, int hide_env, int other_busy,
+                             int recent_hot, int fits, int recent_overflow, char* text, size_t cap) {
+    if (!text || cap == 0) return fail(BLZ_ERR_INVALID_PARAM, "null argument");
+    if (!msm_ops_for(curve, repr) || npts == 0) return fail(BLZ_ERR_INVALID_PARAM, "unknown curve %d or empty task", curve);
+    MsmPlan P;
+    BLZ_TRY(msm_task_plan(curve, npts, sbits, table_c, bit_lo, bit_hi, P, nullptr));
+    uint32_t per = 0;
+    pieces = msm_task_pieces(P, pieces, false, &per);
+    const SortPlan s = plan_sort(P, npts, sbits, pieces, SortInputs{hide_env, other_busy != 0, recent_hot != 0, fits != 0, recent_overflow != 0});
+    const std::string line = describe(s) + " " + describe_level1(s);
+    if (line.size() >= cap) return fail(BLZ_ERR_INVALID_PARAM, "text buffer of %zu bytes for a line of %zu", cap, line.size());
+    memcpy(text, line.c_str(), line.size() + 1);
+    return BLZ_OK;
+}
+
+int blz_test_msm_sort_regions(int curve, uint32_t npts, int sbits, uint32_t* out) {
+    if (!out || npts == 0) return fail(BLZ_ERR_INVALID_PARAM, "null argument or empty task");
+    MsmPlan P;
+    BLZ_TRY(msm_task_plan(curve, npts, sbits, 0, 0, 0, P, nullptr));
+    S3Regions R;
+    memset(out, 0, BLZ_SORT_REGION_WORDS * sizeof(uint32_t));
+    if (!msm_sort3_ok(P, sbits) || !msm_sort3_regions(P, npts, R)) return BLZ_OK;
+    out[0] = (uint32_t)R.W;
+    out[1] = R.rbase[R.W];
+    for (int w = 0; w < R.W; ++w) {
+        const uint32_t row[6] = {P.width[w], R.rbase[w], R.occ2[w], R.cap2[w], R.occ[w], R.cap[w]};
+        memcpy(out + 2 + 6 * w, row, sizeof(row));
+    }
+    return BLZ_OK;
+}
+
+int blz_test_msm_sort_path(blz_msm* h, int out[2]) {
+    if (!h || !out) return fail(BLZ_ERR_INVALID_PARAM, "null argument");
+    out[0] = h->eng.last_sort_optimistic ? 1 : 0;
+    out[1] = h->eng.recent_overflow ? 1 : 0;
+    return BLZ_OK;
+}
+
 int blz_test_law_layout(int curve, int repr, int law, uint32_t out[32]) {
     if (!out) return fail(BLZ_ERR_INVALID_PARAM, "null argument");
     LawLayout L;
diff --git a/include/blaze_hip_aux.h b/include/blaze_hip_aux.h
--- a/include/blaze_hip_aux.h
+++ b/include/blaze_hip_aux.h
@@ -29,6 +29,12 @@
 int blz_test_msm_sort_plan(int curve, int repr, uint32_t npts, int sbits, int pieces, int table_c, int bit_lo, int bit_hi, int hide_env, int other_busy,
                            int recent_hot, int fits, char* text, size_t cap);
 
+#define BLZ_SORT_REGION_WORDS 578
+int blz_test_msm_sort_level1(int curve, int repr, uint32_t npts, int sbits, int pieces, int table_c, int bit_lo, int bit_hi, int hide_env, int other_busy,
+                             int recent_hot, int fits, int recent_overflow, char* text, size_t cap);
+int blz_test_msm_sort_regions(int curve, uint32_t npts, int sbits, uint32_t* out);
+int blz_test_msm_sort_path(blz_msm* h, int out[2]);
+
 int blz_test_law_layout(int curve, int repr, int law, uint32_t out[32]);
 int blz_test_law_op(int device_id, int curve, int repr, int law, int program, int exit, uint32_t k, uint32_t arg, const uint32_t* in,
                     uint32_t* out, size_t n);
```

New measurement: 8.517 (median of 6 runs). About the same (+0.3%).
